# zhoubin-me/agent0

Hardware: AMD Instinct MI355X
Metric: env-frames/sec (learner FPS: transitions collected and saved to replay per second with the learner running, pre-frameskip) (higher is better)
Workload: dtype f32

## Files before the change

### agent0_amd/csrc/a0_internal.h

```cpp
#pragma once
#include "../../include/agent0_hip.h"
#include "a0_defs.h"

#include <exception>
#if defined(__HIPCC__)
#include <hip/hip_ext.h>
#endif
#include <stdexcept>
#include <string>

int a0_fail(int code, const char* msg);
int a0_fail_hip(int hip_error, const char* what);

struct a0_hip_error : std::runtime_error {
    int err;
    a0_hip_error(int e, const std::string& w) : std::runtime_error(w), err(e) {}
};

#define A0_STR2(x) #x
#define A0_STR(x) A0_STR2(x)
#define A0_HIP_THROW(expr)                                                                                  \
    do {                                                                                                    \
        hipError_t a0_e_ = (expr);                                                                          \
        if (a0_e_ != hipSuccess) throw a0_hip_error((int)a0_e_, std::string(__FILE__ ":" A0_STR(__LINE__) ": ") + hipGetErrorString(a0_e_)); \
    } while (0)

#define A0_TRY try {
#define A0_CATCH                                                   \
    }                                                              \
    catch (const a0_hip_error& e) { return a0_fail_hip(e.err, e.what()); } \
    catch (const std::exception& e) { return a0_fail(A0_EINVAL, e.what()); } \
    catch (...) { return a0_fail(A0_EINVAL, "unknown C++ exception"); }

void a0_trace_push_internal(const char* name);
void a0_trace_pop_internal();
struct a0_trace_scope {
    explicit a0_trace_scope(const char* name) { a0_trace_push_internal(name); }
    ~a0_trace_scope() { a0_trace_pop_internal(); }
    a0_trace_scope(const a0_trace_scope&) = delete;
    a0_trace_scope& operator=(const a0_trace_scope&) = delete;
};

#if defined(__HIPCC__)
bool a0_probe_start(int tag, hipStream_t st);
int a0_conv1_wgrad_fused_launch(const a0_frames_arg* f, int C, int H, int W, int B, const float* d1, float* slabs, hipStream_t st);
void a0_probe_stop(hipStream_t st, double flops);
bool a0_probe_events(int tag, hipEvent_t* start, hipEvent_t* stop);
void a0_probe_commit(double flops);
int a0_x9_products_now();
#define A0_LAUNCH_PROBED(tag, flops, kern, grid, block, lds, st, ...)                                                              \
    do {                                                                                                                           \
        hipEvent_t a0_e0_ = nullptr, a0_e1_ = nullptr;                                                                             \
        if (a0_probe_events((tag), &a0_e0_, &a0_e1_)) {                                                                            \
            hipExtLaunchKernelGGL(kern, grid, block, (uint32_t)(lds), st, a0_e0_, a0_e1_, 0, __VA_ARGS__);                         \
            a0_probe_commit(flops);                                                                                                \
        } else                                                                                                                     \
            hipLaunchKernelGGL(kern, grid, block, lds, st, __VA_ARGS__);                                                           \
    } while (0)
struct a0_net_core;
int a0_conv23_wgrad_fused_launch(const a0_net_core& n, int B, const float* act1, const float* act2, const float* d2, const float* d3, float* slab2, float* slab3,
                                 hipStream_t st);
#endif
#define A0_TAG_ENCODER_FUSED 12
#define A0_TAG_ENCODER_DGRAD_FUSED 13
#define A0_TAG_ACTOR_STEP_ENC 14
```

### agent0_amd/csrc/actor_tail.h

```cpp
#pragma once
#include "synth_env.h"
template <class Issued>
A0_D void a0_qhead_wave(const float* __restrict__ slabs, long long slab_stride, int nslab, const float* __restrict__ b1, const float* __restrict__ w2s,
                        const float* __restrict__ b2, int A, int dueling, int er, int lane, float* __restrict__ raw, unsigned long long seed, uint32_t stream_a,
                        uint32_t stream_u, unsigned long long off_a, unsigned long long off_u, float eps, int& out_action, float& out_best, Issued&& issued) {
    const int NQ = A + (dueling ? 1 : 0);
    bool hooked = false;
    float h[8];
#pragma unroll
    for (int i = 0; i < 8; ++i) h[i] = 0.f;
    const float* sp = slabs + (long long)er * 512 + lane;
    int z = 0;
    for (; z + 8 <= nslab; z += 8) {
        float t[8][8];
#pragma unroll
        for (int zz = 0; zz < 8; ++zz)
#pragma unroll
            for (int i = 0; i < 8; ++i) t[zz][i] = sp[(long long)(z + zz) * slab_stride + 64 * i];
        if (!hooked) { issued(); hooked = true; }
#pragma unroll
        for (int zz = 0; zz < 8; ++zz)
#pragma unroll
            for (int i = 0; i < 8; ++i) h[i] += t[zz][i];
    }
// ... 195 lines not shown
    }
    __builtin_amdgcn_fence(__ATOMIC_RELEASE, "wavefront");
    __builtin_amdgcn_wave_barrier();
    __builtin_amdgcn_fence(__ATOMIC_ACQUIRE, "wavefront");
    {
        if (P.dueling) {
            for (int t = lane; t < T; t += 64) {
                float s = 0.f;
                for (int a = 0; a < A; ++a) s += xs[a * T + t];
                const float mean = s / (float)A;
                const float v = xs[A * T + t];
                for (int a = 0; a < A; ++a) xs[a * T + t] = v + (xs[a * T + t] - mean);
            }
            __builtin_amdgcn_fence(__ATOMIC_RELEASE, "wavefront");
            __builtin_amdgcn_wave_barrier();
            __builtin_amdgcn_fence(__ATOMIC_ACQUIRE, "wavefront");
        }
        float best = 0.f;
        int besta = 0;
        for (int a = 0; a < A; ++a) {
            const float* p = xs + a * T;
            float v;
            if (P.mode == 1) {
                float s = 0.f;
                for (int t = lane; t < T; t += 64) s += p[t];
                v = a0_wave_sum(s) / (float)T;
            } else if (P.mode == 3) {
                const float* tau = P.taus + (long long)e * (T + 1);
                float s = 0.f;
                for (int t = lane; t < T; t += 64) s += (tau[t + 1] - tau[t]) * p[t];
                v = a0_wave_sum(s);
            } else {
                float mx = -INFINITY;
                for (int t = lane; t < T; t += 64) mx = fmaxf(mx, p[t]);
                mx = a0_wave_max(mx);
                float se = 0.f, sz = 0.f;
                for (int t = lane; t < T; t += 64) {
                    float ex = expf(p[t] - mx);
                    se += ex;
                    sz += ex * P.atoms[t];
                }
                se = a0_wave_sum(se);
                sz = a0_wave_sum(sz);
                v = sz / se;
            }
            if (a == 0 || v > best) { best = v; besta = a; }
        }
        if (lane == 0) {
            const int ra = (int)(a0_philox_word(seed_v, sa_v, off_a + (unsigned long long)e) % (uint32_t)A);
            const float u = (float)(a0_philox_word(seed_v, su_v, off_u + (unsigned long long)e) >> 8) * 0x1.0p-24f;
            const int act = (u > eps) ? besta : ra;
            action_v[e] = act; qmax_v[e] = best;
            float r_chase = 0.f;
            if (chase) *s_chase_cell_p = a0_chase_step(a0_chase_cell(P.obs_in + ((size_t)e * 4 + 3) * A0_ENV_PIX, e), act, x.w, r_chase);
            a0_env_commit_finish(Z, x, e, g, task_v, A, E_v, n_v, steps, gamma_v, act, O.ep_ret, O.final_mask, O.final_ret, O.ring_act, O.ring_rew, O.ring_done, O.r_act, O.r_rew,
                                 O.r_done, slot, r_chase);
        }
    }
}

A0_D void a0_actor_dist_tail_env_body(const a0_dtenv_args& P, float* __restrict__ xs, int* __restrict__ s_chase_cell_p) {
    const int wave = __builtin_amdgcn_readfirstlane(threadIdx.x >> 6);
    const uint32_t e = blockIdx.x;
    uint32_t g = P.g; long long start = P.start;
    if (P.ctrl) { g += (uint32_t)P.ctrl[A0_CTRL_ENV_STEP]; start += P.ctrl[A0_CTRL_REPLAY_SLOT]; }
    const long long slot = (start + e) % P.cap;
    uint32_t e_v = e;
    asm volatile("" : "+v"(e_v));
    const a0_u4 x = a0_philox4x32_10(e_v, g, 0u, 0x454E56u, (uint32_t)P.env_seed, (uint32_t)(P.env_seed >> 32) ^ P.rank);
    const bool term = (x.y % 500u) == 0u;
    const bool chase = P.task == A0_ENV_TASK_CHASE;
    if (wave != 0) {
        int cell = -1;
        if (chase) { __syncthreads(); cell = *s_chase_cell_p; }
        a0_env_commit_frames(P.env_seed, e, g, term, P.obs_in, P.obs_out, P.obs0, P.frames + slot * (8LL * A0_ENV_PIX), (int)threadIdx.x - 64, 448, cell);
        return;
    }
    a0_actor_dist_tail_wave0(P, xs, s_chase_cell_p, g, slot, x);
    if (chase) __syncthreads();
}


struct a0_encoder_weights;
int a0_actor_step_enc_launch(const a0_qenv_args& Q, const float* wt, const a0_encoder_weights* w, float* act3, hipStream_t st);
int a0_actor_dist_step_enc_launch(const a0_dtenv_args& Q, size_t tail_lds, const float* wt, const a0_encoder_weights* w, float* act3, hipStream_t st);
```

### agent0_amd/csrc/encoder_fused.hip

```cpp
#include "a0_internal.h"
#include "net_tables.h"
#include "operands.h"

#include <cstdlib>
#include <type_traits>

#ifndef A0_X9_MAXORD
#define A0_X9_MAXORD 4
#endif
typedef float a0_acc4 __attribute__((ext_vector_type(4)));

struct a0_fused_args {
    const uint8_t* frames; const int* slot; long long sample_stride; int chan_off;
    const float *wt1, *wt2, *wt3;
    const float *wx2, *wx3;
    const float *b1, *b2, *b3;
    float *act1, *act2, *act3;
    int B;
    int C, H, W, H1, W1, H2, W2, H3, W3;
    int off_act1, off_act2, off_end;
    int rp1, rp2;
};

#ifndef A0_FUSED_WAVES_D
#define A0_FUSED_WAVES_D 8
#endif
constexpr int A0_FUSED_WAVES = A0_FUSED_WAVES_D;
constexpr int A0_WMG1 = A0_FUSED_WAVES / 2;
constexpr int A0_FUSED_THREADS = 64 * A0_FUSED_WAVES;
constexpr int A0_P1 = 33;
constexpr int A0_P2 = 66;

struct AF2 {
    const float* act; int RP1, W2;
    A0_D int row(int m) const { const int oh = m / W2, ow = m - oh * W2; return (2 * oh) * RP1 + 2 * ow * A0_P1; }
    A0_D int chunk_off(int c) const { const int cell = c >> 1; return (cell >> 2) * RP1 + (cell & 3) * A0_P1 + 16 * (c & 1); }
    A0_D int step_off(int s) const { return 4 * s; }
    typedef float Raw;
    A0_D Raw load(int addr) const { return act[addr]; }
    static A0_D float value(Raw r) { return r; }
};
struct AF3 {
    const float* act; int RP2, W3;
    A0_D int row(int m) const { const int oh = m / W3, ow = m - oh * W3; return oh * RP2 + ow * A0_P2; }
    A0_D int chunk_off(int c) const { const int cell = c >> 2; return (cell / 3) * RP2 + (cell % 3) * A0_P2 + 16 * (c & 3); }
    A0_D int step_off(int s) const { return 4 * s; }
    typedef float Raw;
    A0_D Raw load(int addr) const { return act[addr]; }
    static A0_D float value(Raw r) { return r; }
};

template <int N, int WN, int R>
struct a0_wring {
    static constexpr int NBW = N / 16 / WN;
    a0_f4 v[R][NBW];
    const float* base;
    const float* p;
    int nch, left;
    A0_D void init(const float* wp, int K) {
        const int lane = threadIdx.x & 63, wave = __builtin_amdgcn_readfirstlane(threadIdx.x >> 6);
        const int n = (wave % WN) * (NBW * 16) + (lane & 15), q = lane >> 4;
        base = wp + (n * 4 + q) * 4;
        nch = K >> 4;
    }
    A0_D void fill(int slot) {
#pragma unroll
        for (int j = 0; j < NBW; ++j) v[slot][j] = *(const a0_f4*)(p + j * 256);
        const bool more = left > 1;
        p += more ? N * 16 : 0;
        left -= more ? 1 : 0;
    }
    A0_D void prologue() {
        p = base; left = nch;
#pragma unroll
        for (int u = 0; u < R; ++u) fill(u);
    }
};
A0_D float a0_f4_get(const a0_f4& v, int j) { return j == 0 ? v.x : j == 1 ? v.y : j == 2 ? v.z : v.w; }

template <int OWC>
struct EpiFwd {
    static constexpr bool PER_ELEM = false;
    static constexpr bool TR = false;
    const float* bias; float* lds; int pitch, rp, ow; float* glb; int N;
    A0_D float pre_col(int n) const { return bias[n]; }
    A0_D float pre_elem(int, int) const { return 0.f; }
    A0_D void emit(int m, int n, float acc, float pre) const {
        float v = acc + pre;
        v = (v < 0.f) ? 0.f : v;
        if (lds) {
            const int w_ = OWC > 0 ? OWC : ow, oh = m / w_;
            lds[oh * rp + (m - oh * w_) * pitch + n] = v;
        }
        if (glb) glb[(unsigned)(m * N + n)] = v;
    }
    static constexpr bool ROW4 = OWC > 0 && (OWC % 4) == 0;
    A0_D void emit4(int m0, int n, const a0_acc4& acc, float pre) const {
        constexpr int OWD = OWC > 0 ? OWC : 1;
        const int oh = m0 / OWD, ow0 = m0 - oh * OWD;
        float* l = lds ? lds + oh * rp + ow0 * pitch + n : nullptr;
// ... 225 lines not shown
            }
        }
    }
    __syncthreads();
}

template <int N, int WN, int R, int WK = 1>
struct a0_wring9 {
    static constexpr int NBW = N / 16 / WN;
    uint4 v[R][NBW][3];
    const uint4* base;
    const uint4* p;
    int nst, left, stride;
    A0_D void init(const float* wp, int K) {
        const int lane = threadIdx.x & 63, wave = __builtin_amdgcn_readfirstlane(threadIdx.x >> 6);
        base = (const uint4*)wp + (((wave % WN) * (NBW * 16) + (lane & 15)) * 4 + (lane >> 4)) * 3 + (WK > 1 ? (wave / WN) * (N * 12) : 0);
        nst = (K >> 5) / WK;
        stride = N * 12 * WK;
    }
    A0_D void init_at(const uint4* first, int own_steps, int step) { base = first; nst = own_steps; stride = step; }
    A0_D void fill(int slot) {
#pragma unroll
        for (int j = 0; j < NBW; ++j)
#pragma unroll
            for (int s = 0; s < 3; ++s) v[slot][j][s] = p[j * 192 + s];
        const bool more = left > 1;
        p += more ? stride : 0;
        left -= more ? 1 : 0;
    }
    A0_D void prologue() {
        p = base; left = nst;
#pragma unroll
        for (int u = 0; u < R; ++u) fill(u);
    }
};
template <int TERM>
struct AF2X {
    static constexpr int term = TERM;
    const uint16_t* planes; int RP, W2, P;
    A0_D int row(int m) const { const int oh = m / W2, ow = m - oh * W2; return (2 * oh) * RP + 2 * ow * P; }
    A0_D int step_off(int st) const { return (st >> 2) * RP + (st & 3) * P; }
};
template <int TERM>
struct AF3X {
    static constexpr int term = TERM;
    const uint16_t* planes; int RP, W3, P;
    A0_D int row(int m) const { const int oh = m / W3, ow = m - oh * W3; return oh * RP + ow * P; }
    A0_D int step_off(int st) const { const int tap = st >> 1; return (tap / 3) * RP + (tap % 3) * P + 32 * (st & 1); }
};
A0_D void a0_split4(const float (&v)[4], uint2& hi, uint2& mid, uint2& lo) {
    uint32_t h[4], m[4], l[4];
#pragma unroll
    for (int r = 0; r < 4; ++r) {
        h[r] = __float_as_uint(v[r]);
        const float r1 = v[r] - __uint_as_float(h[r] & 0xffff0000u);
        m[r] = __float_as_uint(r1);
        l[r] = __float_as_uint(r1 - __uint_as_float(m[r] & 0xffff0000u));
    }
    hi = uint2{__builtin_amdgcn_perm(h[1], h[0], 0x07060302u), __builtin_amdgcn_perm(h[3], h[2], 0x07060302u)};
    mid = uint2{__builtin_amdgcn_perm(m[1], m[0], 0x07060302u), __builtin_amdgcn_perm(m[3], m[2], 0x07060302u)};
    lo = uint2{__builtin_amdgcn_perm(l[1], l[0], 0x07060302u), __builtin_amdgcn_perm(l[3], l[2], 0x07060302u)};
}
template <int OWC, int P, int RP, int term>
struct EpiFwdX {
    static constexpr bool PER_ELEM = false;
    static constexpr bool ROW4 = false;
    static constexpr bool TR = true;
    static_assert(OWC > 0 && (P % 4) == 0 && (RP % 4) == 0 && (term % 4) == 0, "output width known at compile time; 8-byte aligned plane writes");
    const float* bias; uint16_t* planes; float* glb; int N;
    A0_D float pre_col(int) const { return 0.f; }
    A0_D void emit_n4(int m, int n0, const a0_acc4& acc, const float*) const {
        const a0_f4 bv = *(const a0_f4*)(bias + n0);
        float v[4] = {acc[0] + bv.x, acc[1] + bv.y, acc[2] + bv.z, acc[3] + bv.w};
#pragma unroll
        for (int r = 0; r < 4; ++r) v[r] = (v[r] < 0.f) ? 0.f : v[r];
        if (glb) *(a0_f4*)(glb + (unsigned)(m * N + n0)) = a0_f4{v[0], v[1], v[2], v[3]};
        uint2 hi, mid, lo;
        a0_split4(v, hi, mid, lo);
        const int oh = m / OWC;
        uint16_t* d = planes + oh * RP + (m - oh * OWC) * P + n0;
        *(uint2*)d = hi; *(uint2*)(d + term) = mid; *(uint2*)(d + 2 * term) = lo;
    }
};
struct EpiFwdT {
    static constexpr bool PER_ELEM = false;
    static constexpr bool ROW4 = false;
    static constexpr bool TR = true;
    const float* bias; float* glb; int N;
    A0_D float pre_col(int) const { return 0.f; }
    A0_D void emit_n4(int m, int n0, const a0_acc4& acc, const float*) const {
        const a0_f4 bv = *(const a0_f4*)(bias + n0);
        float v[4] = {acc[0] + bv.x, acc[1] + bv.y, acc[2] + bv.z, acc[3] + bv.w};
#pragma unroll
        for (int r = 0; r < 4; ++r) v[r] = (v[r] < 0.f) ? 0.f : v[r];
        *(a0_f4*)(glb + (unsigned)(m * N + n0)) = a0_f4{v[0], v[1], v[2], v[3]};
    }
};

template <int ORD, int N, int WN, int MBW, int R, int MBWP, class AFX, class EPI, class Between>
A0_D void a0_conv_stage_x9(const AFX& af, int M, a0_wring9<N, WN, R>& ring, const EPI& epi, const a0_pre<N, WN, MBWP, EPI>& pre, Between&& between) {
    constexpr int NB = N / 16, NBW = NB / WN, WMG = A0_FUSED_WAVES / WN;
    static_assert(NBW >= 1 && (R % 2) == 0 && MBWP >= MBW, "tile shape");
    const int tid = threadIdx.x, lane = tid & 63;
    const int wave = __builtin_amdgcn_readfirstlane(tid >> 6);
    const int wn = wave % WN, wmg = wave / WN;
    const int q = lane >> 4, r16 = lane & 15;
    const int MB = (M + 15) >> 4, NST = ring.nst;
    int rows[MBW];
#pragma unroll
    for (int i = 0; i < MBW; ++i) {
        const int m = (wmg + i * WMG) * 16 + r16;
        rows[i] = af.row(m < M ? m : 0) + 8 * q;
    }
    a0_acc4 acc[MBW][NBW];
#pragma unroll
    for (int i = 0; i < MBW; ++i)
#pragma unroll
        for (int j = 0; j < NBW; ++j) acc[i][j] = a0_acc4{0.f, 0.f, 0.f, 0.f};
    uint4 a[2][MBW][3];
    auto fetch = [&](int slot, int off) {
#pragma unroll
        for (int i = 0; i < MBW; ++i)
#pragma unroll
            for (int t = 0; t < 3; ++t) a[slot][i][t] = *(const uint4*)(af.planes + rows[i] + off + t * AFX::term);
    };
    fetch(0, af.step_off(0));
    __builtin_amdgcn_s_waitcnt(0x0F70);
#pragma unroll 1
    for (int tb = 0; tb < NST; tb += R) {
#pragma unroll
        for (int u = 0; u < R; ++u) {
            const int nxt = tb + u + 1;
            fetch((u + 1) & 1, af.step_off(nxt < NST ? nxt : NST - 1));
            __builtin_amdgcn_sched_barrier(0);
#pragma unroll
            for (int ta = 0; ta < 3; ++ta)
#pragma unroll
                for (int tw = 0; tw < 3; ++tw)
#pragma unroll
                    for (int i = 0; i < MBW; ++i)
#pragma unroll
                        for (int jn = 0; jn < NBW; ++jn) {
                            if (ta + tw > ORD) continue;
                            const a0_u32x4 av = {a[u & 1][i][ta].x, a[u & 1][i][ta].y, a[u & 1][i][ta].z, a[u & 1][i][ta].w};
                            const a0_u32x4 bv = {ring.v[u][jn][tw].x, ring.v[u][jn][tw].y, ring.v[u][jn][tw].z, ring.v[u][jn][tw].w};
                            if constexpr (EPI::TR) acc[i][jn] = __builtin_amdgcn_mfma_f32_16x16x32_bf16(__builtin_bit_cast(a0_bf16x8, bv), __builtin_bit_cast(a0_bf16x8, av), acc[i][jn], 0, 0, 0);
                            else acc[i][jn] = __builtin_amdgcn_mfma_f32_16x16x32_bf16(__builtin_bit_cast(a0_bf16x8, av), __builtin_bit_cast(a0_bf16x8, bv), acc[i][jn], 0, 0, 0);
                        }
            __builtin_amdgcn_sched_barrier(0);
            ring.fill(u);
            __builtin_amdgcn_sched_barrier(0);
        }
    }
    between();
#pragma unroll
    for (int i = 0; i < MBW; ++i) {
        const int mb = wmg + i * WMG;
        if (mb < MB) {
            if constexpr (EPI::TR) {
                const int m = mb * 16 + r16;
                if (m < M) {
#pragma unroll
                    for (int j = 0; j < NBW; ++j) epi.emit_n4(m, (wn * NBW + j) * 16 + 4 * q, acc[i][j], EPI::PER_ELEM ? pre.pe[EPI::PER_ELEM ? i : 0][j] : pre.pc[j]);
                }
            } else {
#pragma unroll
                for (int j = 0; j < NBW; ++j) {
                    const int n = (wn * NBW + j) * 16 + r16;
#pragma unroll
                    for (int r = 0; r < 4; ++r) {
                        const int m = mb * 16 + 4 * q + r;
                        if (m < M) epi.emit(m, n, acc[i][j][r], EPI::PER_ELEM ? pre.pe[EPI::PER_ELEM ? i : 0][j][r] : pre.pc[j][0]);
                    }
                }
            }
        }
    }
    __syncthreads();
// ... 52 lines not shown
                __builtin_amdgcn_sched_barrier(0);
            }
            ring.fill(u);
            __builtin_amdgcn_sched_barrier(0);
        }
    }
    between();
    a0_acc4* x0 = (a0_acc4*)xch0;
    a0_acc4* x1 = (a0_acc4*)xch1;
    constexpr int P1 = (HB1 - 1) * 64 + 4 * LR;
    const int last = q * LR + r16;
    const int n0 = wn * 16 + 4 * q;
    float pe[EPI::PER_ELEM ? HB0 : 1][4];
    auto send = [&](auto mine) {
        constexpr int H = decltype(mine)::value;
        if constexpr (EPI::PER_ELEM) {
#pragma unroll
            for (int i = 0; i < (H == 0 ? HB0 : HB1); ++i) {
                const int m = (H * HB0 + i) * 16 + r16;
                const a0_f4 v = epi.pre_elem4(m < M ? m : M - 1, n0);
                pe[i][0] = v.x; pe[i][1] = v.y; pe[i][2] = v.z; pe[i][3] = v.w;
            }
        }
        if constexpr (H == 1) {
#pragma unroll
            for (int i = 0; i < HB0; ++i) x0[(wn * HB0 + i) * 64 + lane] = acc[i];
        } else {
#pragma unroll
            for (int i = 0; i < HB1; ++i) {
                if (i < HB1 - 1) x1[wn * P1 + i * 64 + lane] = acc[HB0 + i];
                else if (r16 < LR) x1[wn * P1 + (HB1 - 1) * 64 + last] = acc[HB0 + i];
            }
        }
    };
    auto recv = [&](auto mine) {
        constexpr int H = decltype(mine)::value;
#pragma unroll
        for (int i = 0; i < (H == 0 ? HB0 : HB1); ++i) {
            const int mb = H * HB0 + i;
            const int m = mb * 16 + r16;
            if constexpr (H == 0) acc[mb] += x0[(wn * HB0 + i) * 64 + lane];
            else {
                if (i < HB1 - 1) acc[mb] += x1[wn * P1 + i * 64 + lane];
                else if (r16 < LR) acc[mb] += x1[wn * P1 + (HB1 - 1) * 64 + last];
            }
            if (mb < MB && m < M) epi.emit_n4(m, n0, acc[mb], EPI::PER_ELEM ? pe[EPI::PER_ELEM ? i : 0] : nullptr);
        }
    };
    if (wk == 0) send(std::integral_constant<int, 0>{});
    else send(std::integral_constant<int, 1>{});
    __syncthreads();
    if (wk == 0) recv(std::integral_constant<int, 0>{});
    else recv(std::integral_constant<int, 1>{});
    __syncthreads();
}
constexpr int A0_P1X = 40, A0_P2X = 80;
#ifndef A0_PADS
#define A0_PADS 1
#endif
constexpr int A0_RP1X = 20 * A0_P1X + (A0_PADS ? 8 : 0);
constexpr int A0_RP2X = 9 * A0_P2X + (A0_PADS ? 96 : 0);
#ifndef A0_RX2_D
#define A0_RX2_D 4
#endif
#ifndef A0_RX3_D
#define A0_RX3_D 6
#endif
[[maybe_unused]] constexpr int A0_RX2 = A0_RX2_D, A0_RX3 = A0_RX3_D;
#ifndef A0_KSPLIT_D
#define A0_KSPLIT_D 1
#endif
#ifndef A0_KSPLIT
#define A0_KSPLIT 1
#endif
#ifndef A0_WNX
#define A0_WNX 4
#endif

constexpr int A0_R1 = 4, A0_R2 = 4, A0_R3 = 6;

#ifndef A0_FUSED_MINWAVES
#define A0_FUSED_MINWAVES 1
#endif
template <int MBW1, int MBW2, int MBW3, int WC, bool X9, bool LOOP = false, int ORD = 4>
__global__ __launch_bounds__(A0_FUSED_THREADS, A0_FUSED_MINWAVES) void a0_encoder_fused_kernel(a0_fused_args P);

constexpr int A0_X9_BIAS_OFF = 2 * 4 * 84 * 84 + 3 * 20 * A0_RP1X * 2;
#ifndef A0_RK2_D
#define A0_RK2_D 2
#endif
#ifndef A0_RK3_D
#define A0_RK3_D 3
#endif
constexpr int A0_RK2 = A0_RK2_D, A0_RK3 = A0_RK3_D;
constexpr int A0_X9_XCH0 = 3 * 9 * A0_RP2X * 2;
constexpr int A0_X9_XCH1 = A0_X9_BIAS_OFF + 160 * 4;
static_assert(A0_X9_XCH0 + 4 * 3 * 1024 <= 2 * 4 * 84 * 84, "conv2 exchange region 0 fits into the image");
constexpr int A0_X9_LDS_BYTES = A0_X9_XCH1 + (A0_KSPLIT ? 4 * (2 * 64 + 4) * 16 : 0);
static_assert(A0_X9_LDS_BYTES <= 160 * 1024, "LDS");
#if A0_KSPLIT
typedef a0_wring9<64, 4, A0_RK2, 2> a0_ring2_t;
typedef a0_wring9<64, 4, A0_RK3, 2> a0_ring3_t;
#else
typedef a0_wring9<64, A0_WNX, A0_RX2> a0_ring2_t;
typedef a0_wring9<64, A0_WNX, A0_RX3> a0_ring3_t;
#endif
template <int ORD, int MBW2, int MBW3, bool LOOP>
A0_D void a0_x9_conv23(const a0_fused_args& P, int b, unsigned char* smem, float* bias_lds, a0_wring1<A0_R1>& ring1, a0_ring2_t& ring2, a0_ring3_t& ring3) {
    const int obs_bytes = P.C * P.H * P.W;
    const int M2 = P.H2 * P.W2, M3 = P.H3 * P.W3;
    uint16_t* a1p = (uint16_t*)(smem + 2 * obs_bytes);
    constexpr int term1 = 20 * A0_RP1X, term2 = 9 * A0_RP2X;
    uint16_t* a2p = (uint16_t*)smem;
    typedef EpiFwdX<9, A0_P2X, A0_RP2X, term2> E2X;
    constexpr int WNX = A0_WNX, WMGX = A0_FUSED_WAVES / WNX;
    constexpr int MBW2X = (6 + WMGX - 1) / WMGX, MBW3X = (4 + WMGX - 1) / WMGX;
    static_assert(MBW2X <= MBW2 * 2 && MBW3X <= MBW3 * 2, "84x84 geometry");
#if !A0_KSPLIT
    a0_pre<64, WNX, MBW2X, E2X> pre2;
    a0_pre<64, WNX, MBW3X, EpiFwdT> pre3;
#endif
    (void)a1p; (void)term1;
    {
        const AF2X<term1> f2{a1p, A0_RP1X, P.W2, A0_P1X};
        const E2X e2{bias_lds + 32, a2p, P.act2 ? P.act2 + (long long)b * M2 * 64 : nullptr, 64};
#if A0_KSPLIT
        const AF3X<term2> f3k{a2p, A0_RP2X, P.W3, A0_P2X};
        const EpiFwdT e3k{bias_lds + 96, P.act3 + (long long)b * M3 * 64, 64};
        a0_conv_stage_x9k<ORD, 64, 4, 6, A0_RK2, 1>(f2, M2, ring2, e2, (float*)(smem + A0_X9_XCH0), (float*)(smem + A0_X9_XCH1), [&] { ring3.prologue(); });
        a0_conv_stage_x9k<ORD, 64, 4, 4, A0_RK3, 16>(f3k, M3, ring3, e3k, (float*)a1p, (float*)a1p + 4 * 2 * 256, [&] { if (LOOP) ring1.prologue(); });
#else
        const int wmgx = __builtin_amdgcn_readfirstlane(threadIdx.x >> 6) / WNX;
        constexpr bool uneven2 = MBW2X > 1 && MBW2X * WMGX > 6, uneven3 = MBW3X > 1 && MBW3X * WMGX > 4;
        if (uneven2 && wmgx + (MBW2X - 1) * WMGX >= 6)
            a0_conv_stage_x9<ORD, 64, WNX, (MBW2X > 1 ? MBW2X - 1 : 1), A0_RX2>(f2, M2, ring2, e2, pre2, [&] { ring3.prologue(); });
        else
            a0_conv_stage_x9<ORD, 64, WNX, MBW2X, A0_RX2>(f2, M2, ring2, e2, pre2, [&] { ring3.prologue(); });
        const AF3X<term2> f3{a2p, A0_RP2X, P.W3, A0_P2X};
        const EpiFwdT e3{bias_lds + 96, P.act3 + (long long)b * M3 * 64, 64};
        if (uneven3 && wmgx + (MBW3X - 1) * WMGX >= 4)
            a0_conv_stage_x9<ORD, 64, WNX, (MBW3X > 1 ? MBW3X - 1 : 1), A0_RX3>(f3, M3, ring3, e3, pre3, [&] { if (LOOP) ring1.prologue(); });
        else
            a0_conv_stage_x9<ORD, 64, WNX, MBW3X, A0_RX3>(f3, M3, ring3, e3, pre3, [&] { if (LOOP) ring1.prologue(); });
#endif
    }
}

template <int ORD, int MBW1, int MBW2, int MBW3, bool LOOP>
A0_D void a0_encoder_fused_x9_body(const a0_fused_args& P, int bid, int nblk) {
    extern __shared__ __attribute__((aligned(16))) unsigned char smem[];
    uint16_t* img = (uint16_t*)smem;
    const int obs_bytes = P.C * P.H * P.W;
    const int M1 = P.H1 * P.W1;
    uint16_t* a1p = (uint16_t*)(smem + 2 * obs_bytes);
    constexpr int term1 = 20 * A0_RP1X;
    typedef EpiFwdX<20, A0_P1X, A0_RP1X, term1> E1X;
    constexpr int WNX = A0_WNX, WMGX = A0_FUSED_WAVES / WNX;
    constexpr int MBW2X = (6 + WMGX - 1) / WMGX, MBW3X = (4 + WMGX - 1) / WMGX;
    static_assert(MBW2X <= MBW2 * 2 && MBW3X <= MBW3 * 2, "84x84 geometry");
    a0_wring1<A0_R1> ring1;
#if A0_KSPLIT
    static_assert(WNX == 4 && A0_FUSED_WAVES == 8, "N-stationary stages: four waves along N, two along K");
#endif
    a0_ring2_t ring2;
    a0_ring3_t ring3;
    ring1.init(P.wt1, P.C);
    ring2.init(P.wx2, 512);
    ring3.init(P.wx3, 576);
    ring1.prologue();
    constexpr int MBW1X = (25 + A0_WMG1 - 1) / A0_WMG1;
    static_assert(A0_FUSED_WAVES != 8 || MBW1X == MBW1, "84x84 geometry");
    a0_pre<32, 2, MBW1X, E1X> pre1;
    float* bias_lds = (float*)(smem + A0_X9_BIAS_OFF);
    if (threadIdx.x < 160) bias_lds[threadIdx.x] = threadIdx.x < 32 ? P.b1[threadIdx.x] : threadIdx.x < 96 ? P.b2[threadIdx.x - 32] : P.b3[threadIdx.x - 96];
    for (int b = bid; b < P.B; b += nblk) {
        const long long s = P.slot ? (long long)P.slot[b] : (long long)b;
        const uint4* src = (const uint4*)(P.frames + s * P.sample_stride + P.chan_off);
        constexpr int TRIPS = 4;
        const int n16 = obs_bytes >> 4;
        for (int i0 = threadIdx.x; i0 < n16; i0 += TRIPS * A0_FUSED_THREADS) {
            uint4 v[TRIPS];
#pragma unroll
            for (int j = 0; j < TRIPS; ++j) {
                const int i = i0 + j * A0_FUSED_THREADS;
                v[j] = src[i < n16 ? i : n16 - 1];
            }
#pragma unroll
            for (int j = 0; j < TRIPS; ++j) {
                int i = i0 + j * A0_FUSED_THREADS;
                i = i < n16 ? i : n16 - 1;
                const uint32_t w[4] = {v[j].x, v[j].y, v[j].z, v[j].w};
                uint32_t o[8];
#pragma unroll
                for (int k = 0; k < 4; ++k) {
                    const uint32_t f0 = __float_as_uint((float)(w[k] & 0xffu)), f1 = __float_as_uint((float)((w[k] >> 8) & 0xffu));
                    const uint32_t f2 = __float_as_uint((float)((w[k] >> 16) & 0xffu)), f3 = __float_as_uint((float)(w[k] >> 24));
                    o[2 * k] = __builtin_amdgcn_perm(f1, f0, 0x07060302u);
                    o[2 * k + 1] = __builtin_amdgcn_perm(f3, f2, 0x07060302u);
                }
                ((uint4*)img)[2 * i] = uint4{o[0], o[1], o[2], o[3]};
                ((uint4*)img)[2 * i + 1] = uint4{o[4], o[5], o[6], o[7]};
            }
        }
        __syncthreads();
        const E1X e1{bias_lds, a1p, P.act1 ? P.act1 + (long long)b * M1 * 32 : nullptr, 32};
        const int wmg1 = __builtin_amdgcn_readfirstlane(threadIdx.x >> 6) / 2;
        if (MBW1X > 1 && wmg1 + (MBW1X - 1) * A0_WMG1 >= ((M1 + 15) >> 4))
            a0_conv1_stage<(MBW1X > 1 ? MBW1X - 1 : 1), A0_R1, 84>(img, P.H * P.W, P.W, P.W1, M1, ring1, e1, pre1, [&] { ring2.prologue(); });
        else
            a0_conv1_stage<MBW1X, A0_R1, 84>(img, P.H * P.W, P.W, P.W1, M1, ring1, e1, pre1, [&] { ring2.prologue(); });
        a0_x9_conv23<ORD, MBW2, MBW3, LOOP>(P, b, smem, bias_lds, ring1, ring2, ring3);
        if constexpr (!LOOP) break;
    }
}

#include "actor_tail.h"
struct a0_step_enc_args { const float *wt, *b1, *b2, *b3; float* act3; };
template <int ORD>
__global__ __launch_bounds__(A0_FUSED_THREADS, A0_FUSED_MINWAVES) void a0_actor_dist_step_enc_kernel(a0_dtenv_args Q, a0_step_enc_args N) {
    __shared__ int s_chase_cell;
    extern __shared__ __attribute__((aligned(16))) unsigned char smem[];
    unsigned long long v_wt = (unsigned long long)N.wt, v_b1 = (unsigned long long)N.b1, v_b2 = (unsigned long long)N.b2, v_b3 = (unsigned long long)N.b3,
                       v_a3 = (unsigned long long)N.act3, v_obs = (unsigned long long)Q.obs_out;
    A0_TO_VGPR(v_wt); A0_TO_VGPR(v_b1); A0_TO_VGPR(v_b2); A0_TO_VGPR(v_b3); A0_TO_VGPR(v_a3); A0_TO_VGPR(v_obs);
    int v_E = Q.E;
    A0_TO_VGPR(v_E);
    a0_actor_dist_tail_env_body(Q, (float*)smem, &s_chase_cell);
    __syncthreads();
    auto uni = [](unsigned long long v) {
        return ((unsigned long long)(unsigned)__builtin_amdgcn_readfirstlane((int)(v >> 32)) << 32) | (unsigned long long)(unsigned)__builtin_amdgcn_readfirstlane((int)(v & 0xffffffffull));
    };
    const float* wt = (const float*)uni(v_wt);
    a0_fused_args P;
    P.frames = (const uint8_t*)uni(v_obs); P.slot = nullptr; P.sample_stride = 4 * 84 * 84; P.chan_off = 0;
    P.wt1 = wt; P.wt2 = wt + 48LL * 4 * 64; P.wt3 = P.wt2 + 64LL * 512;
    P.wx2 = P.wt3 + 64LL * 576 + 64LL * 576 + 4LL * 32 * 256; P.wx3 = P.wx2 + 96LL * 512;
    P.b1 = (const float*)uni(v_b1); P.b2 = (const float*)uni(v_b2); P.b3 = (const float*)uni(v_b3);
    P.act1 = nullptr; P.act2 = nullptr; P.act3 = (float*)uni(v_a3); P.B = __builtin_amdgcn_readfirstlane(v_E);
    P.C = 4; P.H = 84; P.W = 84; P.H1 = 20; P.W1 = 20; P.H2 = 9; P.W2 = 9; P.H3 = 7; P.W3 = 7;
    P.off_act1 = 0; P.off_act2 = 0; P.off_end = 0; P.rp1 = 0; P.rp2 = 0;
    a0_encoder_fused_x9_body<ORD, 7, 3, 2, false>(P, (int)blockIdx.x, (int)gridDim.x);
}

A0_D void a0_bytes16_to_img(uint16_t* img, int idx16, const uint4 v) {
    const uint32_t w[4] = {v.x, v.y, v.z, v.w};
    uint32_t o[8];
#pragma unroll
    for (int k = 0; k < 4; ++k) {
        const uint32_t f0 = __float_as_uint((float)(w[k] & 0xffu)), f1 = __float_as_uint((float)((w[k] >> 8) & 0xffu));
        const uint32_t f2 = __float_as_uint((float)((w[k] >> 16) & 0xffu)), f3 = __float_as_uint((float)(w[k] >> 24));
        o[2 * k] = __builtin_amdgcn_perm(f1, f0, 0x07060302u);
        o[2 * k + 1] = __builtin_amdgcn_perm(f3, f2, 0x07060302u);
    }
    ((uint4*)img)[2 * idx16] = uint4{o[0], o[1], o[2], o[3]};
    ((uint4*)img)[2 * idx16 + 1] = uint4{o[4], o[5], o[6], o[7]};
}

template <int MBW, class EPI, class Mid, class Between>
A0_D void a0_conv1_stage_split(const uint16_t* img, a0_wring1<A0_R1>& ring, const EPI& epi, bool first_before_mid, Mid&& mid, Between&& between) {
    static_assert(A0_R1 == 4 && EPI::TR, "ring of four steps, transposed accumulators");
    constexpr int HW = 84 * 84, W = 84, W1 = 20, M = 400, MB = 25;
    const int tid = threadIdx.x, lane = tid & 63;
    const int wave = __builtin_amdgcn_readfirstlane(tid >> 6);
    const int wn = wave % 2, wmg = wave / 2;
    const int q = lane >> 4, r16 = lane & 15;
    int rows[MBW];
#pragma unroll
    for (int i = 0; i < MBW; ++i) {
        int m = (wmg + i * A0_WMG1) * 16 + r16;
        m = m < M ? m : 0;
        const int oh = m / W1, ow = m - oh * W1;
        rows[i] = (4 * oh + q) * W + 4 * ow;
    }
    a0_acc4 acc[MBW];
#pragma unroll
    for (int i = 0; i < MBW; ++i) acc[i] = a0_acc4{0.f, 0.f, 0.f, 0.f};
    uint2 a[2][MBW][2];
    auto fetch = [&](int slot, int off) {
#pragma unroll
        for (int i = 0; i < MBW; ++i) {
            a[slot][i][0] = *(const uint2*)(img + rows[i] + off);
            a[slot][i][1] = *(const uint2*)(img + rows[i] + off + 4);
        }
    };
    auto off_of = [&](int st) { return (st >> 1) * HW + (st & 1) * 4 * W; };
    auto step = [&](auto UC, int off_next) {
        constexpr int u = decltype(UC)::value;
        fetch((u + 1) & 1, off_next);
        __builtin_amdgcn_sched_barrier(0);
#pragma unroll
        for (int s3 = 0; s3 < 3; ++s3)
#pragma unroll
            for (int i = 0; i < MBW; ++i) {
                const a0_u32x4 av = {a[u & 1][i][0].x, a[u & 1][i][0].y, a[u & 1][i][1].x, a[u & 1][i][1].y};
                const a0_u32x4 bv = {ring.v[u][s3].x, ring.v[u][s3].y, ring.v[u][s3].z, ring.v[u][s3].w};
                acc[i] = __builtin_amdgcn_mfma_f32_16x16x32_bf16(__builtin_bit_cast(a0_bf16x8, bv), __builtin_bit_cast(a0_bf16x8, av), acc[i], 0, 0, 0);
            }
        __builtin_amdgcn_sched_barrier(0);
        ring.fill(u);
        __builtin_amdgcn_sched_barrier(0);
    };
    typedef std::integral_constant<int, 0> U0; typedef std::integral_constant<int, 1> U1; typedef std::integral_constant<int, 2> U2; typedef std::integral_constant<int, 3> U3;
    auto steps05 = [&] {
        fetch(0, off_of(0));
        __builtin_amdgcn_s_waitcnt(0x0F70);
        step(U0{}, off_of(1)); step(U1{}, off_of(2)); step(U2{}, off_of(3)); step(U3{}, off_of(4));
        step(U0{}, off_of(5)); step(U1{}, off_of(5));
    };
    if (first_before_mid) steps05();
    mid();
    if (!first_before_mid) steps05();
    fetch(0, off_of(6));
    __builtin_amdgcn_s_waitcnt(0x0F70);
    step(U2{}, off_of(7)); step(U3{}, off_of(7));
    between();
#pragma unroll
    for (int i = 0; i < MBW; ++i) {
        const int mb = wmg + i * A0_WMG1;
        if (mb < MB) {
            const int m = mb * 16 + r16;
            if (m < M) epi.emit_n4(m, wn * 16 + 4 * q, acc[i], nullptr);
        }
    }
    __syncthreads();
}

struct TailScalar {
    typedef a0_qenv_args Args;
    static A0_D void run(const a0_qenv_args& Q, uint32_t e, uint32_t g, long long steps, unsigned long long off_a, unsigned long long off_u, float eps, long long slot, const a0_u4& x,
                         bool chase, int lane, float* w2s , float* raw, int* s_chase_cell_p) {
        const int NQ = Q.A + (Q.dueling ? 1 : 0);
        a0_env_pre Z;
        a0_env_commit_prefetch(Z, e, Q.E, Q.n, steps, Q.ep_ret, Q.ring_act, Q.ring_rew, Q.ring_done);
        a0_env_pre_to_vgpr(Z);
        const a0_env_out O = a0_env_out_vgpr(Q.ep_ret, Q.final_mask, Q.final_ret, Q.ring_act, Q.ring_rew, Q.ring_done, Q.r_act, Q.r_rew, Q.r_done);
        A0_TO_VGPR(steps); A0_TO_VGPR(off_a); A0_TO_VGPR(off_u); A0_TO_VGPR(eps);
        int n_v = Q.n, E_v = Q.E, task_v = Q.task; double gamma_v = Q.gamma; int* action_v = Q.action; float* qmax_v = Q.qmax;
        A0_TO_VGPR(n_v); A0_TO_VGPR(E_v); A0_TO_VGPR(task_v); A0_TO_VGPR(gamma_v); A0_TO_VGPR(action_v); A0_TO_VGPR(qmax_v);
#pragma unroll 4
        for (int i = lane; i < NQ * 128; i += 64) ((a0_f4*)w2s)[i] = ((const a0_f4*)Q.W2)[i];
        __builtin_amdgcn_fence(__ATOMIC_RELEASE, "wavefront");
        __builtin_amdgcn_wave_barrier();
        __builtin_amdgcn_fence(__ATOMIC_ACQUIRE, "wavefront");
        int act = 0; float best = 0.f;
        a0_qhead_wave(Q.slabs, Q.slab_stride, Q.nslab, Q.b1, w2s, Q.b2, Q.A, Q.dueling, (int)e, lane, raw, Q.rng_seed, Q.stream_a, Q.stream_u, off_a, off_u, eps, act, best);
        if (lane == 0) {
            action_v[e] = act; qmax_v[e] = best;
            float r_chase = 0.f;
            if (chase) *s_chase_cell_p = a0_chase_step(a0_chase_cell(Q.obs_in + ((size_t)e * 4 + 3) * A0_ENV_PIX, e), act, x.w, r_chase);
            a0_env_commit_finish(Z, x, e, g, task_v, Q.A, E_v, n_v, steps, gamma_v, act, O.ep_ret, O.final_mask, O.final_ret, O.ring_act, O.ring_rew, O.ring_done, O.r_act, O.r_rew,
                                 O.r_done, slot, r_chase);
        }
    }
};
template <int ORD, class TAIL>
A0_D void a0_actor_step_enc2_body(const typename TAIL::Args& Q, const a0_step_enc_args& N) {
    __shared__ float raw[64];
    __shared__ int s_chase_cell;
    extern __shared__ __attribute__((aligned(16))) unsigned char smem[];
    constexpr int HW = 84 * 84, G16 = HW / 16;
    uint16_t* img = (uint16_t*)smem;
    uint16_t* a1p = (uint16_t*)(smem + 2 * 4 * HW);
    const int tid = threadIdx.x, lane = tid & 63, wave = __builtin_amdgcn_readfirstlane(tid >> 6);
    const uint32_t e = blockIdx.x;
    a0_fused_args P;
    P.frames = nullptr; P.slot = nullptr; P.sample_stride = 4 * HW; P.chan_off = 0;
    P.wt1 = N.wt; P.wt2 = N.wt + 48LL * 4 * 64; P.wt3 = P.wt2 + 64LL * 512;
    P.wx2 = P.wt3 + 64LL * 576 + 64LL * 576 + 4LL * 32 * 256; P.wx3 = P.wx2 + 96LL * 512;
    P.b1 = N.b1; P.b2 = N.b2; P.b3 = N.b3;
    P.act1 = nullptr; P.act2 = nullptr; P.act3 = N.act3; P.B = Q.E;
    P.C = 4; P.H = 84; P.W = 84; P.H1 = 20; P.W1 = 20; P.H2 = 9; P.W2 = 9; P.H3 = 7; P.W3 = 7;
    P.off_act1 = 0; P.off_act2 = 0; P.off_end = 0; P.rp1 = 0; P.rp2 = 0;
    a0_wring1<A0_R1> ring1;
    a0_ring2_t ring2;
    a0_ring3_t ring3;
    ring1.init(P.wt1, 4);
    ring1.prologue();
    float* bias_lds = (float*)(smem + A0_X9_BIAS_OFF);
    if (tid < 160) bias_lds[tid] = tid < 32 ? P.b1[tid] : tid < 96 ? P.b2[tid - 32] : P.b3[tid - 96];
    unsigned long long v_wx2 = (unsigned long long)P.wx2, v_wx3 = (unsigned long long)P.wx3;
    A0_TO_VGPR(v_wx2); A0_TO_VGPR(v_wx3);
    uint32_t g = Q.g; long long steps = Q.steps, start = Q.start; unsigned long long off_a = Q.off_a, off_u = Q.off_u; float eps = Q.eps;
    if (Q.ctrl) {
        g += (uint32_t)Q.ctrl[A0_CTRL_ENV_STEP]; steps += Q.ctrl[A0_CTRL_ACTOR_STEPS]; start += Q.ctrl[A0_CTRL_REPLAY_SLOT];
        off_a += (unsigned long long)Q.ctrl[A0_CTRL_RNG_ACTION]; off_u += (unsigned long long)Q.ctrl[A0_CTRL_RNG_UNIFORM];
    }
    if (Q.eps_ptr) eps = Q.eps_ptr[0];
    const long long slot = (start + e) % Q.cap;
    uint32_t e_v = e;
    asm volatile("" : "+v"(e_v));
    const a0_u4 x = a0_philox4x32_10(e_v, g, 0u, 0x454E56u, (uint32_t)Q.env_seed, (uint32_t)(Q.env_seed >> 32) ^ Q.rank);
    const bool term = __builtin_amdgcn_readfirstlane((int)((x.y % 500u) == 0u)) != 0;
    const bool chase = Q.task == A0_ENV_TASK_CHASE;
    const bool early = !(chase && term);
    const int j = tid - 64;
    auto has_group = [&] { int jj = j; asm volatile("" : "+v"(jj)); return wave != 0 && jj < G16; };
    const uint32_t pbase = (uint32_t)Q.env_seed ^ a0_env_mix32(e * 0x9E3779B1u + g);
    uint4* out16 = (uint4*)(Q.obs_out + (size_t)e * 4 * HW) + j;
    uint4* row16 = (uint4*)(Q.frames + slot * (8LL * HW)) + j;
    A0_TO_VGPR(out16); A0_TO_VGPR(row16);
    float* act3_v = N.act3;
    A0_TO_VGPR(act3_v);
    auto new_group = [&](uint32_t by, uint32_t bx) {
        uint32_t w[4];
#pragma unroll
        for (int k = 0; k < 4; ++k) {
            const uint32_t p = 16u * (uint32_t)j + 4u * (uint32_t)k;
            w[k] = (uint32_t)a0_env_pixel(pbase, by, bx, p, chase) | ((uint32_t)a0_env_pixel(pbase, by, bx, p + 1, chase) << 8) |
                   ((uint32_t)a0_env_pixel(pbase, by, bx, p + 2, chase) << 16) | ((uint32_t)a0_env_pixel(pbase, by, bx, p + 3, chase) << 24);
        }
        return uint4{w[0], w[1], w[2], w[3]};
    };
    auto put = [&](int c, const uint4 v) {
        out16[c * G16] = v; row16[(4 + c) * G16] = v;
        a0_bytes16_to_img(img, c * G16 + j, v);
    };
    __shared__ int s_staged;
    if (tid == 0) s_staged = 0;
    __syncthreads();
    uint4 keep[9];
    if (wave == 0) {
        TAIL::run(Q, e, g, steps, off_a, off_u, eps, slot, x, chase, lane, (float*)a1p, raw, &s_chase_cell);
    } else {
        if (has_group()) {
            const uint4* in16 = (const uint4*)(Q.obs_in + (size_t)e * 4 * HW) + j;
            A0_TO_VGPR(in16);
            const uint4 i0 = in16[0], i1 = in16[G16], i2 = in16[2 * G16], i3 = in16[3 * G16];
            if (Q.obs0 == Q.obs_in) { keep[0] = i0; keep[1] = i1; keep[2] = i2; keep[3] = i3; }
            else {
                const uint4* o016 = (const uint4*)(Q.obs0 + (size_t)e * 4 * HW) + j;
                A0_TO_VGPR(o016);
                keep[0] = o016[0]; keep[1] = o016[G16]; keep[2] = o016[2 * G16]; keep[3] = o016[3 * G16];
            }
            if (!chase) {
                const uint4 nw = new_group((3u * g + 11u * e) % 77u, (5u * g + 7u * e) % 77u);
                if (term) { keep[4] = nw; keep[5] = nw; keep[6] = nw; } else { keep[4] = i1; keep[5] = i2; keep[6] = i3; }
                keep[7] = nw;
                for (int c = 0; c < 4; ++c) a0_bytes16_to_img(img, c * G16 + j, keep[4 + c]);
            } else if (!term) {
                keep[4] = i1; keep[5] = i2; keep[6] = i3;
                for (int c = 0; c < 3; ++c) a0_bytes16_to_img(img, c * G16 + j, keep[4 + c]);
            }
        }
        asm volatile("s_waitcnt lgkmcnt(0)" ::: "memory");
        if (lane == 0) atomicAdd(&s_staged, 1);
        while (__builtin_amdgcn_readfirstlane(*(volatile int*)&s_staged) < A0_FUSED_WAVES - 1) __builtin_amdgcn_s_sleep(1);
    }
    auto early_stores = [&] {
        if (has_group()) {
#pragma unroll
            for (int c = 0; c < 4; ++c) row16[c * G16] = keep[c];
            const int nc = !chase ? 4 : (!term ? 3 : 0);
#pragma unroll
            for (int c = 0; c < 4; ++c)
                if (c < nc) { out16[c * G16] = keep[4 + c]; row16[(4 + c) * G16] = keep[4 + c]; }
        }
    };
    auto mid = [&] {
        if (wave != 0) early_stores();
        __syncthreads();
        if (chase) {
            if (has_group()) {
                uint32_t by, bx;
                a0_chase_pos(s_chase_cell, by, bx);
                const uint4 nw = new_group(by, bx);
                if (term) { put(0, nw); put(1, nw); put(2, nw); }
                put(3, nw);
            }
            __syncthreads();
        }
    };
    auto uni = [](unsigned long long v) {
        return ((unsigned long long)(unsigned)__builtin_amdgcn_readfirstlane((int)(v >> 32)) << 32) | (unsigned long long)(unsigned)__builtin_amdgcn_readfirstlane((int)(v & 0xffffffffull));
    };
    ring2.init((const float*)uni(v_wx2), 512);
    ring3.init((const float*)uni(v_wx3), 576);
    typedef EpiFwdX<20, A0_P1X, A0_RP1X, 20 * A0_RP1X> E1X;
    const E1X e1{bias_lds, a1p, nullptr, 32};
    constexpr int MBW1X = (25 + A0_WMG1 - 1) / A0_WMG1;
    const bool before = early && wave != 0;
    if (MBW1X > 1 && wave / 2 + (MBW1X - 1) * A0_WMG1 >= 25)
        a0_conv1_stage_split<(MBW1X > 1 ? MBW1X - 1 : 1)>(img, ring1, e1, before, mid, [&] { ring2.prologue(); });
    else
        a0_conv1_stage_split<MBW1X>(img, ring1, e1, before, mid, [&] { ring2.prologue(); });
    P.act3 = (float*)uni((unsigned long long)act3_v);
    a0_x9_conv23<ORD, 3, 2, false>(P, (int)e, smem, bias_lds, ring1, ring2, ring3);
}

template <int ORD>
__global__ __launch_bounds__(A0_FUSED_THREADS, A0_FUSED_MINWAVES) void a0_actor_step_enc2_kernel(a0_qenv_args Q, a0_step_enc_args N) { a0_actor_step_enc2_body<ORD, TailScalar>(Q, N); }

static bool a0_fused_layout(int C, int H, int W, a0_fused_args& P, size_t& lds_bytes);
int a0_actor_dist_step_enc_launch(const a0_dtenv_args& Q, size_t tail_lds, const float* wt, const a0_encoder_weights* w, float* act3, hipStream_t st) {
    a0_fused_args P;
    size_t lds = 0;
    if (!wt || !w || !w->b1 || !w->b2 || !w->b3 || !act3 || !a0_fused_layout(4, 84, 84, P, lds)) return a0_fail(A0_EINVAL, "a0_actor_dist_tail_env_step_enc: bad encoder argument");
    if (P.H1 != 20 || P.W1 != 20 || P.H2 != 9 || P.W2 != 9 || P.H3 != 7 || P.W3 != 7) return a0_fail(A0_EINVAL, "a0_actor_dist_tail_env_step_enc: geometry");
    const a0_step_enc_args N{wt, w->b1, w->b2, w->b3, act3};
    lds = A0_X9_LDS_BYTES > tail_lds ? (size_t)A0_X9_LDS_BYTES : tail_lds;
    if (lds > 160 * 1024 - 64) return a0_fail(A0_EINVAL, "a0_actor_dist_tail_env_step_enc: head too wide for LDS");
    const int six = a0_x9_products_now() == 6;
    auto kern = six ? a0_actor_dist_step_enc_kernel<2> : a0_actor_dist_step_enc_kernel<4>;
    static size_t configured[2] = {0, 0};
    if (lds > configured[six]) {
        if (hipFuncSetAttribute((const void*)kern, hipFuncAttributeMaxDynamicSharedMemorySize, (int)lds) != hipSuccess)
            return a0_fail(A0_EINVAL, "a0_actor_dist_tail_env_step_enc: LDS");
        configured[six] = lds;
    }
    A0_LAUNCH_PROBED(A0_TAG_ACTOR_STEP_ENC, 2.0 * (400.0 * 32 * 256 + 81.0 * 64 * 512 + 49.0 * 64 * 576) * Q.E, kern, dim3(Q.E), dim3(A0_FUSED_THREADS), lds, st, Q, N);
    return a0_fail_hip((int)hipGetLastError(), "a0_actor_dist_tail_env_step_enc");
}
int a0_actor_step_enc_launch(const a0_qenv_args& Q, const float* wt, const a0_encoder_weights* w, float* act3, hipStream_t st) {
    a0_fused_args P;
    size_t lds = 0;
    if (!wt || !w || !w->b1 || !w->b2 || !w->b3 || !act3 || !a0_fused_layout(4, 84, 84, P, lds)) return a0_fail(A0_EINVAL, "a0_actor_qhead_env_step_enc: bad encoder argument");
    if (P.H1 != 20 || P.W1 != 20 || P.H2 != 9 || P.W2 != 9 || P.H3 != 7 || P.W3 != 7) return a0_fail(A0_EINVAL, "a0_actor_qhead_env_step_enc: geometry");
    const a0_step_enc_args N{wt, w->b1, w->b2, w->b3, act3};
    const size_t tail_lds = (size_t)(Q.A + (Q.dueling ? 1 : 0)) * 512 * sizeof(float);
    lds = A0_X9_LDS_BYTES > tail_lds ? (size_t)A0_X9_LDS_BYTES : tail_lds;
    const int six = a0_x9_products_now() == 6;
    auto kern = six ? a0_actor_step_enc2_kernel<2> : a0_actor_step_enc2_kernel<4>;
    static size_t configured[2] = {0, 0};
    if (lds > configured[six]) {
        if (hipFuncSetAttribute((const void*)kern, hipFuncAttributeMaxDynamicSharedMemorySize, (int)lds) != hipSuccess)
            return a0_fail(A0_EINVAL, "a0_actor_qhead_env_step_enc: LDS");
        configured[six] = lds;
    }
    A0_LAUNCH_PROBED(A0_TAG_ACTOR_STEP_ENC, 2.0 * (400.0 * 32 * 256 + 81.0 * 64 * 512 + 49.0 * 64 * 576) * Q.E, kern, dim3(Q.E), dim3(A0_FUSED_THREADS), lds, st, Q, N);
    return a0_fail_hip((int)hipGetLastError(), "a0_actor_qhead_env_step_enc");
}

struct a0_fused_multi_args { a0_fused_args p[3]; int first[4]; };
template <int ORD>
__global__ __launch_bounds__(A0_FUSED_THREADS, A0_FUSED_MINWAVES) void a0_encoder_fused_multi_kernel(a0_fused_multi_args M) {
    const int bid = (int)blockIdx.x;
    const int k = bid >= M.first[2] ? 2 : (bid >= M.first[1] ? 1 : 0);
    a0_encoder_fused_x9_body<ORD, 7, 3, 2, true>(M.p[k], bid - M.first[k], M.first[k + 1] - M.first[k]);
}

template <int MBW1, int MBW2, int MBW3, int WC, bool X9, bool LOOP, int ORD>
__global__ __launch_bounds__(A0_FUSED_THREADS, A0_FUSED_MINWAVES) void a0_encoder_fused_kernel(a0_fused_args P) {
    if constexpr (X9) {
        a0_encoder_fused_x9_body<ORD, MBW1, MBW2, MBW3, LOOP>(P, (int)blockIdx.x, (int)gridDim.x);
        return;
    }
    extern __shared__ __attribute__((aligned(16))) unsigned char smem[];
    uint16_t* img = (uint16_t*)smem;
    float* fl = (float*)smem;
    float* act1 = fl + P.off_act1;
    float* act2 = fl + P.off_act2;
    const int obs_bytes = P.C * P.H * P.W;
    const int M1 = P.H1 * P.W1, M2 = P.H2 * P.W2, M3 = P.H3 * P.W3;
    a0_wring1<A0_R1> ring1;
    a0_wring<64, 4, A0_R2> ring2;
    a0_wring<64, 4, A0_R3> ring3;
    ring1.init(P.wt1, P.C);
    ring2.init(P.wt2, 512);
    ring3.init(P.wt3, 576);
    ring1.prologue();
    constexpr int OW1 = WC == 84 ? 20 : 0, OW2 = WC == 84 ? 9 : 0;
    a0_pre<32, 2, MBW1, EpiFwd<OW1>> pre1;
    a0_pre<64, 4, MBW2, EpiFwd<OW2>> pre2;
    a0_pre<64, 4, MBW3, EpiFwd<0>> pre3;
    pre1.load(EpiFwd<OW1>{P.b1, nullptr, 0, 0, 1, nullptr, 32}, M1);
    pre2.load(EpiFwd<OW2>{P.b2, nullptr, 0, 0, 1, nullptr, 64}, M2);
    pre3.load(EpiFwd<0>{P.b3, nullptr, 0, 0, 1, nullptr, 64}, M3);
    for (int b = blockIdx.x; b < P.B; b += gridDim.x) {
        const long long s = P.slot ? (long long)P.slot[b] : (long long)b;
        const uint4* src = (const uint4*)(P.frames + s * P.sample_stride + P.chan_off);
        constexpr int TRIPS = 4;
        const int n16 = obs_bytes >> 4;
        for (int i0 = threadIdx.x; i0 < n16; i0 += TRIPS * A0_FUSED_THREADS) {
            uint4 v[TRIPS];
#pragma unroll
            for (int j = 0; j < TRIPS; ++j) {
                const int i = i0 + j * A0_FUSED_THREADS;
                v[j] = src[i < n16 ? i : n16 - 1];
            }
#pragma unroll
            for (int j = 0; j < TRIPS; ++j) {
                int i = i0 + j * A0_FUSED_THREADS;
                i = i < n16 ? i : n16 - 1;
                const uint32_t w[4] = {v[j].x, v[j].y, v[j].z, v[j].w};
                uint32_t o[8];
#pragma unroll
                for (int k = 0; k < 4; ++k) {
                    const uint32_t f0 = __float_as_uint((float)(w[k] & 0xffu)), f1 = __float_as_uint((float)((w[k] >> 8) & 0xffu));
                    const uint32_t f2 = __float_as_uint((float)((w[k] >> 16) & 0xffu)), f3 = __float_as_uint((float)(w[k] >> 24));
                    o[2 * k] = __builtin_amdgcn_perm(f1, f0, 0x07060302u);
                    o[2 * k + 1] = __builtin_amdgcn_perm(f3, f2, 0x07060302u);
                }
                ((uint4*)img)[2 * i] = uint4{o[0], o[1], o[2], o[3]};
                ((uint4*)img)[2 * i + 1] = uint4{o[4], o[5], o[6], o[7]};
            }
        }
        __syncthreads();
        const EpiFwd<OW1> e1{P.b1, act1, A0_P1, P.rp1, P.W1, P.act1 ? P.act1 + (long long)b * M1 * 32 : nullptr, 32};
        const int wmg1 = __builtin_amdgcn_readfirstlane(threadIdx.x >> 6) / 2;
        if (MBW1 > 1 && wmg1 + (MBW1 - 1) * 4 >= ((M1 + 15) >> 4))
            a0_conv1_stage<(MBW1 > 1 ? MBW1 - 1 : 1), A0_R1, WC>(img, P.H * P.W, P.W, P.W1, M1, ring1, e1, pre1, [&] { ring2.prologue(); });
        else
            a0_conv1_stage<MBW1, A0_R1, WC>(img, P.H * P.W, P.W, P.W1, M1, ring1, e1, pre1, [&] { ring2.prologue(); });
        AF2 f2{act1, P.rp1, P.W2};
        const EpiFwd<OW2> e2{P.b2, act2, A0_P2, P.rp2, P.W2, P.act2 ? P.act2 + (long long)b * M2 * 64 : nullptr, 64};
        a0_conv_stage<64, 4, MBW2, 3, A0_R2>(f2, M2, 512, ring2, e2, pre2, [&] { ring3.prologue(); });
        AF3 f3{act2, P.rp2, P.W3};
        const EpiFwd<0> e3{P.b3, nullptr, 0, 0, 1, P.act3 + (long long)b * M3 * 64, 64};
        a0_conv_stage<64, 4, MBW3, 3, A0_R3>(f3, M3, 576, ring3, e3, pre3, [&] { ring1.prologue(); });
    }
}

struct a0_dgrad_args {
    const float *d3, *act1, *act2;
    float *d2, *d1;
    const float *wd3, *wd2;
    int B;
};
constexpr int A0_RPDA = 11 * A0_P2X + (A0_PADS ? 96 : 0), A0_RPDB = 11 * A0_P2X + (A0_PADS ? 48 : 0);
constexpr int A0_DTERMA = 11 * A0_RPDA, A0_DTERMB = 11 * A0_RPDB;
struct AFD3X {
    static constexpr int term = A0_DTERMA;
    const uint16_t* planes;
    A0_D int row(int m) const { const int oh = m / 9, ow = m - oh * 9; return oh * A0_RPDA + ow * A0_P2X; }
    A0_D int step_off(int st) const { const int tap = st >> 1; return (tap / 3) * A0_RPDA + (tap % 3) * A0_P2X + 32 * (st & 1); }
};
struct AFD2X {
// ... 202 lines not shown
                out |= (s == 0 ? hi : s == 1 ? mid : lo) << (16 * h);
            }
            { *(uint32_t*)dst = out; if (mirror) *(uint32_t*)(wt2 + (dst - wt)) = out; }
            return;
        }
    }
    int N, seg;
    if (i < n2) { seg = 2; N = 64; }
    else if ((i -= n2) < n3) { seg = 3; N = 64; }
    else if ((i -= n3) < n4) { seg = 4; N = 64; }
    else if ((i -= n4) < n5) { seg = 5; N = 32; }
    else return;
    const int phase = seg == 5 ? i / 8192 : 0;
    if (seg == 5) i -= phase * 8192;
    const int j = i & 3, q = (i >> 2) & 3, n = (i >> 4) % N, c = (i >> 4) / N;
    const int k = 16 * c + 4 * j + q;
    float v;
    if (seg == 2) v = w2[n * 512 + k];
    else if (seg == 3) v = w3[n * 576 + k];
    else if (seg == 4) {
        const int cell = k >> 6, co = k & 63, kh = 2 - cell / 3, kw = 2 - cell % 3;
        v = w3[co * 576 + (kh * 3 + kw) * 64 + n];
    } else {
        const int cell = k >> 6, co = k & 63, kh = (phase >> 1) + 2 * (1 - (cell >> 1)), kw = (phase & 1) + 2 * (1 - (cell & 1));
        v = w2[co * 512 + (kh * 4 + kw) * 32 + n];
    }
    *dst = v;
    if (mirror) wt2[dst - wt] = v;
}

extern "C" long long a0_net_conv_wt_floats(int C) {
    return 48LL * C * 64 + 64LL * 512 + 64LL * 576 + 64LL * 576 + 4LL * 32 * 256 + 96LL * 512 + 96LL * 576 + 96LL * 576 + 4LL * 48 * 256;
}

extern "C" int a0_net_conv_wt_refresh(const a0_encoder_weights* w, int C, float* wt, void* stream) {
    if (!w || !w->w1 || !w->w2 || !w->w3 || !wt || C < 1) return a0_fail(A0_EINVAL, "a0_net_conv_wt_refresh: bad argument");
    const long long n = a0_net_conv_wt_floats(C);
    hipLaunchKernelGGL(a0_conv_wt_kernel, dim3((unsigned)((n + 255) / 256)), dim3(256), 0, (hipStream_t)stream, w->w1, w->w2, w->w3, wt, C * 64, (float*)nullptr,
                       (const int*)nullptr, (int*)nullptr);
    return a0_fail_hip((int)hipGetLastError(), "a0_net_conv_wt_refresh");
}

extern "C" int a0_net_conv_wt_refresh_sync(const a0_encoder_weights* w, int C, float* wt, float* wt_target, const int* state, void* stream) {
    if (!w || !w->w1 || !w->w2 || !w->w3 || !wt || !wt_target || !state || C < 1) return a0_fail(A0_EINVAL, "a0_net_conv_wt_refresh_sync: bad argument");
    const long long n = a0_net_conv_wt_floats(C);
    hipLaunchKernelGGL(a0_conv_wt_kernel, dim3((unsigned)((n + 255) / 256)), dim3(256), 0, (hipStream_t)stream, w->w1, w->w2, w->w3, wt, C * 64, wt_target, state, (int*)nullptr);
    return a0_fail_hip((int)hipGetLastError(), "a0_net_conv_wt_refresh_sync");
}

int a0_conv_wt_refresh_commit(const a0_encoder_weights* w, int C, float* wt, float* wt_target, int* state, hipStream_t st) {
    if (!w || !w->w1 || !w->w2 || !w->w3) return a0_fail(A0_EINVAL, "a0_adam_step_sync_wt: encoder weights missing");
    const long long n = a0_net_conv_wt_floats(C);
    hipLaunchKernelGGL(a0_conv_wt_kernel, dim3((unsigned)((n + 255) / 256)), dim3(256), 0, st, w->w1, w->w2, w->w3, wt, C * 64, wt_target, (const int*)state, state);
    return a0_fail_hip((int)hipGetLastError(), "a0_adam_step_sync_wt");
}

static bool a0_fused_layout(int C, int H, int W, a0_fused_args& P, size_t& lds_bytes) {
    a0_net_core n;
    if (!a0_net_core_init(n, C, H, W)) return false;
    const int M1 = n.H1 * n.W1, M2 = n.H2 * n.W2, M3 = n.H3 * n.W3;
    if (M1 > 7 * 4 * 16 || M2 > 4 * 2 * 16 || M3 > 2 * 2 * 16) return false;
    if ((C * 2) % A0_R1 || (W & 3)) return false;
    const int obs_bytes = C * H * W;
    if (obs_bytes % 16) return false;
    P.C = C; P.H = H; P.W = W; P.H1 = n.H1; P.W1 = n.W1; P.H2 = n.H2; P.W2 = n.W2; P.H3 = n.H3; P.W3 = n.W3;
    P.rp1 = n.W1 * A0_P1;
    while ((P.rp1 - n.W2) & 15) ++P.rp1;
    P.rp2 = n.W2 * A0_P2;
    while ((P.rp2 - 2 * n.W3) & 31) ++P.rp2;
    P.off_act1 = obs_bytes / 2;
    P.off_act2 = P.off_act1 + ((n.H1 * P.rp1 + 3) & ~3);
    P.off_end = P.off_act2 + ((n.H2 * P.rp2 + 3) & ~3);
    lds_bytes = (size_t)P.off_end * 4;
    return lds_bytes <= 160 * 1024;
}

extern "C" int a0_net_encoder_fused_supported(int C, int H, int W) {
    a0_fused_args P; size_t lds;
    return a0_fused_layout(C, H, W, P, lds) ? 1 : 0;
}

extern "C" int a0_net_encoder_fwd_fused(int C, int H, int W, const float* wt, const a0_encoder_weights* w, const a0_frames_arg* f, int B,
                                        float* act1, float* act2, float* act3, void* stream) {
    A0_TRY
    if (!wt || !w || !w->b1 || !w->b2 || !w->b3 || !f || !f->frames || !act3 || B < 1) return a0_fail(A0_EINVAL, "a0_net_encoder_fwd_fused: bad argument");
    a0_fused_args P;
    size_t lds = 0;
    if (!a0_fused_layout(C, H, W, P, lds)) return a0_fail(A0_EINVAL, "a0_net_encoder_fwd_fused: observation shape not supported by the fused kernel");
    if ((f->sample_stride % 16) || (f->chan_off % 16) || (((uintptr_t)f->frames) % 16)) return a0_fail(A0_EINVAL, "a0_net_encoder_fwd_fused: frames must be 16-byte aligned");
    P.frames = f->frames; P.slot = f->slot; P.sample_stride = f->sample_stride; P.chan_off = f->chan_off;
    P.wt1 = wt; P.wt2 = wt + 48LL * C * 64; P.wt3 = P.wt2 + 64LL * 512;
    P.wx2 = P.wt3 + 64LL * 576 + 64LL * 576 + 4LL * 32 * 256; P.wx3 = P.wx2 + 96LL * 512;
    P.b1 = w->b1; P.b2 = w->b2; P.b3 = w->b3;
    P.act1 = act1; P.act2 = act2; P.act3 = act3; P.B = B;
    const int mb1 = (P.H1 * P.W1 + 15) / 16, mb2 = (P.H2 * P.W2 + 15) / 16, mb3 = (P.H3 * P.W3 + 15) / 16;
    const bool standard = ((mb1 + 3) / 4 == 7) && ((mb2 + 1) / 2 == 3) && ((mb3 + 1) / 2 == 2) && W == 84;
    const bool x9 = standard && H == 84 && C == 4;
    int which = x9 ? 2 : (standard ? 1 : 0);
    if (x9) lds = A0_X9_LDS_BYTES;
    static_assert(3 * 9 * A0_RP2X * 2 <= 2 * 4 * 84 * 84, "the act2 term planes fit into the dead image");
    const int gridx = (which == 2 && B > 256) ? 256 : B;
    if (which == 2 && gridx < B) which = 3;
    static size_t configured[6] = {0, 0, 0, 0, 0, 0};
    const int six = a0_x9_products_now() == 6;
    if (six && which >= 2) which += 2;
    typedef void (*a0_enc_kern)(a0_fused_args);
    const a0_enc_kern fn = which == 5 ? a0_encoder_fused_kernel<7, 3, 2, 84, true, true, 2> : which == 4 ? a0_encoder_fused_kernel<7, 3, 2, 84, true, false, 2>
                         : which == 3 ? a0_encoder_fused_kernel<7, 3, 2, 84, true, true> : which == 2 ? a0_encoder_fused_kernel<7, 3, 2, 84, true>
                         : which == 1 ? a0_encoder_fused_kernel<7, 3, 2, 84, false> : a0_encoder_fused_kernel<7, 4, 2, 0, false>;
    if (lds > configured[which]) {
        A0_HIP_THROW(hipFuncSetAttribute((const void*)fn, hipFuncAttributeMaxDynamicSharedMemorySize, (int)lds));
        configured[which] = lds;
    }
    const double per_obs = 2.0 * ((double)P.H1 * P.W1 * 32 * (P.C * 64) + (double)P.H2 * P.W2 * 64 * 512 + (double)P.H3 * P.W3 * 64 * 576);
    A0_LAUNCH_PROBED(A0_TAG_ENCODER_FUSED, per_obs * B, fn, dim3((which == 3 || which == 5) ? gridx : B), dim3(A0_FUSED_THREADS), lds, (hipStream_t)stream, P);
    A0_HIP_THROW(hipGetLastError());
    return A0_OK;
    A0_CATCH
}

extern "C" int a0_net_encoder_fwd_fused_multi(int C, int H, int W, int n, const a0_encoder_pass* pass, void* stream) {
    A0_TRY
    if (n < 1 || n > 3 || !pass) return a0_fail(A0_EINVAL, "a0_net_encoder_fwd_fused_multi: 1 to 3 passes");
    if (!(C == 4 && H == 84 && W == 84)) return a0_fail(A0_EINVAL, "a0_net_encoder_fwd_fused_multi: 4 x 84 x 84 observations on the split-operand kernel only");
    a0_fused_multi_args M;
    size_t lds = 0;
    long long total = 0;
    for (int i = 0; i < n; ++i) {
        const a0_encoder_pass& q = pass[i];
        if (!q.wt || !q.w || !q.w->b1 || !q.w->b2 || !q.w->b3 || !q.f || !q.f->frames || !q.act3 || q.B < 1) return a0_fail(A0_EINVAL, "a0_net_encoder_fwd_fused_multi: bad pass");
        if ((q.f->sample_stride % 16) || (q.f->chan_off % 16) || (((uintptr_t)q.f->frames) % 16)) return a0_fail(A0_EINVAL, "a0_net_encoder_fwd_fused_multi: frames must be 16-byte aligned");
        a0_fused_args& P = M.p[i];
        if (!a0_fused_layout(C, H, W, P, lds)) return a0_fail(A0_EINVAL, "a0_net_encoder_fwd_fused_multi: observation shape");
        P.frames = q.f->frames; P.slot = q.f->slot; P.sample_stride = q.f->sample_stride; P.chan_off = q.f->chan_off;
        P.wt1 = q.wt; P.wt2 = q.wt + 48LL * C * 64; P.wt3 = P.wt2 + 64LL * 512;
        P.wx2 = P.wt3 + 64LL * 576 + 64LL * 576 + 4LL * 32 * 256; P.wx3 = P.wx2 + 96LL * 512;
        P.b1 = q.w->b1; P.b2 = q.w->b2; P.b3 = q.w->b3;
        P.act1 = q.act1; P.act2 = q.act2; P.act3 = q.act3; P.B = q.B;
        total += q.B;
    }
    for (int i = n; i < 3; ++i) M.p[i] = M.p[0];
    int grid = (int)(total < 256 ? total : 256), used = 0;
    if (grid < n) grid = n;
    for (int i = 0; i < n; ++i) {
        M.first[i] = used;
        int share = (i == n - 1) ? grid - used : (int)((long long)grid * pass[i].B / total);
        if (share < 1) share = 1;
        if (share > pass[i].B) share = pass[i].B;
        used += share;
    }
    for (int i = n; i <= 3; ++i) M.first[i] = 0x7fffffff;
    M.first[n] = used;
    lds = A0_X9_LDS_BYTES;
    const int six = a0_x9_products_now() == 6;
    auto kern = six ? a0_encoder_fused_multi_kernel<2> : a0_encoder_fused_multi_kernel<4>;
    static bool configured[2] = {false, false};
    if (!configured[six]) {
        A0_HIP_THROW(hipFuncSetAttribute((const void*)kern, hipFuncAttributeMaxDynamicSharedMemorySize, (int)lds));
        configured[six] = true;
    }
    const a0_fused_args& P0 = M.p[0];
    const double per_obs = 2.0 * ((double)P0.H1 * P0.W1 * 32 * (P0.C * 64) + (double)P0.H2 * P0.W2 * 64 * 512 + (double)P0.H3 * P0.W3 * 64 * 576);
    A0_LAUNCH_PROBED(A0_TAG_ENCODER_FUSED, per_obs * (double)total, kern, dim3(used), dim3(A0_FUSED_THREADS), lds, (hipStream_t)stream, M);
    A0_HIP_THROW(hipGetLastError());
    return A0_OK;
    A0_CATCH
}

extern "C" int a0_net_encoder_dgrad_fused_supported(int C, int H, int W) { return (C >= 1 && H == 84 && W == 84) ? 1 : 0; }

extern "C" int a0_net_encoder_dgrad_fused(int C, int H, int W, const float* wt, const float* d3, const float* act1, const float* act2, int B, float* d2,
                                          float* d1, void* stream) {
    A0_TRY
    if (!wt || !d3 || !act1 || !act2 || !d2 || !d1 || B < 1) return a0_fail(A0_EINVAL, "a0_net_encoder_dgrad_fused: bad argument");
    if (!a0_net_encoder_dgrad_fused_supported(C, H, W)) return a0_fail(A0_EINVAL, "a0_net_encoder_dgrad_fused: 84x84 observations only");
    a0_dgrad_args P;
    P.d3 = d3; P.act1 = act1; P.act2 = act2; P.d2 = d2; P.d1 = d1; P.B = B;
    P.wd3 = wt + 48LL * C * 64 + 64LL * 512 + 64LL * 576 + 64LL * 576 + 4LL * 32 * 256 + 96LL * 512 + 96LL * 576;
    P.wd2 = P.wd3 + 96LL * 576;
    const size_t lds = (size_t)3 * (A0_DTERMA + A0_DTERMB) * 2 + (A0_KSPLIT_D ? (4 * 4 + 4 * 3) * 1024 : 0);
    static bool configured[2] = {false, false};
    const int six = a0_x9_products_now() == 6;
    auto fn = six ? a0_encoder_dgrad_fused_x9_kernel<2> : a0_encoder_dgrad_fused_x9_kernel<4>;
    if (!configured[six]) {
        A0_HIP_THROW(hipFuncSetAttribute((const void*)fn, hipFuncAttributeMaxDynamicSharedMemorySize, (int)lds));
        configured[six] = true;
    }
    const int gridx = B > 256 ? 256 : B;
    A0_LAUNCH_PROBED(A0_TAG_ENCODER_DGRAD_FUSED, 2.0 * (81.0 * 64 * 576 + 400.0 * 32 * 256) * B, fn, dim3(gridx), dim3(A0_FUSED_THREADS), lds, (hipStream_t)stream, P);
    A0_HIP_THROW(hipGetLastError());
// ... 4 lines not shown
```

### agent0_amd/csrc/igemm_x9.h

```cpp
#pragma once
#include "igemm.h"
#if defined(__HIPCC__)
#include <hip/hip_ext.h>
#endif

#if defined(__HIPCC__)

typedef __bf16 a0_bf16x8g __attribute__((ext_vector_type(8)));
typedef short a0_s16x4 __attribute__((ext_vector_type(4)));
typedef uint32_t a0_u32x2g __attribute__((ext_vector_type(2)));
typedef uint32_t a0_u32x4g __attribute__((ext_vector_type(4)));

struct a0_x9_piece {
    a0_f4 v;
    uint32_t h[4], m[4], l[4];
    A0_D void split(int e) {
        const float x = e == 0 ? v.x : e == 1 ? v.y : e == 2 ? v.z : v.w;
        h[e] = __float_as_uint(x);
        const float r1 = x - __uint_as_float(h[e] & 0xffff0000u);
        m[e] = __float_as_uint(r1);
        const float r2 = r1 - __uint_as_float(m[e] & 0xffff0000u);
        l[e] = __float_as_uint(r2);
    }
    A0_D void pack(a0_u32x2g& hi, a0_u32x2g& mid, a0_u32x2g& lo) const {
// ... 105 lines not shown
struct a0_planes_src { const uint32_t* p; int kgroups; };
struct OpPlanesKC {
    static constexpr int MODE = A0_KC;
    typedef a0_planes_src Params;
    struct Row { const uint32_t* p; };
    struct KInfo { int g; };
    struct Raw { a0_u32x4g a; a0_u32x2g b; };
    A0_HD static Row row(const Params& P, int r, int R) { Row o; o.p = P.p + (long long)(r < R ? r : R - 1) * P.kgroups * 6; return o; }
    A0_HD static KInfo kinfo(const Params& P, int k, int Kend) { KInfo ki; ki.g = (k < Kend ? k : 0) >> 2; return ki; }
    A0_HD static Raw load(const Params&, const Row& r, const KInfo& ki) {
        Raw v;
        const uint32_t* q = r.p + (long long)ki.g * 6;
        v.a = *(const a0_u32x4g*)q;
        v.b = *(const a0_u32x2g*)(q + 4);
        return v;
    }
};
template <int BX, int NTH, int KS> struct a0_x9_stager<OpPlanesKC, BX, NTH, KS, A0_KC> {
    static constexpr bool PRESPLIT = true;
    static constexpr int TPR = 4 * KS;
    static constexpr int RPP = NTH / TPR;
    static constexpr int R = BX / RPP;
    static_assert(BX % RPP == 0, "tile rows per pass");
    typedef a0_x9_image<A0_KC, BX, KS> IM;
    typedef OpPlanesKC OP;
    OP::Row rows[R];
    OP::KInfo ki;
    struct Slot { OP::Raw raw[R]; unsigned okmask; };
    A0_D void init(const OP::Params& P, int x0, int X, int kb, int ke, int tid) {
#pragma unroll
        for (int j = 0; j < R; ++j) rows[j] = OP::row(P, x0 + tid / TPR + RPP * j, X);
        ki = OP::kinfo(P, kb + 4 * (tid % TPR), ke);
    }
    template <bool FULL = false> A0_D void fetch_piece(const OP::Params& P, Slot& s, int j, int k0, int ke, int tid) {
        s.raw[j] = OP::load(P, rows[j], ki);
        if (j == R - 1) ki = OP::kinfo(P, k0 + 16 * KS + 4 * (tid % TPR), ke);
    }
    template <bool RS, bool FULL = false> A0_D a0_f4 value(const Slot&, int, a0_f4&) const { return a0_zero4(); }
    A0_D void store(const a0_x9_piece&, int, char*, int) const {}
    A0_D void store_raw(const Slot& s, int j, char* lds, int tid) const {
        const int r = tid / TPR + RPP * j;
        char* p = lds + r * IM::PITCH + 8 * (tid % TPR);
        a0_u32x2g hi, mid; hi.x = s.raw[j].a.x; hi.y = s.raw[j].a.y; mid.x = s.raw[j].a.z; mid.y = s.raw[j].a.w;
        *(a0_u32x2g*)(p) = hi;
        *(a0_u32x2g*)(p + IM::PLANE) = mid;
        *(a0_u32x2g*)(p + 2 * IM::PLANE) = s.raw[j].b;
    }
    A0_D static int frag_base(int lane, int woff) { return (woff + (lane & 31)) * IM::PITCH + (lane >> 5) * 16; }
    A0_D static a0_u32x4g frag(const char* plane, int base, int blk, int s) {
        return *(const a0_u32x4g*)(plane + base + blk * 32 * IM::PITCH + s * 32);
    }
};

template <class OA, class OB, int WM, int WN, int MT, int NT, int KS = 2> struct a0_x9_geom {
    static constexpr int BX = WM * MT * 32, BY = WN * NT * 32;
    static constexpr int ABYTES = 3 * a0_x9_image<OA::MODE, BX, KS>::PLANE;
    static constexpr int BBYTES = 3 * a0_x9_image<OB::MODE, BY, KS>::PLANE;
    static constexpr int LDS_BYTES = 2 * (ABYTES + BBYTES);
};

template <class OP> struct a0_x9_plain { static constexpr bool value = false; };
template <> struct a0_x9_plain<OpMatKC> { static constexpr bool value = true; };
template <> struct a0_x9_plain<OpMatXC> { static constexpr bool value = true; };
struct OpPlanesKC;
template <> struct a0_x9_plain<OpPlanesKC> { static constexpr bool value = true; };
template <class EP> struct a0_is_hadamard { static constexpr bool value = false; };
template <> struct a0_is_hadamard<EpiHadamard> { static constexpr bool value = true; };

int a0_x9_products_now();
template <class OA, class OB, class EP, int WM, int WN, int MT, int NT, int KS = 2, int NPR = 9, bool FULL = false>
__device__ __forceinline__ void a0_igemm_x9_body(const typename OA::Params& pa, const typename OB::Params& pb,
                                                 const typename EP::Params& pe, int X, int Y, int K, int kchunk, int gx, int gy) {
    static_assert(WM * WN == 4 || WM * WN == 8, "four or eight waves per workgroup");
    static_assert(KS == 1 || KS == 2, "tiles of 16 or 32 k");
    typedef a0_x9_geom<OA, OB, WM, WN, MT, NT, KS> G;
    constexpr int BK = 16 * KS, BX = G::BX, BY = G::BY, NTH = WM * WN * 64;
    typedef a0_x9_stager<OA, BX, NTH, KS> SA;
    typedef a0_x9_stager<OB, BY, NTH, KS> SB;
    constexpr int APL = a0_x9_image<OA::MODE, BX, KS>::PLANE, BPL = a0_x9_image<OB::MODE, BY, KS>::PLANE;
    constexpr int RA = SA::R, RB = SB::R, NP = RA + RB;
    static_assert(NPR == 9 || NPR == 6, "nine or six cross products");
    constexpr int NG = NPR * KS;
    static_assert(!EP::ROWSUM_A || OA::MODE == A0_XC, "row sums need an x-contiguous A operand");
    extern __shared__ __attribute__((aligned(16))) char a0_x9_lds[];
    char* const As = a0_x9_lds;
    char* const Bs = a0_x9_lds + 2 * G::ABYTES;

    const int tid = threadIdx.x, lane = tid & 63, wave = tid >> 6;
    const int wm = wave / WN, wn = wave % WN;
    int bx, by, bz;
    {
        const int n = gridDim.x, id = blockIdx.x, per = n >> 3;
        const int L = (id < (per << 3)) ? (id & 7) * per + (id >> 3) : id;
        if (gy <= gx) { by = L % gy; const int t = L / gy; bx = t % gx; bz = t / gx; }
        else          { bx = L % gx; const int t = L / gx; by = t % gy; bz = t / gy; }
    }
    const int x0 = bx * BX, y0 = by * BY;
    const int kb = bz * kchunk;
    const int ke = (K < kb + kchunk) ? K : (kb + kchunk);

    SA sa; SB sb;
    sa.init(pa, x0, X, kb, ke, tid);
    sb.init(pb, y0, Y, kb, ke, tid);

    a0_acc16 acc[MT][NT];
#pragma unroll
    for (int i = 0; i < MT; ++i)
#pragma unroll
        for (int j = 0; j < NT; ++j)
#pragma unroll
            for (int r = 0; r < 16; ++r) acc[i][j][r] = 0.f;

    a0_f4 rowsum = a0_zero4();

    auto fetch_piece = [&](typename SA::Slot& s_a, typename SB::Slot& s_b, int p, int k0) {
        if (p < RA) sa.template fetch_piece<FULL>(pa, s_a, p, k0, ke, tid);
        else sb.template fetch_piece<FULL>(pb, s_b, p - RA, k0, ke, tid);
    };
    a0_x9_piece pc;
    auto micro = [&](int u, const typename SA::Slot& s_a_c, const typename SB::Slot& s_b_c, typename SA::Slot& s_a, typename SB::Slot& s_b,
                     char* a_dst, char* b_dst, int k_fetch) {
        const int p = u / 6, st = u % 6;
        if constexpr (SB::PRESPLIT) {
            if (p >= RA) {
                if (st == 5) { sb.store_raw(s_b_c, p - RA, b_dst, tid); fetch_piece(s_a, s_b, p, k_fetch); }
                return;
            }
        }
        if (st == 0) {
            if (p < RA) pc.v = sa.template value<EP::ROWSUM_A, FULL>(s_a_c, p, rowsum);
            else pc.v = sb.template value<false, FULL>(s_b_c, p - RA, rowsum);
        } else if (st <= 4) {
            pc.split(st - 1);
        } else {
            if (p < RA) sa.store(pc, p, a_dst, tid);
            else sb.store(pc, p - RA, b_dst, tid);
            fetch_piece(s_a, s_b, p, k_fetch);
        }
    };

    const int abase = SA::frag_base(lane, wm * (MT * 32));
    const int bbase = SB::frag_base(lane, wn * (NT * 32));

    auto mma_tile = [&](int buf, typename SA::Slot& s_a, typename SB::Slot& s_b, int k_fetch) {
        const char* ap = As + buf * G::ABYTES;
        const char* bp = Bs + buf * G::BBYTES;
        char* a_dst = As + (buf ^ 1) * G::ABYTES;
        char* b_dst = Bs + (buf ^ 1) * G::BBYTES;
        a0_u32x4g a[KS][MT][3], b[KS][NT][3];
#pragma unroll
        for (int s = 0; s < KS; ++s)
#pragma unroll
            for (int t = 2; t >= 0; --t) {
#pragma unroll
                for (int i = 0; i < MT; ++i) a[s][i][t] = SA::frag(ap + t * APL, abase, i, s);
                const int tq = NPR == 6 ? 2 - t : t;
#pragma unroll
                for (int j = 0; j < NT; ++j) b[s][j][tq] = SB::frag(bp + tq * BPL, bbase, j, s);
            }
        __builtin_amdgcn_sched_barrier(0);
        constexpr int NM = NG * MT * NT, NU = 6 * NP;
#pragma unroll
        for (int n = 0; n < NM; ++n) {
            const int g = n / (MT * NT), i = (n / NT) % MT, j = n % NT;
            const int s = g / NPR, q = g % NPR + (9 - NPR);
            constexpr int TA[9] = {2, 2, 1, 2, 1, 0, 1, 0, 0};
            constexpr int TB[9] = {2, 1, 2, 0, 1, 2, 0, 1, 0};
            acc[i][j] = __builtin_amdgcn_mfma_f32_32x32x16_bf16(__builtin_bit_cast(a0_bf16x8g, a[s][i][TA[q]]),
                                                                 __builtin_bit_cast(a0_bf16x8g, b[s][j][TB[q]]), acc[i][j], 0, 0, 0);
#pragma unroll
            for (int u = n * NU / NM; u < (n + 1) * NU / NM; ++u) micro(u, s_a, s_b, s_a, s_b, a_dst, b_dst, k_fetch);
            __builtin_amdgcn_sched_barrier(0);
        }
    };

    typename SA::Slot sa0, sa1;
    typename SB::Slot sb0, sb1;
    sa0.okmask = sa1.okmask = 0u; sb0.okmask = sb1.okmask = 0u;
#pragma unroll
    for (int p = 0; p < NP; ++p) fetch_piece(sa0, sb0, p, kb);
#pragma unroll
    for (int p = 0; p < NP; ++p) fetch_piece(sa1, sb1, p, kb + BK);
#pragma unroll
    for (int u = 0; u < 6 * NP; ++u) micro(u, sa0, sb0, sa0, sb0, As, Bs, kb + 2 * BK);
    __syncthreads();
    for (int k0 = kb; k0 < ke; k0 += 2 * BK) {
        mma_tile(0, sa1, sb1, k0 + 3 * BK);
        __syncthreads();
        if (k0 + BK >= ke) break;
        mma_tile(1, sa0, sb0, k0 + 4 * BK);
        __syncthreads();
    }
    if constexpr (EP::ROWSUM_A) {
        if (by == 0) {
            constexpr int Q = BX / 4;
            a0_f4* red = (a0_f4*)a0_x9_lds;
            red[tid] = rowsum;
            __syncthreads();
            if (tid < BX && x0 + tid < X) {
                const float* rf = (const float*)a0_x9_lds;
                float t = 0.f;
#pragma unroll
                for (int g = 0; g < NTH / Q; ++g) t += rf[4 * (g * Q + (tid >> 2)) + (tid & 3)];
                EP::store_rowsum(pe, x0 + tid, t, bz);
            }
// ... 190 lines not shown
```

### agent0_amd/csrc/net.hip

```cpp
#include "igemm_x9.h"
#include "short_k_fwd.h"
#include "a0_internal.h"
#include "net_impl.h"

#include <vector>

__global__ __launch_bounds__(256) void a0_reduce_slabs_kernel(const float* __restrict__ slabs, long long slab_stride, int nslab,
                                                               float* __restrict__ out, long long count) {
    __shared__ float red[8][33];
    const int c = threadIdx.x & 31, g = threadIdx.x >> 5;
    const long long i = (long long)blockIdx.x * 32 + c;
    float s = 0.f;
    if (i < count)
        for (int z = g; z < nslab; z += 8) s += slabs[(long long)z * slab_stride + i];
    red[g][c] = s;
    __syncthreads();
    if (g == 0 && i < count) {
        float t = 0.f;
#pragma unroll
        for (int j = 0; j < 8; ++j) t += red[j][c];
        out[i] = t;
    }
}

// ... 345 lines not shown
    a0_x9_piece pc;
    pc.v = W[i];
#pragma unroll
    for (int e = 0; e < 4; ++e) pc.split(e);
    a0_u32x2g hi, mid, lo;
    pc.pack(hi, mid, lo);
    a0_u32x2g* o = (a0_u32x2g*)(planes + i * 6);
    o[0] = hi; o[1] = mid; o[2] = lo;
}
extern "C" long long a0_weight_planes_words(int N, int K) { return (long long)N * (K / 4) * 6; }
extern "C" int a0_split_planes(const float* W, unsigned int* planes, int N, int K, void* stream) {
    if (!W || !planes || N < 1 || K < 4 || (K & 3)) return a0_fail(A0_EINVAL, "a0_split_planes: bad argument (K a multiple of 4)");
    const long long groups = (long long)N * (K / 4);
    hipLaunchKernelGGL(a0_split_planes_kernel, dim3((unsigned)((groups + 255) / 256)), dim3(256), 0, (hipStream_t)stream, (const a0_f4*)W, planes, groups);
    return a0_fail_hip((int)hipGetLastError(), "a0_split_planes");
}
extern "C" int a0_dense_fwd_wplanes_ok(int R, int N, int K) {
    return (R >= 2048 && N >= 128 && !(N & 3) && !(K & 31) && a0_fwd_splits((R + 127) / 128, (N + 63) / 64, K) == 1 && g_gemm_x9 != 0) ? 1 : 0;
}
extern "C" int a0_dense_fwd_wplanes(const float* X, int ldx, const unsigned int* Wplanes, const float* b, float* Y, int R, int N, int K, int relu, void* stream) {
    A0_TRY
    if (!X || !Wplanes || !b || !Y || (ldx & 3) || !a0_dense_fwd_wplanes_ok(R, N, K)) return a0_fail(A0_EINVAL, "a0_dense_fwd_wplanes: shapes a0_dense_fwd_wplanes_ok accepts");
    hipStream_t st = (hipStream_t)stream;
    const a0_mat_src a{X, ldx};
    const a0_planes_src bw{Wplanes, K / 4};
    const EpiBiasAct::Params e{Y, b, N, relu};
    hipEvent_t e0 = nullptr, e1 = nullptr;
    const bool probe = a0_probe_events(A0_TAG_DENSE_FWD, &e0, &e1);
    const long long huge = (long long)((R + 255) / 256) * ((N + 127) / 128), big = (long long)((R + 127) / 128) * ((N + 127) / 128);
    const double fill_huge = (double)huge / (256.0 * (double)((huge + 255) / 256)), fill_big = (double)big / (256.0 * (double)((big + 255) / 256));
    if (R >= 256 && huge >= A0_X9_HUGE_TILES && fill_huge >= 0.93 * fill_big) A0_HIP_THROW((a0_igemm_x9_launch<OpMatKC, OpPlanesKC, EpiBiasAct, 4, 2, 2, 2, 1>(st, a, bw, e, R, N, K, 1, e0, e1)));
    else A0_HIP_THROW((a0_igemm_x9_launch<OpMatKC, OpPlanesKC, EpiBiasAct, 4, 2, 1, 2>(st, a, bw, e, R, N, K, 1, e0, e1)));
    if (probe) a0_probe_commit(2.0 * (double)R * (double)N * (double)K);
    return A0_OK;
    A0_CATCH
}

extern "C" int a0_dense_fwd_mul(const float* X, int ldx, const float* W, const float* b, const float* M, int group, float* Y, int R, int N, int K, int relu, void* stream) {
    A0_TRY
    if (!X || !W || !b || !M || !Y || R < 1 || group < 1 || (N & 3) || (K & 3) || (ldx & 3)) return a0_fail(A0_EINVAL, "a0_dense_fwd_mul: bad shape (N, K, ldx must be multiples of 4)");
    if (a0_fwd_splits((R + 127) / 128, (N + 63) / 64, K) != 1) return a0_fail(A0_EINVAL, "a0_dense_fwd_mul: this shape runs as a split GEMM; use a0_dense_fwd + a0_hadamard_fwd");
    a0_hip_backend bk{(hipStream_t)stream};
    bk.tag = A0_TAG_DENSE_FWD;
    if (a0_short_k_shape(R, N, K, ldx)) { bk.short_k_fwd(X, ldx, W, b, M, group, Y, nullptr, R, N, relu); return A0_OK; }
    a0_mat_src a{X, ldx};
    a0_mat_src bw{W, K};
    EpiBiasActMul::Params e{Y, b, N, relu, M, group, a0_udiv_magic((unsigned)group)};
    bk.tag = A0_TAG_DENSE_FWD;
    if (N <= 32) bk.template igemm<OpMatKC, OpMatKC, EpiBiasActMul, 4, 1, 1, 1>(a, bw, e, R, N, K, 1);
    else bk.template igemm<OpMatKC, OpMatKC, EpiBiasActMul, 4, 1, 1, 2>(a, bw, e, R, N, K, 1);
    return A0_OK;
    A0_CATCH
}

extern "C" int a0_dense_fwd_mul_keep_ok(int R, int N, int K, int ldx) { return a0_short_k_shape(R, N, K, ldx) ? 1 : 0; }

extern "C" int a0_dense_fwd_mul_keep(const float* X, int ldx, const float* W, const float* b, const float* M, int group, float* E, float* Y, int R, int N, int K, int relu, void* stream) {
    A0_TRY
    if (!X || !W || !b || !M || !E || !Y || R < 1 || group < 1 || (N & 3)) return a0_fail(A0_EINVAL, "a0_dense_fwd_mul_keep: bad shape");
    if (!a0_short_k_shape(R, N, K, ldx)) return a0_fail(A0_EINVAL, "a0_dense_fwd_mul_keep: not a short-reduction shape (a0_dense_fwd_mul_keep_ok); use a0_dense_fwd + a0_hadamard_fwd");
    a0_hip_backend bk{(hipStream_t)stream};
    bk.tag = A0_TAG_DENSE_FWD;
    bk.short_k_fwd(X, ldx, W, b, M, group, E, Y, R, N, relu);
    return A0_OK;
    A0_CATCH
}

static inline bool a0_fc1_small(int R) { return R <= 256; }
static inline int a0_fc1_splits(int R, int N, int K) {
    const int bx = a0_fc1_small(R) ? 64 : 128, by = 64;
    const int blocks = ((R + bx - 1) / bx) * ((N + by - 1) / by);
    int splits = blocks < 256 ? 256 / blocks : 1;
    const int maxs = (K / 32) / 2;
    if (splits > maxs) splits = maxs;
    if (splits > 64) splits = 64;
    return splits < 1 ? 1 : splits;
}
template <class BK>
static void a0_fc1_partial_launch(BK& bk, const a0_mat_src& a, const a0_mat_src& bw, const EpiSlab::Params& ep, int R, int N, int K, int splits) {
    if (a0_fc1_small(R)) bk.template igemm<OpMatKC, OpMatKC, EpiSlab, 2, 2, 1, 1>(a, bw, ep, R, N, K, splits);
    else bk.template igemm<OpMatKC, OpMatKC, EpiSlab, 4, 2, 1, 1>(a, bw, ep, R, N, K, splits);
}

extern "C" int a0_reduce_bias_act_multi(int n, const float* const* slabs, const long long* slab_stride, const int* nslab, const float* const* bias, float* const* out,
                                       const int* rows, int N, int relu, void* stream) {
    if (n < 1 || n > 4 || !slabs || !slab_stride || !nslab || !bias || !out || !rows || N < 4 || (N & 3)) return a0_fail(A0_EINVAL, "a0_reduce_bias_act_multi: bad argument (1..4 layers, N a multiple of 4)");
    a0_rba_multi_args A;
    A.n = n; A.N = N; A.relu = relu;
    int maxrows = 0;
    for (int i = 0; i < n; ++i) {
        if (!slabs[i] || !bias[i] || !out[i] || rows[i] < 1 || nslab[i] < 1 || (slab_stride[i] & 3) || slab_stride[i] < (long long)rows[i] * N ||
            ((((uintptr_t)slabs[i]) | ((uintptr_t)bias[i]) | ((uintptr_t)out[i])) & 15))
            return a0_fail(A0_EINVAL, "a0_reduce_bias_act_multi: bad layer (16-byte aligned buffers, slab stride a multiple of 4 floats)");
        A.seg[i] = a0_rba_seg{slabs[i], slab_stride[i], nslab[i], bias[i], out[i], rows[i]};
        if (rows[i] > maxrows) maxrows = rows[i];
    }
    for (int i = n; i < 4; ++i) A.seg[i] = A.seg[0];
    hipLaunchKernelGGL(a0_reduce_bias_act_multi_kernel, dim3(a0_grid_for((long long)maxrows * (N >> 2)), n), dim3(256), 0, (hipStream_t)stream, A);
    return a0_fail_hip((int)hipGetLastError(), "a0_reduce_bias_act_multi");
}

extern "C" int a0_dense_fwd_partial_slabs(int R, int N, int K) {
    const int s = N <= 32 ? a0_fwd_splits((R + 127) / 128, (N + 63) / 64, K) : a0_fc1_splits(R, N, K);
    return s < 1 ? 1 : s;
}

extern "C" int a0_dense_fwd_partial(const float* X, int ldx, const float* W, int R, int N, int K, float* slabs, void* stream) {
    A0_TRY
    if (!X || !W || !slabs || R < 1 || (N & 3) || (K & 3) || (ldx & 3)) return a0_fail(A0_EINVAL, "a0_dense_fwd_partial: bad shape (N, K, ldx must be multiples of 4)");
    a0_hip_backend bk{(hipStream_t)stream};
    const int splits = a0_dense_fwd_partial_slabs(R, N, K);
    a0_mat_src a{X, ldx};
    a0_mat_src bw{W, K};
    EpiSlab::Params ep{slabs, (long long)R * N, N};
    bk.tag = A0_TAG_DENSE_FWD;
    if (N <= 32) bk.template igemm<OpMatKC, OpMatKC, EpiSlab, 4, 1, 1, 1>(a, bw, ep, R, N, K, splits);
    else a0_fc1_partial_launch(bk, a, bw, ep, R, N, K, splits);
    return A0_OK;
    A0_CATCH
}

static int a0_fwd_multi_splits(int n, int R, int N, int K) {
    const int blocks = n * ((R + 127) / 128) * ((N + 63) / 64);
    int splits = blocks < 256 ? 256 / blocks : 1;
    const int maxs = (K / 32) / 2;
    if (splits > maxs) splits = maxs;
    return splits < 1 ? 1 : splits;
}
extern "C" int a0_dense_fwd_partial_multi_ok(int n, int R, int N, int K) {
    return (g_gemm_x9 != 0 && (n == 2 || n == 3) && R >= 257 && R <= 4096 && N > 32 && !(N & 3) && !(K & 3)) ? 1 : 0;
}
extern "C" int a0_dense_fwd_partial_multi_slabs(int n, int R, int N, int K) { return a0_fwd_multi_splits(n, R, N, K); }

extern "C" int a0_dense_fwd_partial_multi(int n, const float* const* X, int ldx, const float* const* W, int R, int N, int K, float* const* slabs, const long long* slab_stride,
                                          void* stream) {
    A0_TRY
    if (!X || !W || !slabs || (ldx & 3) || !a0_dense_fwd_partial_multi_ok(n, R, N, K)) return a0_fail(A0_EINVAL, "a0_dense_fwd_partial_multi: shapes a0_dense_fwd_partial_multi_ok accepts");
    a0_x9_group<OpMatKC, OpMatKC, EpiSlab> grp;
    for (int i = 0; i < 3; ++i) {
        const int j = i < n ? i : 0;
        if (!X[j] || !W[j] || !slabs[j]) return a0_fail(A0_EINVAL, "a0_dense_fwd_partial_multi: null operand");
        grp.pa[i] = a0_mat_src{X[j], ldx};
        grp.pb[i] = a0_mat_src{W[j], K};
        const long long stride = slab_stride ? slab_stride[j] : (long long)R * N;
        if (stride < (long long)R * N || (stride & 3)) return a0_fail(A0_EINVAL, "a0_dense_fwd_partial_multi: slab stride");
        grp.pe[i] = EpiSlab::Params{slabs[j], stride, N};
    }
    const int splits = a0_fwd_multi_splits(n, R, N, K);
    hipEvent_t e0 = nullptr, e1 = nullptr;
    const bool probe = a0_probe_events(A0_TAG_DENSE_FWD, &e0, &e1);
    A0_HIP_THROW((a0_igemm_x9_group_launch<OpMatKC, OpMatKC, EpiSlab, 4, 2, 1, 1>((hipStream_t)stream, n, grp, R, N, K, splits, e0, e1)));
    if (probe) a0_probe_commit(2.0 * n * (double)R * (double)N * (double)K);
    return A0_OK;
    A0_CATCH
}

#include "actor_tail.h"
__global__ __launch_bounds__(256) void a0_actor_qhead_kernel(const float* __restrict__ slabs, long long slab_stride, int nslab, const float* __restrict__ b1,
                                                             const float* __restrict__ W2, const float* __restrict__ b2, int A, int dueling, int E,
                                                             unsigned long long seed, uint32_t stream_a, uint32_t stream_u, unsigned long long off_a,
                                                             unsigned long long off_u, float eps, const long long* __restrict__ ctrl,
                                                             const float* __restrict__ eps_ptr, int* __restrict__ action, float* __restrict__ qmax) {
    __shared__ float raw[4][64];
    extern __shared__ float w2s[];
    const int lane = threadIdx.x & 63, wave = threadIdx.x >> 6;
    const int e = blockIdx.x * 4 + wave;
    const int NQ = A + (dueling ? 1 : 0);
    for (int i = threadIdx.x; i < NQ * 128; i += 256) ((a0_f4*)w2s)[i] = ((const a0_f4*)W2)[i];
    __syncthreads();
    if (e >= E) return;
    if (ctrl) { off_a += (unsigned long long)ctrl[A0_CTRL_RNG_ACTION]; off_u += (unsigned long long)ctrl[A0_CTRL_RNG_UNIFORM]; }
    if (eps_ptr) eps = eps_ptr[0];
    int act = 0; float best = 0.f;
    a0_qhead_wave(slabs, slab_stride, nslab, b1, w2s, b2, A, dueling, e, lane, raw[wave], seed, stream_a, stream_u, off_a, off_u, eps, act, best);
    if (lane == 0) { action[e] = act; qmax[e] = best; }
}

__global__ __launch_bounds__(512) void a0_actor_qhead_env_kernel(a0_qenv_args P) {
    __shared__ float raw[64];
    __shared__ int s_chase_cell;
    extern __shared__ float w2s[];
    a0_actor_qhead_env_body(P, raw, w2s, &s_chase_cell);
}

extern "C" long long a0_actor_qhead_scratch(int E, int K) {
    const int splits = a0_fc1_splits(E, 512, K);
    return (long long)splits * E * 512;
}

extern "C" int a0_actor_qhead(const float* feat, int E, int K, const float* W1, const float* b1, const float* W2, const float* b2, int A, int dueling,
                              float* scratch, unsigned long long seed, unsigned int stream_a, unsigned int stream_u, unsigned long long off_a,
                              unsigned long long off_u, float eps, const long long* ctrl, const float* eps_ptr, int* action, float* qmax, void* stream) {
    A0_TRY
    if (!feat || !W1 || !b1 || !W2 || !b2 || !scratch || !action || !qmax || E < 1 || K < 4 || (K & 3) || A < 1 || A + (dueling ? 1 : 0) > 24)
        return a0_fail(A0_EINVAL, "a0_actor_qhead: bad argument (A + dueling <= 24: the head rows are staged in 48 KB of LDS)");
    a0_hip_backend bk{(hipStream_t)stream};
    const int splits = a0_fc1_splits(E, 512, K);
    a0_mat_src a{feat, K};
    a0_mat_src bw{W1, K};
    EpiSlab::Params ep{scratch, (long long)E * 512, 512};
    bk.tag = A0_TAG_DENSE_FWD;
    a0_fc1_partial_launch(bk, a, bw, ep, E, 512, K, splits);
    hipLaunchKernelGGL(a0_actor_qhead_kernel, dim3((E + 3) / 4), dim3(256), (size_t)(A + (dueling ? 1 : 0)) * 512 * sizeof(float), (hipStream_t)stream, scratch, (long long)E * 512, splits, b1, W2, b2, A, dueling, E,
                       seed, stream_a, stream_u, off_a, off_u, eps, ctrl, eps_ptr, action, qmax);
    A0_HIP_THROW(hipGetLastError());
    return A0_OK;
    A0_CATCH
}

extern "C" int a0_actor_qhead_env_step(const float* feat, int E, int K, const float* W1, const float* b1, const float* W2, const float* b2, int A, int dueling,
                                       float* scratch, unsigned long long seed, unsigned int stream_a, unsigned int stream_u, unsigned long long off_a,
                                       unsigned long long off_u, float eps, const long long* ctrl, const float* eps_ptr, int* action, float* qmax,
                                       unsigned long long env_seed, unsigned int rank, unsigned int g, const uint8_t* obs_in, uint8_t* obs_out, float* ep_ret,
                                       float* final_mask, float* final_ret, int n, long long steps, double gamma, int* ring_act, float* ring_rew, float* ring_done,
                                       const uint8_t* obs0, uint8_t* frames, long long cap, long long start_slot, int* r_act, float* r_rew, float* r_done, int task, void* stream) {
    A0_TRY
    if (!feat || !W1 || !b1 || !W2 || !b2 || !scratch || !action || !qmax || E < 1 || K < 4 || (K & 3) || A < 1 || A + (dueling ? 1 : 0) > 24)
        return a0_fail(A0_EINVAL, "a0_actor_qhead_env_step: bad argument (A + dueling <= 24: the head rows are staged in 48 KB of LDS)");
    if (!obs_in || !obs_out || obs_in == obs_out || !ep_ret || !final_mask || !final_ret || !ring_act || !ring_rew || !ring_done || !obs0 || !frames || !r_act ||
        !r_rew || !r_done || n < 1 || steps < 0 || cap < E || start_slot < 0 || task < A0_ENV_TASK_STREAM || task > A0_ENV_TASK_CHASE || (task == A0_ENV_TASK_CHASE && A < 4))
        return a0_fail(A0_EINVAL, "a0_actor_qhead_env_step: bad env argument (the chase task needs at least four actions)");
    if ((((uintptr_t)obs_in) | ((uintptr_t)obs_out) | ((uintptr_t)obs0) | ((uintptr_t)frames)) & 15) return a0_fail(A0_EINVAL, "a0_actor_qhead_env_step: buffers must be 16-byte aligned");
    a0_hip_backend bk{(hipStream_t)stream};
    const int splits = a0_fc1_splits(E, 512, K);
    a0_mat_src a{feat, K};
    a0_mat_src bw{W1, K};
    EpiSlab::Params ep{scratch, (long long)E * 512, 512};
    bk.tag = A0_TAG_DENSE_FWD;
    a0_fc1_partial_launch(bk, a, bw, ep, E, 512, K, splits);
    a0_qenv_args P;
    P.slabs = scratch; P.slab_stride = (long long)E * 512; P.nslab = splits; P.b1 = b1; P.W2 = W2; P.b2 = b2; P.A = A; P.dueling = dueling; P.E = E;
    P.rng_seed = seed; P.stream_a = stream_a; P.stream_u = stream_u; P.off_a = off_a; P.off_u = off_u; P.eps = eps; P.ctrl = ctrl; P.eps_ptr = eps_ptr;
    P.action = action; P.qmax = qmax;
    P.env_seed = env_seed; P.rank = rank; P.g = g; P.obs_in = obs_in; P.obs_out = obs_out; P.ep_ret = ep_ret; P.final_mask = final_mask; P.final_ret = final_ret;
    P.n = n; P.steps = steps; P.gamma = gamma; P.ring_act = ring_act; P.ring_rew = ring_rew; P.ring_done = ring_done; P.obs0 = obs0; P.frames = frames;
    P.cap = cap; P.start = start_slot % cap; P.r_act = r_act; P.r_rew = r_rew; P.r_done = r_done; P.task = task;
    hipLaunchKernelGGL(a0_actor_qhead_env_kernel, dim3(E), dim3(512), (size_t)(A + (dueling ? 1 : 0)) * 512 * sizeof(float), (hipStream_t)stream, P);
    A0_HIP_THROW(hipGetLastError());
    return A0_OK;
    A0_CATCH
}

extern "C" int a0_actor_qhead_env_step_enc(const float* feat, int E, int K, const float* W1, const float* b1, const float* W2, const float* b2, int A, int dueling,
                                           float* scratch, unsigned long long seed, unsigned int stream_a, unsigned int stream_u, unsigned long long off_a,
                                           unsigned long long off_u, float eps, const long long* ctrl, const float* eps_ptr, int* action, float* qmax,
                                           unsigned long long env_seed, unsigned int rank, unsigned int g, const uint8_t* obs_in, uint8_t* obs_out, float* ep_ret,
                                           float* final_mask, float* final_ret, int n, long long steps, double gamma, int* ring_act, float* ring_rew, float* ring_done,
                                           const uint8_t* obs0, uint8_t* frames, long long cap, long long start_slot, int* r_act, float* r_rew, float* r_done, int task,
                                           const float* wt, const a0_encoder_weights* w, float* act3_next, void* stream) {
    A0_TRY
    if (!feat || !W1 || !b1 || !W2 || !b2 || !scratch || !action || !qmax || E < 1 || K != 3136 || A < 1 || A + (dueling ? 1 : 0) > 24)
        return a0_fail(A0_EINVAL, "a0_actor_qhead_env_step_enc: bad argument (4 x 84 x 84 observations, A + dueling <= 24)");
    if (!obs_in || !obs_out || obs_in == obs_out || !ep_ret || !final_mask || !final_ret || !ring_act || !ring_rew || !ring_done || !obs0 || !frames || !r_act ||
        !r_rew || !r_done || n < 1 || steps < 0 || cap < E || start_slot < 0 || task < A0_ENV_TASK_STREAM || task > A0_ENV_TASK_CHASE || (task == A0_ENV_TASK_CHASE && A < 4))
        return a0_fail(A0_EINVAL, "a0_actor_qhead_env_step_enc: bad env argument");
    if ((((uintptr_t)obs_in) | ((uintptr_t)obs_out) | ((uintptr_t)obs0) | ((uintptr_t)frames)) & 15) return a0_fail(A0_EINVAL, "a0_actor_qhead_env_step_enc: buffers must be 16-byte aligned");
    a0_hip_backend bk{(hipStream_t)stream};
    const int splits = a0_fc1_splits(E, 512, K);
    a0_mat_src a{feat, K};
    a0_mat_src bw{W1, K};
    EpiSlab::Params ep{scratch, (long long)E * 512, 512};
    bk.tag = A0_TAG_DENSE_FWD;
    a0_fc1_partial_launch(bk, a, bw, ep, E, 512, K, splits);
    a0_qenv_args P;
    P.slabs = scratch; P.slab_stride = (long long)E * 512; P.nslab = splits; P.b1 = b1; P.W2 = W2; P.b2 = b2; P.A = A; P.dueling = dueling; P.E = E;
    P.rng_seed = seed; P.stream_a = stream_a; P.stream_u = stream_u; P.off_a = off_a; P.off_u = off_u; P.eps = eps; P.ctrl = ctrl; P.eps_ptr = eps_ptr;
    P.action = action; P.qmax = qmax;
    P.env_seed = env_seed; P.rank = rank; P.g = g; P.obs_in = obs_in; P.obs_out = obs_out; P.ep_ret = ep_ret; P.final_mask = final_mask; P.final_ret = final_ret;
    P.n = n; P.steps = steps; P.gamma = gamma; P.ring_act = ring_act; P.ring_rew = ring_rew; P.ring_done = ring_done; P.obs0 = obs0; P.frames = frames;
    P.cap = cap; P.start = start_slot % cap; P.r_act = r_act; P.r_rew = r_rew; P.r_done = r_done; P.task = task;
    return a0_actor_step_enc_launch(P, wt, w, act3_next, (hipStream_t)stream);
    A0_CATCH
}

__global__ __launch_bounds__(256) void a0_mean_rows_kernel(const float* __restrict__ x, int E, float* __restrict__ out) {
    __shared__ float red[256];
    const float* p = x + (long long)blockIdx.x * E;
    float s = 0.f;
    for (int e = threadIdx.x; e < E; e += 256) s += p[e];
    red[threadIdx.x] = s;
    __syncthreads();
    for (int o = 128; o > 0; o >>= 1) { if ((int)threadIdx.x < o) red[threadIdx.x] += red[threadIdx.x + o]; __syncthreads(); }
    if (threadIdx.x == 0) out[blockIdx.x] = red[0] / (float)E;
}

extern "C" int a0_mean_rows(const float* x, int T, int E, float* out, void* stream) {
    if (!x || !out || T < 1 || E < 1) return a0_fail(A0_EINVAL, "a0_mean_rows: bad argument");
    hipLaunchKernelGGL(a0_mean_rows_kernel, dim3(T), dim3(256), 0, (hipStream_t)stream, x, E, out);
    return a0_fail_hip((int)hipGetLastError(), "a0_mean_rows");
}

extern "C" int a0_dense_dgrad(const float* dY, const float* W, const float* act_mask, float* dX, int R, int N, int K, void* stream) {
    A0_TRY
    if (!dY || !W || !dX || R < 1 || (N & 3) || (K & 3)) return a0_fail(A0_EINVAL, "a0_dense_dgrad: bad shape");
    a0_hip_backend bk{(hipStream_t)stream};
    a0_dense_dgrad_impl(bk, dY, W, act_mask, dX, R, N, K);
    return A0_OK;
    A0_CATCH
}

extern "C" int a0_dense_dgrad_hadamard_ok(int R, int N, int K, int n) {
    return (g_gemm_x9 != 0 && (n == 32 || n == 64) && R >= 4096 && !(R & 255) && !(R % n) && !(N & 15) && N >= 64 && !(K & 3) && K >= 128) ? 1 : 0;
}
extern "C" int a0_dense_dgrad_hadamard(const float* dY, const float* W, const float* emb, const float* feat, float* demb, float* d3, int R, int N, int K, int n, void* stream) {
    A0_TRY
    if (!dY || !W || !emb || !feat || !demb || !d3 || !a0_dense_dgrad_hadamard_ok(R, N, K, n)) return a0_fail(A0_EINVAL, "a0_dense_dgrad_hadamard: shapes a0_dense_dgrad_hadamard_ok accepts");
    const a0_mat_src a{dY, N};
    const a0_mat_src bw{W, K};
    const EpiHadamard::Params e{emb, feat, demb, d3, K, n};
    hipEvent_t e0 = nullptr, e1 = nullptr;
    const bool probe = a0_probe_events(A0_TAG_DENSE_DGRAD, &e0, &e1);
    A0_HIP_THROW((a0_igemm_x9_launch<OpMatKC, OpMatXC, EpiHadamard, 4, 2, 2, 2, 1>((hipStream_t)stream, a, bw, e, R, K, N, 1, e0, e1)));
    if (probe) a0_probe_commit(2.0 * (double)R * (double)N * (double)K);
    return A0_OK;
    A0_CATCH
}

extern "C" int a0_dense_dgrad_wgrad_ok(int R, int N, int K) {
    const long long b128 = (long long)((R + 127) / 128) * ((K + 63) / 64), b64 = (long long)((N + 63) / 64) * ((K + 63) / 64);
    return (g_gemm_x9 != 0 && g_probe.tag == 0 && R == N && R >= 1 && R <= 1024 && !(N & 3) && !(K & 3) && b128 < 256 && b64 >= 256 && N >= 512 &&
            (long long)((R + 127) / 128) * ((K + 127) / 128) < A0_X9_BIG_TILES) ? 1 : 0;
}
static int a0_dense_dgrad_wgrad_small_ok(int R, int N, int K) {
    const long long t1 = (long long)((R + 63) / 64) * ((K + 63) / 64), t2 = (long long)((N + 63) / 64) * ((K + 63) / 64);
    return (g_gemm_x9 != 0 && g_probe.tag == 0 && R >= 64 && R <= 1024 && N >= 64 && !(N & 3) && !(K & 3) && t1 + t2 <= 256 && t2 >= 16) ? 1 : 0;
}
extern "C" int a0_dense_dgrad_wgrad_ok2(int R, int N, int K) { return (a0_dense_dgrad_wgrad_ok(R, N, K) || a0_dense_dgrad_wgrad_small_ok(R, N, K)) ? 1 : 0; }
extern "C" int a0_dense_dgrad_wgrad(const float* dY, const float* W, const float* X, int ldx, float* dX, float* grad, int R, int N, int K, void* stream) {
    A0_TRY
    if (!dY || !W || !X || !dX || !grad || ldx < K || (ldx & 3) || !a0_dense_dgrad_wgrad_ok2(R, N, K)) return a0_fail(A0_EINVAL, "a0_dense_dgrad_wgrad: shapes a0_dense_dgrad_wgrad_ok2 accepts");
    a0_mat_src a1{dY, N}, b1{W, K};
    EpiMaskMat::Params e1{dX, X, K};
    a0_mat_src a2{dY, N}, b2{X, ldx};
    EpiWgradSlab::Params e2{grad, 0, K, (long long)N * K};
    if (!a0_dense_dgrad_wgrad_ok(R, N, K)) {
        A0_HIP_THROW((a0_igemm_x9_pair_launch<OpMatKC, OpMatXC, EpiMaskMat, OpMatXC, OpMatXC, EpiWgradSlab, 2, 2, 1, 1>((hipStream_t)stream, a1, b1, e1, R, K, N, a2, b2, e2, N, K, R)));
        return A0_OK;
    }
    A0_HIP_THROW((a0_igemm_x9_pair_launch<OpMatKC, OpMatXC, EpiMaskMat, OpMatXC, OpMatXC, EpiWgradSlab, 4, 2, 1, 1>((hipStream_t)stream, a1, b1, e1, R, K, N, a2, b2, e2, N, K, R)));
    return A0_OK;
    A0_CATCH
}

extern "C" int a0_dense_dgrad_wgrad2_ok(int R, int N, int K, int N2, int K2) {
    return (a0_dense_dgrad_wgrad_ok(R, N, K) && N2 >= 4 && !(N2 & 3) && K2 >= 4 && !(K2 & 3) &&
            (long long)((N2 + 127) / 128) * ((K2 + 63) / 64) <= 8) ? 1 : 0;
}
extern "C" int a0_dense_dgrad_wgrad2(const float* dY, const float* W, const float* X, int ldx, float* dX, float* grad, int R, int N, int K,
                                     const float* dY2, const float* X2, int ldx2, float* grad2, int N2, int K2, void* stream) {
    A0_TRY
    if (!dY || !W || !X || !dX || !grad || ldx < K || (ldx & 3) || !a0_dense_dgrad_wgrad_ok(R, N, K)) return a0_fail(A0_EINVAL, "a0_dense_dgrad_wgrad2: shapes a0_dense_dgrad_wgrad_ok accepts");
    if (!dY2 || !X2 || !grad2 || N2 < 4 || (N2 & 3) || K2 < 4 || (K2 & 3) || ldx2 < K2 || (ldx2 & 3) ||
        (long long)((N2 + 127) / 128) * ((K2 + 63) / 64) > (long long)((R + 127) / 128) * ((K + 63) / 64))
        return a0_fail(A0_EINVAL, "a0_dense_dgrad_wgrad2: the second layer's weight gradient must have no more 128 x 64 tiles than the first layer's data gradient");
// ... 73 lines not shown
```

### agent0_amd/csrc/runtime.hip

```cpp
#include "learner_state.h"

namespace {

typedef a0_host_rng Rng;
constexpr int STREAM_EGREEDY_U = 1, STREAM_EGREEDY_A = 2, STREAM_SUMTREE = 5, STREAM_PERM = 6;

struct Owned {
    std::vector<void*> ptrs;
    template <class T> T* alloc(long long n, bool zero = true) {
        void* p = nullptr;
        A0_HIP_THROW(hipMalloc(&p, (size_t)(n > 0 ? n : 1) * sizeof(T)));
        ptrs.push_back(p);
        if (zero) A0_HIP_THROW(hipMemset(p, 0, (size_t)(n > 0 ? n : 1) * sizeof(T)));
        return (T*)p;
    }
    ~Owned() { for (void* p : ptrs) (void)hipFree(p); }
};

__global__ void a0_pow_scalar_kernel(const float* __restrict__ p, double alpha, float* __restrict__ out) {
    const double x = (double)p[0];
    out[0] = (float)(alpha == 0.5 ? sqrt(x) : pow(x, alpha));
}
__global__ void a0_fill_one_kernel(float* __restrict__ p, long long n, float v) {
    const long long i = (long long)blockIdx.x * blockDim.x + threadIdx.x;
// ... 161 lines not shown
    if (!R->ep.open || R->ep.pos + 1 >= R->ep.nb) {
        R->ep.top = R->top; R->ep.nb = (R->top + B - 1) / B; R->ep.pos = 0; R->ep.seed = R->rng.next_seed32(STREAM_PERM); R->ep.open = true;
        if (R->ep.nb < 2) { R->ep.open = false; return a0_fail(A0_EINVAL, "a0_rbuf_sample: the ring holds fewer than two batches (the reference's fetcher cannot return one either)"); }
    }
    const long long start = R->ep.pos * B;
    R->ep.pos += 1;
    A0_CHECK(a0_replay_sample_slots((unsigned long long)start, (unsigned long long)R->ep.top, R->ep.seed, R->top, R->head(), R->size, R->act, R->rew, R->done, R->flat ? R->prio_vec : nullptr, B,
                                    R->b_idx, R->b_slot, R->b_act, R->b_rew, R->b_done, R->b_prio, stream));
    if (R->flat) {
        A0_CHECK(a0_sum_f32(R->prio_vec, R->size, R->sum_scratch, R->psum, stream));
        A0_CHECK(a0_is_weights(R->b_prio, B, R->psum, R->top, (float)R->beta_use, R->b_w, stream));
    }
    *out = a0_batch{R->b_idx, R->b_slot, R->b_act, R->b_rew, R->b_done, R->b_prio, R->flat ? R->b_w : R->ones};
    return A0_OK;
    A0_CATCH
}

extern "C" int a0_rbuf_sample_block(a0_rbuf* R, int n, a0_batch* out, void* stream) {
    A0_TRY
    a0_trace_scope range("sample");
    if (!R || !out || n < 1 || n > 32) return a0_fail(A0_EINVAL, "a0_rbuf_sample_block: 1..32 batches");
    if (R->prio) return a0_fail(A0_EINVAL, "a0_rbuf_sample_block: prioritized batches depend on the update before them (a0_rbuf_sample)");
    const int B = R->B;
    unsigned long long start[32], n_perm[32];
    unsigned int seed[32];
    for (int g = 0; g < n; ++g) {
        if (!R->ep.open || R->ep.pos + 1 >= R->ep.nb) {
            R->ep.top = R->top; R->ep.nb = (R->top + B - 1) / B; R->ep.pos = 0; R->ep.seed = R->rng.next_seed32(STREAM_PERM); R->ep.open = true;
            if (R->ep.nb < 2) { R->ep.open = false; return a0_fail(A0_EINVAL, "a0_rbuf_sample_block: the ring holds fewer than two batches"); }
        }
        start[g] = (unsigned long long)(R->ep.pos * B); n_perm[g] = (unsigned long long)R->ep.top; seed[g] = R->ep.seed;
        R->ep.pos += 1;
    }
    A0_CHECK(a0_replay_sample_slots_multi(n, start, n_perm, seed, R->top, R->head(), R->size, R->act, R->rew, R->done, B, R->m_idx, R->m_slot, R->m_act, R->m_rew, R->m_done,
                                          R->m_prio, stream));
    for (int g = 0; g < n; ++g) {
        const long long o = (long long)g * B;
        out[g] = a0_batch{R->m_idx + o, R->m_slot + o, R->m_act + o, R->m_rew + o, R->m_done + o, R->m_prio + o, R->ones};
    }
    return A0_OK;
    A0_CATCH
}

extern "C" int a0_rbuf_update_priority(a0_rbuf* R, const float* loss, const int* learner_state, void* stream) {
    A0_TRY
    if (!R || !loss) return a0_fail(A0_EINVAL, "a0_rbuf_update_priority: null argument");
    if (!R->prio) return A0_OK;
    if (R->flat) return a0_priority_update(R->prio_vec, R->b_idx, loss, R->B, (float)R->d.eps, (float)R->d.alpha, R->pstate, learner_state, stream);
    if (a0_sumtree_set_from_loss_ok(R->cap2)) {
        R->top_stale = true;
        return a0_sumtree_set_from_loss(R->tree, R->cap2, R->b_idx, loss, R->B, (float)R->d.eps, (float)R->d.alpha, R->pstate, learner_state, 1, stream);
    }
    A0_CHECK(a0_priority_from_loss(loss, R->B, (float)R->d.eps, (float)R->d.alpha, R->b_prio, R->pstate, learner_state, stream));
    return a0_sumtree_set(R->tree, R->cap2, R->b_idx, R->b_prio, R->B, learner_state, stream);
    A0_CATCH
}

struct a0_actor {
    a0_actor_desc d;
    int E = 0, T = 0, n = 1, K = 2, cur = 0, feat = 3136, obs_bytes = 4 * 84 * 84;
    unsigned g = 0;
    long long steps = 0;
    Rng rng;
    Owned mem;
    std::vector<uint8_t*> obs;
    float *ep_ret = nullptr, *qmax_all = nullptr, *stat_mask = nullptr, *stat_ret = nullptr, *qs = nullptr, *ring_rew = nullptr, *ring_done = nullptr, *act3 = nullptr, *scratch = nullptr;
    int *action = nullptr, *ring_act = nullptr;
    std::vector<float> h_mask, h_ret;
    float *p_mask = nullptr, *p_ret = nullptr, *p_qs = nullptr;
    hipEvent_t stats_ev = nullptr;
    ~a0_actor() {
        if (p_mask) (void)hipHostFree(p_mask);
        if (p_ret) (void)hipHostFree(p_ret);
        if (p_qs) (void)hipHostFree(p_qs);
        if (stats_ev) (void)hipEventDestroy(stats_ev);
    }
    float *h = nullptr, *head_slabs = nullptr, *fwd_scratch = nullptr;
    int dist_Npad = 0;
    float *q_taus = nullptr, *q_cosx = nullptr, *q_x = nullptr;
    float *f_logits = nullptr, *f_tau_all = nullptr;
    bool bound = false;
    float *own_flat = nullptr, *own_wt = nullptr, *own_eff = nullptr, *own_noise = nullptr;
    unsigned int* w_planes = nullptr;
};

struct a0_actor_net {
    const float* flat; const float* wt; float* eff; float* noise;
    const a0_learner* L;
    const float* Wf() const { return L->d.noisy ? eff + L->eff_fc1.w() : flat + L->fc1.w(); }
    const float* bf() const { return L->d.noisy ? eff + L->eff_fc1.b() : flat + L->fc1.b(); }
    const float* Wh() const { return L->d.noisy ? eff + L->eff_head.w() : flat + L->head.w(); }
    const float* bh() const { return L->d.noisy ? eff + L->eff_head.b() : flat + L->head.b(); }
};
static a0_actor_net a0_actor_view(const a0_actor* a, a0_learner* L) {
    if (a->own_flat) return a0_actor_net{a->own_flat, a->own_wt, a->own_eff, a->own_noise, L};
    return a0_actor_net{L->online, L->wt_on, L->eff_on, L->noise, L};
}

extern "C" int a0_actor_bind(a0_actor* a, const a0_learner* L, int own_network) {
    A0_TRY
    if (!a || !L) return a0_fail(A0_EINVAL, "a0_actor_bind: null argument");
    if (L->d.A != a->d.A || (L->d.dueling != 0) != (a->d.dueling != 0)) return a0_fail(A0_EINVAL, "a0_actor_bind: actor and learner were created for different heads");
    const int E = a->E;
    const bool dist = L->d.algo == A0_ALGO_C51 || L->d.algo == A0_ALGO_QR, fqf = L->d.algo == A0_ALGO_FQF, quant = L->d.algo == A0_ALGO_IQN || fqf;
    if (a->bound && a->dist_Npad != L->Npad) return a0_fail(A0_EINVAL, "a0_actor_bind: this actor was sized for another head");
    if (!a->bound) {
        const int nt = fqf ? L->F : (quant ? L->d.iqn_K : 1);
        if (quant) {
            const long long R = (long long)E * nt;
            if (a0_dense_fwd_scratch((int)R, L->feat, 64) != 0) return a0_fail(A0_EINVAL, "a0_actor_bind: E * K rows too few for the embedding kernel this path takes");
            a->h = a->mem.alloc<float>(R * 512);
            a->head_slabs = a->mem.alloc<float>((long long)a0_dense_fwd_partial_slabs((int)R, L->Npad, 512) * R * L->Npad);
            long long sc = a0_dense_fwd_scratch((int)R, 512, L->feat);
            if (fqf && a0_dense_fwd_scratch(E, 32, L->feat) > sc) sc = a0_dense_fwd_scratch(E, 32, L->feat);
            a->fwd_scratch = a->mem.alloc<float>(sc > 4 ? sc : 4);
            a->q_taus = a->mem.alloc<float>(ceil_to(R, 4)); a->q_cosx = a->mem.alloc<float>(R * 64); a->q_x = a->mem.alloc<float>(R * L->feat);
            if (fqf) { a->f_logits = a->mem.alloc<float>((long long)E * 32); a->f_tau_all = a->mem.alloc<float>((long long)E * (nt + 1)); }
            if (a0_dense_fwd_wplanes_ok((int)R, 512, L->feat)) a->w_planes = a->mem.alloc<unsigned int>(a0_weight_planes_words(512, L->feat), false);
        } else if (dist) {
            a->h = a->mem.alloc<float>((long long)E * 512);
            a->head_slabs = a->mem.alloc<float>((long long)a0_dense_fwd_partial_slabs(E, L->Npad, 512) * E * L->Npad);
            const long long sc = a0_dense_fwd_scratch(E, 512, L->feat);
            a->fwd_scratch = a->mem.alloc<float>(sc > 4 ? sc : 4);
        }
        a->dist_Npad = L->Npad;
        a->bound = true;
    }
    if (own_network && !a->own_flat) {
        a->own_flat = a->mem.alloc<float>(L->n_pad); a->own_wt = a->mem.alloc<float>(L->wt_floats);
        if (L->d.noisy) { a->own_eff = a->mem.alloc<float>(L->n_eff); a->own_noise = a->mem.alloc<float>(L->noise_len); }
    }
    A0_HIP_THROW(hipDeviceSynchronize());
    return A0_OK;
    A0_CATCH
}

extern "C" int a0_actor_snapshot(a0_actor* a, const a0_learner* L, void* stream) {
    A0_TRY
    if (!a || !L || !a->own_flat) return a0_fail(A0_EINVAL, "a0_actor_snapshot: an actor bound with its own network (a0_actor_bind(actor, learner, 1))");
    hipStream_t st = (hipStream_t)stream;
    A0_HIP_THROW(hipMemcpyAsync(a->own_flat, L->online, (size_t)L->n_pad * 4, hipMemcpyDeviceToDevice, st));
    A0_HIP_THROW(hipMemcpyAsync(a->own_wt, L->wt_on, (size_t)L->wt_floats * 4, hipMemcpyDeviceToDevice, st));
    if (L->d.noisy) {
        A0_HIP_THROW(hipMemcpyAsync(a->own_eff, L->eff_on, (size_t)L->n_eff * 4, hipMemcpyDeviceToDevice, st));
        A0_HIP_THROW(hipMemcpyAsync(a->own_noise, L->noise, (size_t)L->noise_len * 4, hipMemcpyDeviceToDevice, st));
    }
    return A0_OK;
    A0_CATCH
}

extern "C" int a0_actor_create(const a0_actor_desc* d, a0_actor** out) {
    A0_TRY
    if (!d || !out) return a0_fail(A0_EINVAL, "a0_actor_create: null argument");
    if (d->E < 1 || d->T < 1 || d->A < 1 || d->n_step < 1 || d->reset_noise_freq < 0 || !(d->discount > 0.0) || d->env_task < A0_ENV_TASK_STREAM || d->env_task > A0_ENV_TASK_CHASE || (d->env_task == A0_ENV_TASK_CHASE && d->A < 4))
        return a0_fail(A0_EINVAL, "a0_actor_create: bad description");
    a0_actor* a = new a0_actor();
    try {
        a->d = *d; a->E = d->E; a->T = d->T; a->n = d->n_step;
        a->rng.init(d->seed, d->rank);
        a->K = 2;
        if (a->n > 1) {
            a->K = a->n + 1;
            for (int r = a->n + 1; r < 2 * a->n + 3; ++r) if (a->T % r == 0) { a->K = r; break; }
        }
        const long long E = a->E, T = a->T;
        for (int i = 0; i < a->K; ++i) a->obs.push_back(a->mem.alloc<uint8_t>(E * a->obs_bytes));
        a->ep_ret = a->mem.alloc<float>(E); a->qmax_all = a->mem.alloc<float>(T * E); a->stat_mask = a->mem.alloc<float>(T * E); a->stat_ret = a->mem.alloc<float>(T * E);
        a->qs = a->mem.alloc<float>(T); a->action = a->mem.alloc<int>(E);
        a->ring_act = a->mem.alloc<int>((long long)a->n * E); a->ring_rew = a->mem.alloc<float>((long long)a->n * E); a->ring_done = a->mem.alloc<float>((long long)a->n * E);
        a->act3 = a->mem.alloc<float>(E * a->feat); a->scratch = a->mem.alloc<float>(a0_actor_qhead_scratch(a->E, a->feat));
        a->h_mask.resize((size_t)(T * E)); a->h_ret.resize((size_t)(T * E));
        if (a0_env_synth_reset_task(d->seed, d->rank, a->E, a->obs[0], a->ep_ret, d->env_task, nullptr) != A0_OK) { delete a; return A0_EINVAL; }
        A0_HIP_THROW(hipDeviceSynchronize());
    } catch (...) { delete a; throw; }
    *out = a;
    return A0_OK;
    A0_CATCH
}

extern "C" int a0_actor_destroy(a0_actor* a) { delete a; return A0_OK; }

static int a0_actor_compose(const a0_actor_net& V, void* stream) {
    const a0_learner* L = V.L;
    const float *mu[3], *sg[3], *nin[3], *nw[3], *nb[3];
    float* eff[3];
    int N[3], K[3], r0[3], r1[3];
    for (int k = 0; k < L->n_mods; ++k) {
        const a0_noise_mod& m = L->mods[k];
        const Blk &bm = m.block ? L->head : L->fc1, &bs = m.block ? L->head_sigma : L->fc1_sigma, &be = m.block ? L->eff_head : L->eff_fc1;
        mu[k] = V.flat + bm.off; sg[k] = V.flat + bs.off; eff[k] = V.eff + be.off; N[k] = bm.N; K[k] = bm.K; r0[k] = m.r0; r1[k] = m.r1;
        nin[k] = V.noise + m.off_in; nw[k] = V.noise + m.off_w; nb[k] = V.noise + m.off_b;
    }
    return a0_noisy_multi(0, L->n_mods, mu, sg, eff, N, K, r0, r1, nin, nw, nb, stream);
}

extern "C" int a0_actor_rollout(a0_actor* a, a0_learner* L, a0_rbuf* R, float epsilon, void* stream) {
    A0_TRY
    a0_trace_scope range("rollout");
    if (!a || !L || !R) return a0_fail(A0_EINVAL, "a0_actor_rollout: null argument");
    if (L->d.A != a->d.A || (L->d.dueling != 0) != (a->d.dueling != 0) || R->obs_bytes != a->obs_bytes || R->size < a->E)
        return a0_fail(A0_EINVAL, "a0_actor_rollout: actor, learner and replay were created for different shapes");
    const int E = a->E, A = a->d.A;
    const bool dist = L->d.algo == A0_ALGO_C51 || L->d.algo == A0_ALGO_QR, fqf = L->d.algo == A0_ALGO_FQF, quant = L->d.algo == A0_ALGO_IQN || fqf;
    const int freq = a->d.reset_noise_freq > 0 ? a->d.reset_noise_freq : 4;
    const int nt = fqf ? L->F : (quant ? L->d.iqn_K : 1);
    if (!a->bound || a->dist_Npad != L->Npad) A0_CHECK(a0_actor_bind(a, L, 0));
    const a0_actor_net V = a0_actor_view(a, L);
    const long long start = R->written % R->size;
    a0_encoder_weights w = L->enc(V.flat);
    if (L->d.noisy && a->steps % freq != 0) A0_CHECK(a0_actor_compose(V, stream));
    const bool planes = quant && a->w_planes && a0_dense_fwd_wplanes_ok(E * nt, 512, L->feat);
    if (planes && !(L->d.noisy && a->steps % freq == 0)) A0_CHECK(a0_split_planes(V.Wf(), a->w_planes, 512, L->feat, stream));
    const bool step_enc = !a->own_flat;
    bool feat_ready = false;
    for (int t = 0; t < a->T; ++t) {
        if (L->d.noisy && a->steps % freq == 0) {
            A0_CHECK(a0_rng_normal(a->rng.seed, 4 , a->rng.reserve(4, L->noise_len), 0.1f, V.noise, L->noise_len, stream));
            A0_CHECK(a0_actor_compose(V, stream));
            if (planes) A0_CHECK(a0_split_planes(V.Wf(), a->w_planes, 512, L->feat, stream));
        }
        const uint8_t* cur_obs = a->obs[a->cur];
        a0_frames_arg f{cur_obs, nullptr, (long long)a->obs_bytes, 0};
        if (!feat_ready) A0_CHECK(a0_net_encoder_fwd_fused(L->C, L->H, L->W, V.wt, &w, &f, E, nullptr, nullptr, a->act3, stream));
        feat_ready = false;
        const long long back = (a->steps + 1 < a->n ? a->steps + 1 : a->n) - 1;
        const uint8_t* obs0 = a->obs[((a->cur - back) % a->K + a->K) % a->K];
        if (quant) {
            const int rows = E * nt;
            const float* on = V.flat;
            if (fqf) {
                A0_CHECK(a0_dense_fwd(a->act3, L->feat, on + L->frac.w(), on + L->frac.b(), a->f_logits, E, 32, L->feat, 0, a->fwd_scratch, stream));
                A0_CHECK(a0_fqf_taus_cos(a->f_logits, 32, a->f_tau_all, a->q_taus, a->q_cosx, 64, E, nt, stream));
            } else {
                A0_CHECK(a0_tau_cos_features(a->rng.seed, 3 , a->rng.reserve(3, rows), nullptr, 0, a->q_taus, a->q_cosx, rows, 64, stream));
            }
            A0_CHECK(a0_dense_fwd_mul(a->q_cosx, 64, on + L->cos.w(), on + L->cos.b(), a->act3, nt, a->q_x, rows, L->feat, 64, 1, stream));
            if (planes) A0_CHECK(a0_dense_fwd_wplanes(a->q_x, L->feat, a->w_planes, V.bf(), a->h, rows, 512, L->feat, 1, stream));
            else A0_CHECK(a0_dense_fwd(a->q_x, L->feat, V.Wf(), V.bf(), a->h, rows, 512, L->feat, 1, a->fwd_scratch, stream));
            const int ns = a0_dense_fwd_partial_slabs(rows, L->Npad, 512);
            A0_CHECK(a0_dense_fwd_partial(a->h, 512, V.Wh(), rows, L->Npad, 512, a->head_slabs, stream));
            const unsigned long long oa = a->rng.reserve(STREAM_EGREEDY_A, E), ou = a->rng.reserve(STREAM_EGREEDY_U, E);
            const int nx = (a->cur + 1) % a->K;
            a->g += 1;
            if (step_enc && t + 1 < a->T) {
                A0_CHECK(a0_actor_quantile_tail_env_step_enc(a->head_slabs, (long long)rows * L->Npad, ns, V.bh(), L->Npad, A, nt, a->d.dueling ? 1 : 0, fqf ? 3 : 1, fqf ? a->f_tau_all : nullptr, E, a->rng.seed,
                                                             STREAM_EGREEDY_A, STREAM_EGREEDY_U, oa, ou, epsilon, nullptr, nullptr, a->action, a->qmax_all + (long long)t * E, a->d.seed,
                                                             a->d.rank, a->g, cur_obs, a->obs[nx], a->ep_ret, a->stat_mask + (long long)t * E, a->stat_ret + (long long)t * E, a->n, a->steps,
                                                             a->d.discount, a->ring_act, a->ring_rew, a->ring_done, obs0, R->frames, R->size, (start + (long long)t * E) % R->size, R->act,
                                                             R->rew, R->done, a->d.env_task, V.wt, &w, a->act3, stream));
                feat_ready = true;
            } else
            A0_CHECK(a0_actor_quantile_tail_env_step(a->head_slabs, (long long)rows * L->Npad, ns, V.bh(), L->Npad, A, nt, a->d.dueling ? 1 : 0, fqf ? 3 : 1, fqf ? a->f_tau_all : nullptr, E, a->rng.seed,
                                                     STREAM_EGREEDY_A, STREAM_EGREEDY_U, oa, ou, epsilon, nullptr, nullptr, a->action, a->qmax_all + (long long)t * E, a->d.seed,
                                                     a->d.rank, a->g, cur_obs, a->obs[nx], a->ep_ret, a->stat_mask + (long long)t * E, a->stat_ret + (long long)t * E, a->n, a->steps,
                                                     a->d.discount, a->ring_act, a->ring_rew, a->ring_done, obs0, R->frames, R->size, (start + (long long)t * E) % R->size, R->act,
                                                     R->rew, R->done, a->d.env_task, stream));
            a->cur = nx;
            a->steps += 1;
            continue;
        }
        if (dist) {
            A0_CHECK(a0_dense_fwd(a->act3, L->feat, V.Wf(), V.bf(), a->h, E, 512, L->feat, 1, a->fwd_scratch, stream));
            const int ns = a0_dense_fwd_partial_slabs(E, L->Npad, 512);
            A0_CHECK(a0_dense_fwd_partial(a->h, 512, V.Wh(), E, L->Npad, 512, a->head_slabs, stream));
            const unsigned long long oa = a->rng.reserve(STREAM_EGREEDY_A, E), ou = a->rng.reserve(STREAM_EGREEDY_U, E);
            const int nx = (a->cur + 1) % a->K;
            a->g += 1;
            if (4LL * ((long long)A * L->T + L->T) * 4 > 160 * 1024) return a0_fail(A0_EINVAL, "a0_actor_rollout: head too wide for the distributional tail kernel");
            if (step_enc && t + 1 < a->T) {
                A0_CHECK(a0_actor_dist_tail_env_step_enc(a->head_slabs, (long long)E * L->Npad, ns, V.bh(), L->Npad, A, L->T, a->d.dueling ? 1 : 0, L->d.algo == A0_ALGO_C51 ? 2 : 1,
                                                         L->d.algo == A0_ALGO_C51 ? L->atoms : nullptr, E, a->rng.seed,
                                                         STREAM_EGREEDY_A, STREAM_EGREEDY_U, oa, ou, epsilon, nullptr, nullptr, a->action, a->qmax_all + (long long)t * E, a->d.seed, a->d.rank,
                                                         a->g, cur_obs, a->obs[nx], a->ep_ret, a->stat_mask + (long long)t * E, a->stat_ret + (long long)t * E, a->n, a->steps, a->d.discount,
                                                         a->ring_act, a->ring_rew, a->ring_done, obs0, R->frames, R->size, (start + (long long)t * E) % R->size, R->act, R->rew, R->done,
                                                         a->d.env_task, V.wt, &w, a->act3, stream));
                feat_ready = true;
            } else
            A0_CHECK(a0_actor_dist_tail_env_step(a->head_slabs, (long long)E * L->Npad, ns, V.bh(), L->Npad, A, L->T, a->d.dueling ? 1 : 0, L->d.algo == A0_ALGO_C51 ? 2 : 1,
                                                 L->d.algo == A0_ALGO_C51 ? L->atoms : nullptr, E, a->rng.seed,
                                                 STREAM_EGREEDY_A, STREAM_EGREEDY_U, oa, ou, epsilon, nullptr, nullptr, a->action, a->qmax_all + (long long)t * E, a->d.seed, a->d.rank,
                                                 a->g, cur_obs, a->obs[nx], a->ep_ret, a->stat_mask + (long long)t * E, a->stat_ret + (long long)t * E, a->n, a->steps, a->d.discount,
                                                 a->ring_act, a->ring_rew, a->ring_done, obs0, R->frames, R->size, (start + (long long)t * E) % R->size, R->act, R->rew, R->done,
                                                 a->d.env_task, stream));
            a->cur = nx;
            a->steps += 1;
            continue;
        }
        if (A + (a->d.dueling ? 1 : 0) > 24) return a0_fail(A0_EINVAL, "a0_actor_rollout: scalar heads with A + dueling <= 24 actions");
        const unsigned long long off_a = a->rng.reserve(STREAM_EGREEDY_A, E), off_u = a->rng.reserve(STREAM_EGREEDY_U, E);
        const int nxt = (a->cur + 1) % a->K;
        a->g += 1;
        if (step_enc && t + 1 < a->T) {
            A0_CHECK(a0_actor_qhead_env_step_enc(a->act3, E, a->feat, V.Wf(), V.bf(), V.Wh(), V.bh(), A, a->d.dueling ? 1 : 0,
                                                 a->scratch, a->rng.seed, STREAM_EGREEDY_A, STREAM_EGREEDY_U, off_a, off_u, epsilon, nullptr, nullptr, a->action, a->qmax_all + (long long)t * E,
                                                 a->d.seed, a->d.rank, a->g, cur_obs, a->obs[nxt], a->ep_ret, a->stat_mask + (long long)t * E, a->stat_ret + (long long)t * E, a->n, a->steps,
                                                 a->d.discount, a->ring_act, a->ring_rew, a->ring_done, obs0, R->frames, R->size, (start + (long long)t * E) % R->size, R->act, R->rew, R->done,
                                                 a->d.env_task, V.wt, &w, a->act3, stream));
            feat_ready = true;
        } else
        A0_CHECK(a0_actor_qhead_env_step(a->act3, E, a->feat, V.Wf(), V.bf(), V.Wh(), V.bh(), A, a->d.dueling ? 1 : 0,
                                         a->scratch, a->rng.seed, STREAM_EGREEDY_A, STREAM_EGREEDY_U, off_a, off_u, epsilon, nullptr, nullptr, a->action, a->qmax_all + (long long)t * E,
                                         a->d.seed, a->d.rank, a->g, cur_obs, a->obs[nxt], a->ep_ret, a->stat_mask + (long long)t * E, a->stat_ret + (long long)t * E, a->n, a->steps,
                                         a->d.discount, a->ring_act, a->ring_rew, a->ring_done, obs0, R->frames, R->size, (start + (long long)t * E) % R->size, R->act, R->rew, R->done,
                                         a->d.env_task, stream));
        a->cur = nxt;
        a->steps += 1;
    }
    return a0_mean_rows(a->qmax_all, a->T, E, a->qs, stream);
    A0_CATCH
}

extern "C" int a0_actor_collect(a0_actor* a, float* qs_host, float* returns_host, int max_returns, int* n_returns, void* stream) {
    A0_TRY
    if (!a) return a0_fail(A0_EINVAL, "a0_actor_collect: null handle");
    hipStream_t st = (hipStream_t)stream;
    const size_t n = (size_t)a->T * a->E;
    if (qs_host) A0_HIP_THROW(hipMemcpyAsync(qs_host, a->qs, (size_t)a->T * 4, hipMemcpyDeviceToHost, st));
    A0_HIP_THROW(hipMemcpyAsync(a->h_mask.data(), a->stat_mask, n * 4, hipMemcpyDeviceToHost, st));
    A0_HIP_THROW(hipMemcpyAsync(a->h_ret.data(), a->stat_ret, n * 4, hipMemcpyDeviceToHost, st));
    A0_HIP_THROW(hipStreamSynchronize(st));
    int k = 0;
    for (size_t i = 0; i < n; ++i)
        if (a->h_mask[i] != 0.f) { if (returns_host && k < max_returns) returns_host[k] = a->h_ret[i]; ++k; }
    if (n_returns) *n_returns = k;
    return A0_OK;
    A0_CATCH
}

extern "C" int a0_actor_collect_begin(a0_actor* a, void* stream) {
    A0_TRY
    if (!a) return a0_fail(A0_EINVAL, "a0_actor_collect_begin: null handle");
    hipStream_t st = (hipStream_t)stream;
    const size_t n = (size_t)a->T * a->E;
    if (!a->p_mask) {
        A0_HIP_THROW(hipHostMalloc((void**)&a->p_mask, n * 4, hipHostMallocDefault));
        A0_HIP_THROW(hipHostMalloc((void**)&a->p_ret, n * 4, hipHostMallocDefault));
        A0_HIP_THROW(hipHostMalloc((void**)&a->p_qs, (size_t)a->T * 4, hipHostMallocDefault));
        A0_HIP_THROW(hipEventCreateWithFlags(&a->stats_ev, hipEventDisableTiming));
    }
    A0_HIP_THROW(hipMemcpyAsync(a->p_qs, a->qs, (size_t)a->T * 4, hipMemcpyDeviceToHost, st));
    A0_HIP_THROW(hipMemcpyAsync(a->p_mask, a->stat_mask, n * 4, hipMemcpyDeviceToHost, st));
    A0_HIP_THROW(hipMemcpyAsync(a->p_ret, a->stat_ret, n * 4, hipMemcpyDeviceToHost, st));
    A0_HIP_THROW(hipEventRecord(a->stats_ev, st));
    return A0_OK;
    A0_CATCH
}

extern "C" int a0_actor_collect_end(a0_actor* a, float* qs_host, float* returns_host, int max_returns, int* n_returns) {
    A0_TRY
    if (!a || !a->stats_ev) return a0_fail(A0_EINVAL, "a0_actor_collect_end: no a0_actor_collect_begin before it");
    A0_HIP_THROW(hipEventSynchronize(a->stats_ev));
    const size_t n = (size_t)a->T * a->E;
    if (qs_host) for (int t = 0; t < a->T; ++t) qs_host[t] = a->p_qs[t];
    int k = 0;
    for (size_t i = 0; i < n; ++i)
        if (a->p_mask[i] != 0.f) { if (returns_host && k < max_returns) returns_host[k] = a->p_ret[i]; ++k; }
    if (n_returns) *n_returns = k;
    return A0_OK;
    A0_CATCH
}
```

### include/agent0_hip.h

```cpp
#ifndef AGENT0_HIP_H
#define AGENT0_HIP_H

#include <stdint.h>

#ifdef __cplusplus
extern "C" {
#endif

#define A0_ABI_VERSION 1

#define A0_CTRL_ENV_STEP 0
#define A0_CTRL_ACTOR_STEPS 1
#define A0_CTRL_RNG_ACTION 2
#define A0_CTRL_RNG_UNIFORM 3
#define A0_CTRL_REPLAY_SLOT 4
#define A0_CTRL_RNG_TAUS 5
#define A0_CTRL_RNG_NOISE 6
#define A0_CTRL_WORDS 8

const char* a0_last_error(void);
int a0_abi_version(void);
const char* a0_build_info(void);
int a0_device_info(int* cu_count, long long* hbm_bytes, char* arch_name64);

// ... 171 lines not shown
                      void* stream);
int a0_adam_step_sync_wt(float* params, const float* grads, float* exp_avg, float* exp_avg_sq, long long n, int* state, float* scalars2, double lr,
                         double beta1, double beta2, double eps, int target_update_freq, float* target, long long n_total, const float* extra_nan_flag,
                         const a0_encoder_weights* w, int C, float* wt, float* wt_target, const float* loss, int loss_n, float* loss_ring, int ring_cap, void* stream);
#define A0_ALGO_DQN 0
#define A0_ALGO_C51 1
#define A0_ALGO_QR 4
#define A0_ALGO_MDQN 5
#define A0_ALGO_FQF 3
#define A0_ALGO_IQN 2
typedef struct a0_learner a0_learner;
typedef struct a0_learner_desc {
    int A, dueling, double_q;
    int B, n_step;
    double discount, lr, adam_eps;
    int target_update_freq;
    int algo;
    int num_atoms; double vmin, vmax;
    int noisy;
    unsigned long long seed;
    int iqn_K, iqn_N, iqn_N_dash;
    int fqf_F;
    double mdqn_tau, mdqn_lo;
    double max_grad_norm;
} a0_learner_desc;
int a0_learner_create(const a0_learner_desc* desc, a0_learner** out);
typedef struct a0_learner_buffers {
    float *online, *target, *grads, *adam_m, *adam_v;
    int* state;
    float* scalars;
    float* loss_ring; int loss_ring_cap;
    float *wt_online, *wt_target;
    float *eff_online, *eff_target, *noise;
    float* rms_sq;
} a0_learner_buffers;
int a0_learner_create_on(const a0_learner_desc* desc, const a0_learner_buffers* buffers, a0_learner** out);
int a0_learner_set_rng(a0_learner* learner, int stream_id, unsigned long long offset);
int a0_learner_destroy(a0_learner* learner);
long long a0_learner_param_floats(const a0_learner* learner);
int a0_learner_set_exchange(a0_learner* learner, long long comm);
int a0_learner_set_params(a0_learner* learner, const float* online_packed, const float* target_packed, void* stream);
int a0_learner_get(const a0_learner* learner, float* online_out, float* target_out, float* adam_m_out, float* adam_v_out, int* state_out8, void* stream);
int a0_learner_loss_buffer(const a0_learner* learner, float** loss_dev);
enum { A0_PEEK_GRADS = 0, A0_PEEK_ACT1 = 1, A0_PEEK_ACT2 = 2, A0_PEEK_ACT3 = 3, A0_PEEK_FC1 = 4, A0_PEEK_LOSS = 5 };
int a0_learner_peek(const a0_learner* learner, int what, float** dev_ptr, long long* count);
int a0_learner_get_frac_loss(const a0_learner* learner, float* out_dev, void* stream);
int a0_learner_set_support(a0_learner* learner, const float* atoms_host);
int a0_learner_update(a0_learner* learner, const uint8_t* frames, const int* slot, long long row_bytes, const int* act, const float* rew, const float* done,
                      const float* wgt, float* loss_out, void* stream);

typedef struct a0_rbuf a0_rbuf;
typedef struct a0_rbuf_desc {
    long long size; int obs_bytes, B, prioritize;
    double alpha, eps, beta0; long long total_steps;
    unsigned long long seed;
} a0_rbuf_desc;
typedef struct a0_batch { const long long* idx; const int* slot; const int* act; const float* rew; const float* done; const float* prio; const float* weights; } a0_batch;
int a0_rbuf_create(const a0_rbuf_desc* desc, a0_rbuf** out);
int a0_rbuf_create_on(const a0_rbuf_desc* desc, uint8_t* frames, int* act, float* rew, float* done, float* tree, float* max_p, a0_rbuf** out);
int a0_rbuf_destroy(a0_rbuf* replay);
long long a0_rbuf_len(const a0_rbuf* replay);
long long a0_rbuf_write_cursor(const a0_rbuf* replay);
int a0_rbuf_info(const a0_rbuf* replay, long long* top, long long* written, double* beta);
int a0_rbuf_buffers(a0_rbuf* replay, uint8_t** frames, int** act, float** rew, float** done, float** tree, float** max_p);
int a0_rbuf_read(const a0_rbuf* replay, long long rows, uint8_t* frames_out, int* act_out, float* rew_out, float* done_out, float* tree_out, float* max_p_out, void* stream);
int a0_rbuf_commit(a0_rbuf* replay, long long n, void* stream);
int a0_rbuf_extend_from(a0_rbuf* replay, const a0_rbuf* stage, long long start_row, long long n, void* stream);
int a0_rbuf_sample(a0_rbuf* replay, a0_batch* out, void* stream);
int a0_rbuf_sample_block(a0_rbuf* replay, int n, a0_batch* out, void* stream);
int a0_rbuf_update_priority(a0_rbuf* replay, const float* loss, const int* learner_state, void* stream);

typedef struct a0_actor a0_actor;
typedef struct a0_actor_desc {
    int E, T, A, dueling, n_step;
    double discount;
    unsigned long long seed; unsigned int rank;
    int env_task;
    int reset_noise_freq;
} a0_actor_desc;
int a0_actor_create(const a0_actor_desc* desc, a0_actor** out);
int a0_actor_destroy(a0_actor* actor);
int a0_actor_bind(a0_actor* actor, const a0_learner* learner, int own_network);
int a0_actor_snapshot(a0_actor* actor, const a0_learner* learner, void* stream);
int a0_actor_rollout(a0_actor* actor, a0_learner* learner, a0_rbuf* replay, float epsilon, void* stream);
int a0_actor_collect(a0_actor* actor, float* qs_host, float* returns_host, int max_returns, int* n_returns, void* stream);
int a0_actor_collect_begin(a0_actor* actor, void* stream);
int a0_actor_collect_end(a0_actor* actor, float* qs_host, float* returns_host, int max_returns, int* n_returns);

int a0_nan_flag_export(const int* state, float* out, void* stream);
int a0_rmsprop_step(float* params, const float* grads, float* square_avg, long long n, double lr, double alpha, double eps,
                    double max_grad_norm, float* clip_scratch, void* stream);
int a0_target_sync(float* target, const float* online, long long n, const int* state, int force, void* stream);
int a0_noisy_compose(const float* mu, const float* sigma, float* eff, int N, int K, int r0, int r1, const float* noise_in,
                     const float* noise_out_w, const float* noise_out_b, void* stream);
int a0_noisy_grad_sigma(const float* gmu, float* gsigma, int N, int K, int r0, int r1, const float* noise_in,
                        const float* noise_out_w, const float* noise_out_b, void* stream);
int a0_noisy_multi(int grad, int nmod, const float* const* mu, const float* const* sigma, float* const* eff, const int* N, const int* K, const int* r0,
                   const int* r1, const float* const* noise_in, const float* const* noise_out_w, const float* const* noise_out_b, void* stream);

int a0_replay_insert(uint8_t* frames, long long cap, int obs_bytes, long long start_slot, int n, const uint8_t* obs,
                     const uint8_t* obs_next, const int* act, const float* rew, const float* done, int* r_act,
                     float* r_rew, float* r_done, const long long* ctrl, void* stream);
int a0_replay_lookup(const long long* idx, int B, long long top, long long head, long long cap, int* slot, const int* r_act,
                     const float* r_rew, const float* r_done, const float* priority, int* act, float* rew, float* done,
                     float* prio, long long* idx_out, void* stream);
int a0_replay_gather(const uint8_t* frames, int row_bytes, const int* slot, int B, uint8_t* out, void* stream);
int a0_replay_sample_gather(int mode, unsigned long long start, unsigned long long n_perm, unsigned int seed, const float* tree, long long cap2,
                            const float* xi, long long top, long long head, long long cap, const uint8_t* frames, int row_bytes, const int* r_act,
                            const float* r_rew, const float* r_done, const float* priority, int B, uint8_t* out, long long* idx_out, int* slot_out,
                            int* act, float* rew, float* done, float* prio, void* stream);
int a0_replay_sample_slots(unsigned long long start, unsigned long long n_perm, unsigned int seed, long long top, long long head, long long cap,
                           const int* r_act, const float* r_rew, const float* r_done, const float* priority, int B, long long* idx_out, int* slot_out,
                           int* act, float* rew, float* done, float* prio, void* stream);
int a0_replay_sample_slots_multi(int n, const unsigned long long* start, const unsigned long long* n_perm, const unsigned int* seed, long long top, long long head, long long cap,
                                 const int* r_act, const float* r_rew, const float* r_done, int B, long long* idx_out, int* slot_out, int* act, float* rew, float* done,
                                 float* prio, void* stream);
int a0_fill_f32(float* p, long long n, float v, void* stream);
int a0_priority_update(float* priority, const long long* ids, const float* loss, int B, float eps, float alpha,
                       float* pstate, const int* state, void* stream);
int a0_priority_tail(float* priority, long long size, long long n, const float* pstate, float alpha, void* stream);
int a0_sum_f32(const float* x, long long n, float* scratch256, float* out, void* stream);
int a0_is_weights(const float* prio, int B, const float* psum, long long top, float beta, float* w, void* stream);
int a0_perm_batch(unsigned long long start, int count, unsigned long long n, unsigned int seed, long long* out, void* stream);
int a0_sumtree_set(float* tree, long long cap2, const long long* idx, const float* val, int n, const int* state, void* stream);
int a0_sumtree_set_range(float* tree, long long cap2, long long start, long long n, long long size, const float* val, void* stream);
int a0_sumtree_rebuild(float* tree, long long cap2, void* stream);
int a0_sumtree_sample(const float* tree, long long cap2, const float* xi, int B, long long* out_idx, float* out_p, void* stream);
int a0_sumtree_sample_batch(unsigned long long seed, unsigned int stream, unsigned long long offset, float* tree, long long cap2, int B, long long top,
                            long long cap, float beta, const int* r_act, const float* r_rew, const float* r_done, long long* idx_out, int* slot_out,
                            int* act, float* rew, float* done, float* prio, float* w, int rebuild_top, void* stream_h);
int a0_priority_from_loss(const float* loss, int n, float eps, float alpha, float* val, float* pstate, const int* state, void* stream);
int a0_sumtree_set_from_loss_ok(long long cap2);
int a0_sumtree_set_from_loss(float* tree, long long cap2, const long long* idx, const float* loss, int n, float eps, float alpha, float* pstate, const int* state,
                             int defer_top, void* stream);
int a0_sumtree_top_rebuild(float* tree, long long cap2, void* stream);

int a0_actor_egreedy(const int* greedy, const int* rand_action, const float* u, float eps, int E, int* action,
                     const float* qmax, float* qs_out, void* stream);
long long a0_actor_qhead_scratch(int E, int K);
int a0_actor_qhead(const float* feat, int E, int K, const float* W1, const float* b1, const float* W2, const float* b2, int A, int dueling,
                   float* scratch, unsigned long long seed, unsigned int stream_a, unsigned int stream_u, unsigned long long off_a,
                   unsigned long long off_u, float eps, const long long* ctrl, const float* eps_ptr, int* action, float* qmax, void* stream);
int a0_actor_qhead_env_step(const float* feat, int E, int K, const float* W1, const float* b1, const float* W2, const float* b2, int A, int dueling,
                            float* scratch, unsigned long long seed, unsigned int stream_a, unsigned int stream_u, unsigned long long off_a,
                            unsigned long long off_u, float eps, const long long* ctrl, const float* eps_ptr, int* action, float* qmax,
                            unsigned long long env_seed, unsigned int rank, unsigned int g, const uint8_t* obs_in, uint8_t* obs_out, float* ep_ret,
                            float* final_mask, float* final_ret, int n, long long steps, double gamma, int* ring_act, float* ring_rew, float* ring_done,
                            const uint8_t* obs0, uint8_t* frames, long long cap, long long start_slot, int* r_act, float* r_rew, float* r_done, int task, void* stream);
int a0_mean_rows(const float* x, int T, int E, float* out, void* stream);

int a0_actor_qhead_env_step_enc(const float* feat, int E, int K, const float* W1, const float* b1, const float* W2, const float* b2, int A, int dueling,
                                float* scratch, unsigned long long seed, unsigned int stream_a, unsigned int stream_u, unsigned long long off_a,
                                unsigned long long off_u, float eps, const long long* ctrl, const float* eps_ptr, int* action, float* qmax,
                                unsigned long long env_seed, unsigned int rank, unsigned int g, const uint8_t* obs_in, uint8_t* obs_out, float* ep_ret,
                                float* final_mask, float* final_ret, int n, long long steps, double gamma, int* ring_act, float* ring_rew, float* ring_done,
                                const uint8_t* obs0, uint8_t* frames, long long cap, long long start_slot, int* r_act, float* r_rew, float* r_done, int task,
                                const float* wt, const a0_encoder_weights* w, float* act3_next, void* stream);
int a0_actor_dist_tail_env_step_enc(const float* slabs, long long slab_stride, int nslab, const float* bias, int ld, int A, int T, int dueling, int mode,
                                    const float* atoms, int E, unsigned long long seed, unsigned int stream_a, unsigned int stream_u, unsigned long long off_a,
                                    unsigned long long off_u, float eps, const long long* ctrl, const float* eps_ptr, int* action, float* qmax,
                                    unsigned long long env_seed, unsigned int rank, unsigned int g, const uint8_t* obs_in, uint8_t* obs_out, float* ep_ret,
                                    float* final_mask, float* final_ret, int n, long long steps, double gamma, int* ring_act, float* ring_rew, float* ring_done,
                                    const uint8_t* obs0, uint8_t* frames, long long cap, long long start_slot, int* r_act, float* r_rew, float* r_done, int task,
                                    const float* wt, const a0_encoder_weights* w, float* act3_next, void* stream);
int a0_actor_quantile_tail_env_step_enc(const float* slabs, long long slab_stride, int nslab, const float* bias, int ld, int A, int T, int dueling, int mode,
                                        const float* taus, int E, unsigned long long seed, unsigned int stream_a, unsigned int stream_u, unsigned long long off_a,
// ... 53 lines not shown
```

Before: 2.323 million.

## Emit encoder features as pre-split operand planes for the actor fc1 GEMM

The encoder's final conv epilogue can now write act3 directly as hi/mid/lo split planes instead of fp32. The actor fc1 GEMM then consumes those planes together with pre-split weight planes, which removes a separate split pass over the features on each step. New PL template variants are added to the fused encoder and to the step-encode kernels. The path is on by default for non-noisy, non-distributional actors with 84x84x4 inputs, and it costs extra plane buffers plus more kernel instantiations.

```diff
diff --git a/agent0_amd/csrc/a0_internal.h b/agent0_amd/csrc/a0_internal.h
--- a/agent0_amd/csrc/a0_internal.h
+++ b/agent0_amd/csrc/a0_internal.h
@@ -61,6 +61,24 @@
 int a0_conv23_wgrad_fused_launch(const a0_net_core& n, int B, const float* act1, const float* act2, const float* d2, const float* d3, float* slab2, float* slab3,
                                  hipStream_t st);
 #endif
+int a0_net_encoder_fwd_fused_planes(int C, int H, int W, const float* wt, const a0_encoder_weights* w, const a0_frames_arg* f, int B,
+                                    float* act1, float* act2, float* act3, uint32_t* act3p, void* stream);
+int a0_fc1_planes_ok(int R, int K);
+int a0_actor_qhead_env_step_planes(const float* feat, int E, int K, const float* W1, const float* b1, const float* W2, const float* b2, int A, int dueling,
+                                   float* scratch, unsigned long long seed, unsigned int stream_a, unsigned int stream_u, unsigned long long off_a,
+                                   unsigned long long off_u, float eps, const long long* ctrl, const float* eps_ptr, int* action, float* qmax,
+                                   unsigned long long env_seed, unsigned int rank, unsigned int g, const uint8_t* obs_in, uint8_t* obs_out, float* ep_ret,
+                                   float* final_mask, float* final_ret, int n, long long steps, double gamma, int* ring_act, float* ring_rew, float* ring_done,
+                                   const uint8_t* obs0, uint8_t* frames, long long cap, long long start_slot, int* r_act, float* r_rew, float* r_done, int task,
+                                   const uint32_t* feat_planes, const uint32_t* w_planes, void* stream);
+int a0_actor_qhead_env_step_enc_planes(const float* feat, int E, int K, const float* W1, const float* b1, const float* W2, const float* b2, int A, int dueling,
+                                       float* scratch, unsigned long long seed, unsigned int stream_a, unsigned int stream_u, unsigned long long off_a,
+                                       unsigned long long off_u, float eps, const long long* ctrl, const float* eps_ptr, int* action, float* qmax,
+                                       unsigned long long env_seed, unsigned int rank, unsigned int g, const uint8_t* obs_in, uint8_t* obs_out, float* ep_ret,
+                                       float* final_mask, float* final_ret, int n, long long steps, double gamma, int* ring_act, float* ring_rew, float* ring_done,
+                                       const uint8_t* obs0, uint8_t* frames, long long cap, long long start_slot, int* r_act, float* r_rew, float* r_done, int task,
+                                       const float* wt, const a0_encoder_weights* w, float* act3_next, const uint32_t* feat_planes, const uint32_t* w_planes,
+                                       uint32_t* act3p_next, void* stream);
 #define A0_TAG_ENCODER_FUSED 12
 #define A0_TAG_ENCODER_DGRAD_FUSED 13
 #define A0_TAG_ACTOR_STEP_ENC 14
diff --git a/agent0_amd/csrc/actor_tail.h b/agent0_amd/csrc/actor_tail.h
--- a/agent0_amd/csrc/actor_tail.h
+++ b/agent0_amd/csrc/actor_tail.h
@@ -301,5 +301,5 @@
 
 
 struct a0_encoder_weights;
-int a0_actor_step_enc_launch(const a0_qenv_args& Q, const float* wt, const a0_encoder_weights* w, float* act3, hipStream_t st);
+int a0_actor_step_enc_launch(const a0_qenv_args& Q, const float* wt, const a0_encoder_weights* w, float* act3, uint32_t* act3p, hipStream_t st);
 int a0_actor_dist_step_enc_launch(const a0_dtenv_args& Q, size_t tail_lds, const float* wt, const a0_encoder_weights* w, float* act3, hipStream_t st);
diff --git a/agent0_amd/csrc/encoder_fused.hip b/agent0_amd/csrc/encoder_fused.hip
--- a/agent0_amd/csrc/encoder_fused.hip
+++ b/agent0_amd/csrc/encoder_fused.hip
@@ -16,6 +16,7 @@
     const float *wx2, *wx3;
     const float *b1, *b2, *b3;
     float *act1, *act2, *act3;
+    uint32_t* act3p = nullptr;
     int B;
     int C, H, W, H1, W1, H2, W2, H3, W3;
     int off_act1, off_act2, off_end;
@@ -407,18 +408,28 @@
         *(uint2*)d = hi; *(uint2*)(d + term) = mid; *(uint2*)(d + 2 * term) = lo;
     }
 };
+template <bool PL = false>
 struct EpiFwdT {
     static constexpr bool PER_ELEM = false;
     static constexpr bool ROW4 = false;
     static constexpr bool TR = true;
     const float* bias; float* glb; int N;
+    uint32_t* planes;
     A0_D float pre_col(int) const { return 0.f; }
     A0_D void emit_n4(int m, int n0, const a0_acc4& acc, const float*) const {
         const a0_f4 bv = *(const a0_f4*)(bias + n0);
         float v[4] = {acc[0] + bv.x, acc[1] + bv.y, acc[2] + bv.z, acc[3] + bv.w};
 #pragma unroll
         for (int r = 0; r < 4; ++r) v[r] = (v[r] < 0.f) ? 0.f : v[r];
-        *(a0_f4*)(glb + (unsigned)(m * N + n0)) = a0_f4{v[0], v[1], v[2], v[3]};
+        if constexpr (PL) {
+            uint2 hi, mid, lo;
+            a0_split4(v, hi, mid, lo);
+            uint32_t* d = planes + 6u * ((unsigned)(m * N + n0) >> 2);
+            *(uint4*)d = uint4{hi.x, hi.y, mid.x, mid.y};
+            *(uint2*)(d + 4) = lo;
+        } else {
+            *(a0_f4*)(glb + (unsigned)(m * N + n0)) = a0_f4{v[0], v[1], v[2], v[3]};
+        }
     }
 };
 
@@ -637,7 +648,7 @@
 #ifndef A0_FUSED_MINWAVES
 #define A0_FUSED_MINWAVES 1
 #endif
-template <int MBW1, int MBW2, int MBW3, int WC, bool X9, bool LOOP = false, int ORD = 4>
+template <int MBW1, int MBW2, int MBW3, int WC, bool X9, bool LOOP = false, int ORD = 4, bool PL = false>
 __global__ __launch_bounds__(A0_FUSED_THREADS, A0_FUSED_MINWAVES) void a0_encoder_fused_kernel(a0_fused_args P);
 
 constexpr int A0_X9_BIAS_OFF = 2 * 4 * 84 * 84 + 3 * 20 * A0_RP1X * 2;
@@ -660,7 +671,7 @@
 typedef a0_wring9<64, A0_WNX, A0_RX2> a0_ring2_t;
 typedef a0_wring9<64, A0_WNX, A0_RX3> a0_ring3_t;
 #endif
-template <int ORD, int MBW2, int MBW3, bool LOOP>
+template <int ORD, int MBW2, int MBW3, bool LOOP, bool PL = false>
 A0_D void a0_x9_conv23(const a0_fused_args& P, int b, unsigned char* smem, float* bias_lds, a0_wring1<A0_R1>& ring1, a0_ring2_t& ring2, a0_ring3_t& ring3) {
     const int obs_bytes = P.C * P.H * P.W;
     const int M2 = P.H2 * P.W2, M3 = P.H3 * P.W3;
@@ -673,7 +684,7 @@
     static_assert(MBW2X <= MBW2 * 2 && MBW3X <= MBW3 * 2, "84x84 geometry");
 #if !A0_KSPLIT
     a0_pre<64, WNX, MBW2X, E2X> pre2;
-    a0_pre<64, WNX, MBW3X, EpiFwdT> pre3;
+    a0_pre<64, WNX, MBW3X, EpiFwdT<PL>> pre3;
 #endif
     (void)a1p; (void)term1;
     {
@@ -681,7 +692,7 @@
         const E2X e2{bias_lds + 32, a2p, P.act2 ? P.act2 + (long long)b * M2 * 64 : nullptr, 64};
 #if A0_KSPLIT
         const AF3X<term2> f3k{a2p, A0_RP2X, P.W3, A0_P2X};
-        const EpiFwdT e3k{bias_lds + 96, P.act3 + (long long)b * M3 * 64, 64};
+        const EpiFwdT<PL> e3k{bias_lds + 96, PL ? nullptr : P.act3 + (long long)b * M3 * 64, 64, PL ? P.act3p + (long long)b * M3 * 96 : nullptr};
         a0_conv_stage_x9k<ORD, 64, 4, 6, A0_RK2, 1>(f2, M2, ring2, e2, (float*)(smem + A0_X9_XCH0), (float*)(smem + A0_X9_XCH1), [&] { ring3.prologue(); });
         a0_conv_stage_x9k<ORD, 64, 4, 4, A0_RK3, 16>(f3k, M3, ring3, e3k, (float*)a1p, (float*)a1p + 4 * 2 * 256, [&] { if (LOOP) ring1.prologue(); });
 #else
@@ -692,7 +703,7 @@
         else
             a0_conv_stage_x9<ORD, 64, WNX, MBW2X, A0_RX2>(f2, M2, ring2, e2, pre2, [&] { ring3.prologue(); });
         const AF3X<term2> f3{a2p, A0_RP2X, P.W3, A0_P2X};
-        const EpiFwdT e3{bias_lds + 96, P.act3 + (long long)b * M3 * 64, 64};
+        const EpiFwdT<PL> e3{bias_lds + 96, PL ? nullptr : P.act3 + (long long)b * M3 * 64, 64, PL ? P.act3p + (long long)b * M3 * 96 : nullptr};
         if (uneven3 && wmgx + (MBW3X - 1) * WMGX >= 4)
             a0_conv_stage_x9<ORD, 64, WNX, (MBW3X > 1 ? MBW3X - 1 : 1), A0_RX3>(f3, M3, ring3, e3, pre3, [&] { if (LOOP) ring1.prologue(); });
         else
@@ -701,7 +712,7 @@
     }
 }
 
-template <int ORD, int MBW1, int MBW2, int MBW3, bool LOOP>
+template <int ORD, int MBW1, int MBW2, int MBW3, bool LOOP, bool PL = false>
 A0_D void a0_encoder_fused_x9_body(const a0_fused_args& P, int bid, int nblk) {
     extern __shared__ __attribute__((aligned(16))) unsigned char smem[];
     uint16_t* img = (uint16_t*)smem;
@@ -764,13 +775,13 @@
             a0_conv1_stage<(MBW1X > 1 ? MBW1X - 1 : 1), A0_R1, 84>(img, P.H * P.W, P.W, P.W1, M1, ring1, e1, pre1, [&] { ring2.prologue(); });
         else
             a0_conv1_stage<MBW1X, A0_R1, 84>(img, P.H * P.W, P.W, P.W1, M1, ring1, e1, pre1, [&] { ring2.prologue(); });
-        a0_x9_conv23<ORD, MBW2, MBW3, LOOP>(P, b, smem, bias_lds, ring1, ring2, ring3);
+        a0_x9_conv23<ORD, MBW2, MBW3, LOOP, PL>(P, b, smem, bias_lds, ring1, ring2, ring3);
         if constexpr (!LOOP) break;
     }
 }
 
 #include "actor_tail.h"
-struct a0_step_enc_args { const float *wt, *b1, *b2, *b3; float* act3; };
+struct a0_step_enc_args { const float *wt, *b1, *b2, *b3; float* act3; uint32_t* act3p; };
 template <int ORD>
 __global__ __launch_bounds__(A0_FUSED_THREADS, A0_FUSED_MINWAVES) void a0_actor_dist_step_enc_kernel(a0_dtenv_args Q, a0_step_enc_args N) {
     __shared__ int s_chase_cell;
@@ -908,7 +919,7 @@
         }
     }
 };
-template <int ORD, class TAIL>
+template <int ORD, class TAIL, bool PL>
 A0_D void a0_actor_step_enc2_body(const typename TAIL::Args& Q, const a0_step_enc_args& N) {
     __shared__ float raw[64];
     __shared__ int s_chase_cell;
@@ -954,7 +965,7 @@
     uint4* out16 = (uint4*)(Q.obs_out + (size_t)e * 4 * HW) + j;
     uint4* row16 = (uint4*)(Q.frames + slot * (8LL * HW)) + j;
     A0_TO_VGPR(out16); A0_TO_VGPR(row16);
-    float* act3_v = N.act3;
+    unsigned long long act3_v = PL ? (unsigned long long)N.act3p : (unsigned long long)N.act3;
     A0_TO_VGPR(act3_v);
     auto new_group = [&](uint32_t by, uint32_t bx) {
         uint32_t w[4];
@@ -1038,12 +1049,13 @@
         a0_conv1_stage_split<(MBW1X > 1 ? MBW1X - 1 : 1)>(img, ring1, e1, before, mid, [&] { ring2.prologue(); });
     else
         a0_conv1_stage_split<MBW1X>(img, ring1, e1, before, mid, [&] { ring2.prologue(); });
-    P.act3 = (float*)uni((unsigned long long)act3_v);
-    a0_x9_conv23<ORD, 3, 2, false>(P, (int)e, smem, bias_lds, ring1, ring2, ring3);
-}
-
-template <int ORD>
-__global__ __launch_bounds__(A0_FUSED_THREADS, A0_FUSED_MINWAVES) void a0_actor_step_enc2_kernel(a0_qenv_args Q, a0_step_enc_args N) { a0_actor_step_enc2_body<ORD, TailScalar>(Q, N); }
+    if constexpr (PL) P.act3p = (uint32_t*)uni(act3_v);
+    else P.act3 = (float*)uni(act3_v);
+    a0_x9_conv23<ORD, 3, 2, false, PL>(P, (int)e, smem, bias_lds, ring1, ring2, ring3);
+}
+
+template <int ORD, bool PL>
+__global__ __launch_bounds__(A0_FUSED_THREADS, A0_FUSED_MINWAVES) void a0_actor_step_enc2_kernel(a0_qenv_args Q, a0_step_enc_args N) { a0_actor_step_enc2_body<ORD, TailScalar, PL>(Q, N); }
 
 static bool a0_fused_layout(int C, int H, int W, a0_fused_args& P, size_t& lds_bytes);
 int a0_actor_dist_step_enc_launch(const a0_dtenv_args& Q, size_t tail_lds, const float* wt, const a0_encoder_weights* w, float* act3, hipStream_t st) {
@@ -1051,7 +1063,7 @@
     size_t lds = 0;
     if (!wt || !w || !w->b1 || !w->b2 || !w->b3 || !act3 || !a0_fused_layout(4, 84, 84, P, lds)) return a0_fail(A0_EINVAL, "a0_actor_dist_tail_env_step_enc: bad encoder argument");
     if (P.H1 != 20 || P.W1 != 20 || P.H2 != 9 || P.W2 != 9 || P.H3 != 7 || P.W3 != 7) return a0_fail(A0_EINVAL, "a0_actor_dist_tail_env_step_enc: geometry");
-    const a0_step_enc_args N{wt, w->b1, w->b2, w->b3, act3};
+    const a0_step_enc_args N{wt, w->b1, w->b2, w->b3, act3, nullptr};
     lds = A0_X9_LDS_BYTES > tail_lds ? (size_t)A0_X9_LDS_BYTES : tail_lds;
     if (lds > 160 * 1024 - 64) return a0_fail(A0_EINVAL, "a0_actor_dist_tail_env_step_enc: head too wide for LDS");
     const int six = a0_x9_products_now() == 6;
@@ -1065,21 +1077,22 @@
     A0_LAUNCH_PROBED(A0_TAG_ACTOR_STEP_ENC, 2.0 * (400.0 * 32 * 256 + 81.0 * 64 * 512 + 49.0 * 64 * 576) * Q.E, kern, dim3(Q.E), dim3(A0_FUSED_THREADS), lds, st, Q, N);
     return a0_fail_hip((int)hipGetLastError(), "a0_actor_dist_tail_env_step_enc");
 }
-int a0_actor_step_enc_launch(const a0_qenv_args& Q, const float* wt, const a0_encoder_weights* w, float* act3, hipStream_t st) {
+int a0_actor_step_enc_launch(const a0_qenv_args& Q, const float* wt, const a0_encoder_weights* w, float* act3, uint32_t* act3p, hipStream_t st) {
     a0_fused_args P;
     size_t lds = 0;
     if (!wt || !w || !w->b1 || !w->b2 || !w->b3 || !act3 || !a0_fused_layout(4, 84, 84, P, lds)) return a0_fail(A0_EINVAL, "a0_actor_qhead_env_step_enc: bad encoder argument");
     if (P.H1 != 20 || P.W1 != 20 || P.H2 != 9 || P.W2 != 9 || P.H3 != 7 || P.W3 != 7) return a0_fail(A0_EINVAL, "a0_actor_qhead_env_step_enc: geometry");
-    const a0_step_enc_args N{wt, w->b1, w->b2, w->b3, act3};
+    const a0_step_enc_args N{wt, w->b1, w->b2, w->b3, act3, act3p};
     const size_t tail_lds = (size_t)(Q.A + (Q.dueling ? 1 : 0)) * 512 * sizeof(float);
     lds = A0_X9_LDS_BYTES > tail_lds ? (size_t)A0_X9_LDS_BYTES : tail_lds;
     const int six = a0_x9_products_now() == 6;
-    auto kern = six ? a0_actor_step_enc2_kernel<2> : a0_actor_step_enc2_kernel<4>;
-    static size_t configured[2] = {0, 0};
-    if (lds > configured[six]) {
+    const int pl = act3p ? 1 : 0;
+    auto kern = pl ? (six ? a0_actor_step_enc2_kernel<2, true> : a0_actor_step_enc2_kernel<4, true>) : (six ? a0_actor_step_enc2_kernel<2, false> : a0_actor_step_enc2_kernel<4, false>);
+    static size_t configured[2][2] = {{0, 0}, {0, 0}};
+    if (lds > configured[pl][six]) {
         if (hipFuncSetAttribute((const void*)kern, hipFuncAttributeMaxDynamicSharedMemorySize, (int)lds) != hipSuccess)
             return a0_fail(A0_EINVAL, "a0_actor_qhead_env_step_enc: LDS");
-        configured[six] = lds;
+        configured[pl][six] = lds;
     }
     A0_LAUNCH_PROBED(A0_TAG_ACTOR_STEP_ENC, 2.0 * (400.0 * 32 * 256 + 81.0 * 64 * 512 + 49.0 * 64 * 576) * Q.E, kern, dim3(Q.E), dim3(A0_FUSED_THREADS), lds, st, Q, N);
     return a0_fail_hip((int)hipGetLastError(), "a0_actor_qhead_env_step_enc");
@@ -1093,10 +1106,11 @@
     a0_encoder_fused_x9_body<ORD, 7, 3, 2, true>(M.p[k], bid - M.first[k], M.first[k + 1] - M.first[k]);
 }
 
-template <int MBW1, int MBW2, int MBW3, int WC, bool X9, bool LOOP, int ORD>
+template <int MBW1, int MBW2, int MBW3, int WC, bool X9, bool LOOP, int ORD, bool PL>
 __global__ __launch_bounds__(A0_FUSED_THREADS, A0_FUSED_MINWAVES) void a0_encoder_fused_kernel(a0_fused_args P) {
+    static_assert(!PL || X9, "feature planes from the split-operand encoder");
     if constexpr (X9) {
-        a0_encoder_fused_x9_body<ORD, MBW1, MBW2, MBW3, LOOP>(P, (int)blockIdx.x, (int)gridDim.x);
+        a0_encoder_fused_x9_body<ORD, MBW1, MBW2, MBW3, LOOP, PL>(P, (int)blockIdx.x, (int)gridDim.x);
         return;
     }
     extern __shared__ __attribute__((aligned(16))) unsigned char smem[];
@@ -1465,8 +1479,13 @@
 
 extern "C" int a0_net_encoder_fwd_fused(int C, int H, int W, const float* wt, const a0_encoder_weights* w, const a0_frames_arg* f, int B,
                                         float* act1, float* act2, float* act3, void* stream) {
+    return a0_net_encoder_fwd_fused_planes(C, H, W, wt, w, f, B, act1, act2, act3, nullptr, stream);
+}
+int a0_net_encoder_fwd_fused_planes(int C, int H, int W, const float* wt, const a0_encoder_weights* w, const a0_frames_arg* f, int B,
+                                    float* act1, float* act2, float* act3, uint32_t* act3p, void* stream) {
     A0_TRY
     if (!wt || !w || !w->b1 || !w->b2 || !w->b3 || !f || !f->frames || !act3 || B < 1) return a0_fail(A0_EINVAL, "a0_net_encoder_fwd_fused: bad argument");
+    if (act3p && !(C == 4 && H == 84 && W == 84)) return a0_fail(A0_EINVAL, "a0_net_encoder_fwd_fused: feature planes from the split-operand kernel (4 x 84 x 84) only");
     a0_fused_args P;
     size_t lds = 0;
     if (!a0_fused_layout(C, H, W, P, lds)) return a0_fail(A0_EINVAL, "a0_net_encoder_fwd_fused: observation shape not supported by the fused kernel");
@@ -1475,7 +1494,7 @@
     P.wt1 = wt; P.wt2 = wt + 48LL * C * 64; P.wt3 = P.wt2 + 64LL * 512;
     P.wx2 = P.wt3 + 64LL * 576 + 64LL * 576 + 4LL * 32 * 256; P.wx3 = P.wx2 + 96LL * 512;
     P.b1 = w->b1; P.b2 = w->b2; P.b3 = w->b3;
-    P.act1 = act1; P.act2 = act2; P.act3 = act3; P.B = B;
+    P.act1 = act1; P.act2 = act2; P.act3 = act3; P.act3p = act3p; P.B = B;
     const int mb1 = (P.H1 * P.W1 + 15) / 16, mb2 = (P.H2 * P.W2 + 15) / 16, mb3 = (P.H3 * P.W3 + 15) / 16;
     const bool standard = ((mb1 + 3) / 4 == 7) && ((mb2 + 1) / 2 == 3) && ((mb3 + 1) / 2 == 2) && W == 84;
     const bool x9 = standard && H == 84 && C == 4;
@@ -1484,11 +1503,14 @@
     static_assert(3 * 9 * A0_RP2X * 2 <= 2 * 4 * 84 * 84, "the act2 term planes fit into the dead image");
     const int gridx = (which == 2 && B > 256) ? 256 : B;
     if (which == 2 && gridx < B) which = 3;
-    static size_t configured[6] = {0, 0, 0, 0, 0, 0};
+    if (act3p && which != 2) return a0_fail(A0_EINVAL, "a0_net_encoder_fwd_fused: feature planes from the split-operand kernel, at most 256 observations");
+    static size_t configured[8] = {0, 0, 0, 0, 0, 0, 0, 0};
     const int six = a0_x9_products_now() == 6;
-    if (six && which >= 2) which += 2;
+    if (act3p) which = 6;
+    if (six && which >= 2) which += which >= 6 ? 1 : 2;
     typedef void (*a0_enc_kern)(a0_fused_args);
-    const a0_enc_kern fn = which == 5 ? a0_encoder_fused_kernel<7, 3, 2, 84, true, true, 2> : which == 4 ? a0_encoder_fused_kernel<7, 3, 2, 84, true, false, 2>
+    const a0_enc_kern fn = which == 7 ? a0_encoder_fused_kernel<7, 3, 2, 84, true, false, 2, true> : which == 6 ? a0_encoder_fused_kernel<7, 3, 2, 84, true, false, 4, true>
+                         : which == 5 ? a0_encoder_fused_kernel<7, 3, 2, 84, true, true, 2> : which == 4 ? a0_encoder_fused_kernel<7, 3, 2, 84, true, false, 2>
                          : which == 3 ? a0_encoder_fused_kernel<7, 3, 2, 84, true, true> : which == 2 ? a0_encoder_fused_kernel<7, 3, 2, 84, true>
                          : which == 1 ? a0_encoder_fused_kernel<7, 3, 2, 84, false> : a0_encoder_fused_kernel<7, 4, 2, 0, false>;
     if (lds > configured[which]) {
diff --git a/agent0_amd/csrc/igemm_x9.h b/agent0_amd/csrc/igemm_x9.h
--- a/agent0_amd/csrc/igemm_x9.h
+++ b/agent0_amd/csrc/igemm_x9.h
@@ -211,6 +211,7 @@
     static_assert(NPR == 9 || NPR == 6, "nine or six cross products");
     constexpr int NG = NPR * KS;
     static_assert(!EP::ROWSUM_A || OA::MODE == A0_XC, "row sums need an x-contiguous A operand");
+    static_assert(!EP::ROWSUM_A || !SA::PRESPLIT, "row sums are taken from fp32 A pieces");
     extern __shared__ __attribute__((aligned(16))) char a0_x9_lds[];
     char* const As = a0_x9_lds;
     char* const Bs = a0_x9_lds + 2 * G::ABYTES;
@@ -250,6 +251,12 @@
     auto micro = [&](int u, const typename SA::Slot& s_a_c, const typename SB::Slot& s_b_c, typename SA::Slot& s_a, typename SB::Slot& s_b,
                      char* a_dst, char* b_dst, int k_fetch) {
         const int p = u / 6, st = u % 6;
+        if constexpr (SA::PRESPLIT) {
+            if (p < RA) {
+                if (st == 5) { sa.store_raw(s_a_c, p, a_dst, tid); fetch_piece(s_a, s_b, p, k_fetch); }
+                return;
+            }
+        }
         if constexpr (SB::PRESPLIT) {
             if (p >= RA) {
                 if (st == 5) { sb.store_raw(s_b_c, p - RA, b_dst, tid); fetch_piece(s_a, s_b, p, k_fetch); }
diff --git a/agent0_amd/csrc/net.hip b/agent0_amd/csrc/net.hip
--- a/agent0_amd/csrc/net.hip
+++ b/agent0_amd/csrc/net.hip
@@ -451,6 +451,14 @@
     else bk.template igemm<OpMatKC, OpMatKC, EpiSlab, 4, 2, 1, 1>(a, bw, ep, R, N, K, splits);
 }
 
+int a0_fc1_planes_ok(int R, int K) { return (g_gemm_x9 != 0 && R >= 1 && a0_fc1_small(R) && K >= 32 && !(K & 31)) ? 1 : 0; }
+static void a0_fc1_partial_planes_launch(hipStream_t st, const uint32_t* xp, const uint32_t* wp, const EpiSlab::Params& ep, int R, int N, int K, int splits) {
+    hipEvent_t e0 = nullptr, e1 = nullptr;
+    const bool probe = a0_probe_events(A0_TAG_DENSE_FWD, &e0, &e1);
+    A0_HIP_THROW((a0_igemm_x9_launch<OpPlanesKC, OpPlanesKC, EpiSlab, 2, 2, 1, 1>(st, a0_planes_src{xp, K / 4}, a0_planes_src{wp, K / 4}, ep, R, N, K, splits, e0, e1)));
+    if (probe) a0_probe_commit(2.0 * (double)R * (double)N * (double)K);
+}
+
 extern "C" int a0_reduce_bias_act_multi(int n, const float* const* slabs, const long long* slab_stride, const int* nslab, const float* const* bias, float* const* out,
                                        const int* rows, int N, int relu, void* stream) {
     if (n < 1 || n > 4 || !slabs || !slab_stride || !nslab || !bias || !out || !rows || N < 4 || (N & 3)) return a0_fail(A0_EINVAL, "a0_reduce_bias_act_multi: bad argument (1..4 layers, N a multiple of 4)");
@@ -583,7 +591,20 @@
                                        unsigned long long env_seed, unsigned int rank, unsigned int g, const uint8_t* obs_in, uint8_t* obs_out, float* ep_ret,
                                        float* final_mask, float* final_ret, int n, long long steps, double gamma, int* ring_act, float* ring_rew, float* ring_done,
                                        const uint8_t* obs0, uint8_t* frames, long long cap, long long start_slot, int* r_act, float* r_rew, float* r_done, int task, void* stream) {
-    A0_TRY
+    return a0_actor_qhead_env_step_planes(feat, E, K, W1, b1, W2, b2, A, dueling, scratch, seed, stream_a, stream_u, off_a, off_u, eps, ctrl, eps_ptr, action, qmax,
+                                          env_seed, rank, g, obs_in, obs_out, ep_ret, final_mask, final_ret, n, steps, gamma, ring_act, ring_rew, ring_done, obs0, frames, cap,
+                                          start_slot, r_act, r_rew, r_done, task, nullptr, nullptr, stream);
+}
+int a0_actor_qhead_env_step_planes(const float* feat, int E, int K, const float* W1, const float* b1, const float* W2, const float* b2, int A, int dueling,
+                                   float* scratch, unsigned long long seed, unsigned int stream_a, unsigned int stream_u, unsigned long long off_a,
+                                   unsigned long long off_u, float eps, const long long* ctrl, const float* eps_ptr, int* action, float* qmax,
+                                   unsigned long long env_seed, unsigned int rank, unsigned int g, const uint8_t* obs_in, uint8_t* obs_out, float* ep_ret,
+                                   float* final_mask, float* final_ret, int n, long long steps, double gamma, int* ring_act, float* ring_rew, float* ring_done,
+                                   const uint8_t* obs0, uint8_t* frames, long long cap, long long start_slot, int* r_act, float* r_rew, float* r_done, int task,
+                                   const uint32_t* feat_planes, const uint32_t* w_planes, void* stream) {
+    A0_TRY
+    if ((feat_planes != nullptr) != (w_planes != nullptr) || (feat_planes && !a0_fc1_planes_ok(E, K)))
+        return a0_fail(A0_EINVAL, "a0_actor_qhead_env_step: pre-split fc1 operands come in pairs, for shapes a0_fc1_planes_ok accepts");
     if (!feat || !W1 || !b1 || !W2 || !b2 || !scratch || !action || !qmax || E < 1 || K < 4 || (K & 3) || A < 1 || A + (dueling ? 1 : 0) > 24)
         return a0_fail(A0_EINVAL, "a0_actor_qhead_env_step: bad argument (A + dueling <= 24: the head rows are staged in 48 KB of LDS)");
     if (!obs_in || !obs_out || obs_in == obs_out || !ep_ret || !final_mask || !final_ret || !ring_act || !ring_rew || !ring_done || !obs0 || !frames || !r_act ||
@@ -596,7 +617,8 @@
     a0_mat_src bw{W1, K};
     EpiSlab::Params ep{scratch, (long long)E * 512, 512};
     bk.tag = A0_TAG_DENSE_FWD;
-    a0_fc1_partial_launch(bk, a, bw, ep, E, 512, K, splits);
+    if (feat_planes) a0_fc1_partial_planes_launch((hipStream_t)stream, feat_planes, w_planes, ep, E, 512, K, splits);
+    else a0_fc1_partial_launch(bk, a, bw, ep, E, 512, K, splits);
     a0_qenv_args P;
     P.slabs = scratch; P.slab_stride = (long long)E * 512; P.nslab = splits; P.b1 = b1; P.W2 = W2; P.b2 = b2; P.A = A; P.dueling = dueling; P.E = E;
     P.rng_seed = seed; P.stream_a = stream_a; P.stream_u = stream_u; P.off_a = off_a; P.off_u = off_u; P.eps = eps; P.ctrl = ctrl; P.eps_ptr = eps_ptr;
@@ -617,7 +639,21 @@
                                            float* final_mask, float* final_ret, int n, long long steps, double gamma, int* ring_act, float* ring_rew, float* ring_done,
                                            const uint8_t* obs0, uint8_t* frames, long long cap, long long start_slot, int* r_act, float* r_rew, float* r_done, int task,
                                            const float* wt, const a0_encoder_weights* w, float* act3_next, void* stream) {
-    A0_TRY
+    return a0_actor_qhead_env_step_enc_planes(feat, E, K, W1, b1, W2, b2, A, dueling, scratch, seed, stream_a, stream_u, off_a, off_u, eps, ctrl, eps_ptr, action, qmax,
+                                              env_seed, rank, g, obs_in, obs_out, ep_ret, final_mask, final_ret, n, steps, gamma, ring_act, ring_rew, ring_done, obs0, frames, cap,
+                                              start_slot, r_act, r_rew, r_done, task, wt, w, act3_next, nullptr, nullptr, nullptr, stream);
+}
+int a0_actor_qhead_env_step_enc_planes(const float* feat, int E, int K, const float* W1, const float* b1, const float* W2, const float* b2, int A, int dueling,
+                                       float* scratch, unsigned long long seed, unsigned int stream_a, unsigned int stream_u, unsigned long long off_a,
+                                       unsigned long long off_u, float eps, const long long* ctrl, const float* eps_ptr, int* action, float* qmax,
+                                       unsigned long long env_seed, unsigned int rank, unsigned int g, const uint8_t* obs_in, uint8_t* obs_out, float* ep_ret,
+                                       float* final_mask, float* final_ret, int n, long long steps, double gamma, int* ring_act, float* ring_rew, float* ring_done,
+                                       const uint8_t* obs0, uint8_t* frames, long long cap, long long start_slot, int* r_act, float* r_rew, float* r_done, int task,
+                                       const float* wt, const a0_encoder_weights* w, float* act3_next, const uint32_t* feat_planes, const uint32_t* w_planes,
+                                       uint32_t* act3p_next, void* stream) {
+    A0_TRY
+    if ((feat_planes != nullptr) != (w_planes != nullptr) || (feat_planes && !a0_fc1_planes_ok(E, K)))
+        return a0_fail(A0_EINVAL, "a0_actor_qhead_env_step_enc: pre-split fc1 operands come in pairs, for shapes a0_fc1_planes_ok accepts");
     if (!feat || !W1 || !b1 || !W2 || !b2 || !scratch || !action || !qmax || E < 1 || K != 3136 || A < 1 || A + (dueling ? 1 : 0) > 24)
         return a0_fail(A0_EINVAL, "a0_actor_qhead_env_step_enc: bad argument (4 x 84 x 84 observations, A + dueling <= 24)");
     if (!obs_in || !obs_out || obs_in == obs_out || !ep_ret || !final_mask || !final_ret || !ring_act || !ring_rew || !ring_done || !obs0 || !frames || !r_act ||
@@ -630,7 +666,8 @@
     a0_mat_src bw{W1, K};
     EpiSlab::Params ep{scratch, (long long)E * 512, 512};
     bk.tag = A0_TAG_DENSE_FWD;
-    a0_fc1_partial_launch(bk, a, bw, ep, E, 512, K, splits);
+    if (feat_planes) a0_fc1_partial_planes_launch((hipStream_t)stream, feat_planes, w_planes, ep, E, 512, K, splits);
+    else a0_fc1_partial_launch(bk, a, bw, ep, E, 512, K, splits);
     a0_qenv_args P;
     P.slabs = scratch; P.slab_stride = (long long)E * 512; P.nslab = splits; P.b1 = b1; P.W2 = W2; P.b2 = b2; P.A = A; P.dueling = dueling; P.E = E;
     P.rng_seed = seed; P.stream_a = stream_a; P.stream_u = stream_u; P.off_a = off_a; P.off_u = off_u; P.eps = eps; P.ctrl = ctrl; P.eps_ptr = eps_ptr;
@@ -638,7 +675,7 @@
     P.env_seed = env_seed; P.rank = rank; P.g = g; P.obs_in = obs_in; P.obs_out = obs_out; P.ep_ret = ep_ret; P.final_mask = final_mask; P.final_ret = final_ret;
     P.n = n; P.steps = steps; P.gamma = gamma; P.ring_act = ring_act; P.ring_rew = ring_rew; P.ring_done = ring_done; P.obs0 = obs0; P.frames = frames;
     P.cap = cap; P.start = start_slot % cap; P.r_act = r_act; P.r_rew = r_rew; P.r_done = r_done; P.task = task;
-    return a0_actor_step_enc_launch(P, wt, w, act3_next, (hipStream_t)stream);
+    return a0_actor_step_enc_launch(P, wt, w, act3_next, act3p_next, (hipStream_t)stream);
     A0_CATCH
 }
 
diff --git a/agent0_amd/csrc/runtime.hip b/agent0_amd/csrc/runtime.hip
--- a/agent0_amd/csrc/runtime.hip
+++ b/agent0_amd/csrc/runtime.hip
@@ -267,6 +267,8 @@
     bool bound = false;
     float *own_flat = nullptr, *own_wt = nullptr, *own_eff = nullptr, *own_noise = nullptr;
     unsigned int* w_planes = nullptr;
+    uint32_t* f_planes = nullptr;
+    bool fc1_planes_on = true;
 };
 
 struct a0_actor_net {
@@ -307,6 +309,9 @@
             a->head_slabs = a->mem.alloc<float>((long long)a0_dense_fwd_partial_slabs(E, L->Npad, 512) * E * L->Npad);
             const long long sc = a0_dense_fwd_scratch(E, 512, L->feat);
             a->fwd_scratch = a->mem.alloc<float>(sc > 4 ? sc : 4);
+        } else if (!L->d.noisy && L->C == 4 && L->H == 84 && L->W == 84 && a->feat == L->feat && a0_fc1_planes_ok(E, L->feat)) {
+            a->w_planes = a->mem.alloc<unsigned int>(a0_weight_planes_words(512, L->feat), false);
+            a->f_planes = a->mem.alloc<uint32_t>(a0_weight_planes_words(E, L->feat), false);
         }
         a->dist_Npad = L->Npad;
         a->bound = true;
@@ -364,6 +369,12 @@
 }
 
 extern "C" int a0_actor_destroy(a0_actor* a) { delete a; return A0_OK; }
+
+extern "C" int a0_actor_fc1_planes(a0_actor* a, int enable) {
+    if (!a) return a0_fail(A0_EINVAL, "a0_actor_fc1_planes: null handle");
+    a->fc1_planes_on = enable != 0;
+    return A0_OK;
+}
 
 static int a0_actor_compose(const a0_actor_net& V, void* stream) {
     const a0_learner* L = V.L;
@@ -398,6 +409,10 @@
     if (planes && !(L->d.noisy && a->steps % freq == 0)) A0_CHECK(a0_split_planes(V.Wf(), a->w_planes, 512, L->feat, stream));
     const bool step_enc = !a->own_flat;
     bool feat_ready = false;
+    const bool fc1p = !quant && !dist && step_enc && a->f_planes && a->fc1_planes_on;
+    uint32_t* const fp = fc1p ? a->f_planes : nullptr;
+    const uint32_t* const wp = fc1p ? a->w_planes : nullptr;
+    if (fc1p) A0_CHECK(a0_split_planes(V.Wf(), a->w_planes, 512, L->feat, stream));
     for (int t = 0; t < a->T; ++t) {
         if (L->d.noisy && a->steps % freq == 0) {
             A0_CHECK(a0_rng_normal(a->rng.seed, 4 , a->rng.reserve(4, L->noise_len), 0.1f, V.noise, L->noise_len, stream));
@@ -406,7 +421,7 @@
         }
         const uint8_t* cur_obs = a->obs[a->cur];
         a0_frames_arg f{cur_obs, nullptr, (long long)a->obs_bytes, 0};
-        if (!feat_ready) A0_CHECK(a0_net_encoder_fwd_fused(L->C, L->H, L->W, V.wt, &w, &f, E, nullptr, nullptr, a->act3, stream));
+        if (!feat_ready) A0_CHECK(a0_net_encoder_fwd_fused_planes(L->C, L->H, L->W, V.wt, &w, &f, E, nullptr, nullptr, a->act3, fp, stream));
         feat_ready = false;
         const long long back = (a->steps + 1 < a->n ? a->steps + 1 : a->n) - 1;
         const uint8_t* obs0 = a->obs[((a->cur - back) % a->K + a->K) % a->K];
@@ -476,18 +491,18 @@
         const int nxt = (a->cur + 1) % a->K;
         a->g += 1;
         if (step_enc && t + 1 < a->T) {
-            A0_CHECK(a0_actor_qhead_env_step_enc(a->act3, E, a->feat, V.Wf(), V.bf(), V.Wh(), V.bh(), A, a->d.dueling ? 1 : 0,
+            A0_CHECK(a0_actor_qhead_env_step_enc_planes(a->act3, E, a->feat, V.Wf(), V.bf(), V.Wh(), V.bh(), A, a->d.dueling ? 1 : 0,
                                                  a->scratch, a->rng.seed, STREAM_EGREEDY_A, STREAM_EGREEDY_U, off_a, off_u, epsilon, nullptr, nullptr, a->action, a->qmax_all + (long long)t * E,
                                                  a->d.seed, a->d.rank, a->g, cur_obs, a->obs[nxt], a->ep_ret, a->stat_mask + (long long)t * E, a->stat_ret + (long long)t * E, a->n, a->steps,
                                                  a->d.discount, a->ring_act, a->ring_rew, a->ring_done, obs0, R->frames, R->size, (start + (long long)t * E) % R->size, R->act, R->rew, R->done,
-                                                 a->d.env_task, V.wt, &w, a->act3, stream));
+                                                 a->d.env_task, V.wt, &w, a->act3, fp, wp, fp, stream));
             feat_ready = true;
         } else
-        A0_CHECK(a0_actor_qhead_env_step(a->act3, E, a->feat, V.Wf(), V.bf(), V.Wh(), V.bh(), A, a->d.dueling ? 1 : 0,
+        A0_CHECK(a0_actor_qhead_env_step_planes(a->act3, E, a->feat, V.Wf(), V.bf(), V.Wh(), V.bh(), A, a->d.dueling ? 1 : 0,
                                          a->scratch, a->rng.seed, STREAM_EGREEDY_A, STREAM_EGREEDY_U, off_a, off_u, epsilon, nullptr, nullptr, a->action, a->qmax_all + (long long)t * E,
                                          a->d.seed, a->d.rank, a->g, cur_obs, a->obs[nxt], a->ep_ret, a->stat_mask + (long long)t * E, a->stat_ret + (long long)t * E, a->n, a->steps,
                                          a->d.discount, a->ring_act, a->ring_rew, a->ring_done, obs0, R->frames, R->size, (start + (long long)t * E) % R->size, R->act, R->rew, R->done,
-                                         a->d.env_task, stream));
+                                         a->d.env_task, fp, wp, stream));
         a->cur = nxt;
         a->steps += 1;
     }
diff --git a/include/agent0_hip.h b/include/agent0_hip.h
--- a/include/agent0_hip.h
+++ b/include/agent0_hip.h
@@ -277,6 +277,7 @@
 int a0_actor_destroy(a0_actor* actor);
 int a0_actor_bind(a0_actor* actor, const a0_learner* learner, int own_network);
 int a0_actor_snapshot(a0_actor* actor, const a0_learner* learner, void* stream);
+int a0_actor_fc1_planes(a0_actor* actor, int enable);
 int a0_actor_rollout(a0_actor* actor, a0_learner* learner, a0_rbuf* replay, float epsilon, void* stream);
 int a0_actor_collect(a0_actor* actor, float* qs_host, float* returns_host, int max_returns, int* n_returns, void* stream);
 int a0_actor_collect_begin(a0_actor* actor, void* stream);
```

Result: no change. 2.333 million (median of 6 runs) (+0.4%).
